# skamann/mcmc-dynamics

Measured on AMD Instinct MI355X. Metric: star-walker log-L terms/sec, higher is better.
Workload: dtype f64; 1 GPU; C3: 1e6 synthetic stars x 256 walkers, rotation+dispersion + fixed single-Gaussian background mixture (ConstantFit + background.Gaussian), fixed centre; stars_per_gpu=1000000, stars_total=1000000, walkers=256, likelihood=bgfixed, parallelism=1 GPU

## Files before the change

include/mcd.h:

```cpp
#ifndef MCD_H
#define MCD_H

#include <stdint.h>

#ifdef __cplusplus
extern "C" {
#endif

#define MCD_ABI_VERSION 1
#define MCD_UNIQUE_ID_BYTES 128

typedef struct mcd_ctx mcd_ctx;
typedef struct mcd_catalog mcd_catalog;

typedef enum {
    MCD_OK = 0,
    MCD_ERR_INVALID = -1,
    MCD_ERR_HIP = -2,
    MCD_ERR_RCCL = -3,
    MCD_ERR_NO_DEVICE = -4,
    MCD_ERR_NONFINITE = -5,
    MCD_ERR_NOMEM = -6
} mcd_status;

typedef enum {
    MCD_MODEL_CONST = 0,
    MCD_MODEL_CONST_BGFIXED = 1,
    MCD_MODEL_CONST_BGGAUSS = 2,
    MCD_MODEL_PROFILE = 3,
    MCD_MODEL_PROFILE_BGGAUSS = 4,
    MCD_MODEL_PROFILE_BGDENS = 5,
    MCD_MODEL_PROFILE_BGFIXED = 6
} mcd_model;

typedef enum {
    MCD_CENTRE_FIXED = 0,
    MCD_CENTRE_FREE = 1
} mcd_centre;

typedef enum {
    MCD_F64 = 0,
    MCD_F32 = 1,
    MCD_F32_ACC64 = 2
} mcd_precision;

typedef struct {
    int64_t n_stars;
    const double* ra;
    const double* dec;
    const double* v;
    const double* verr;
    const double* lnlike_bg;
    const double* pmember;
    const double* density;
    int32_t model;
    int32_t centre;
    int32_t precision;
    int32_t reserved;
    double ra_center;
    double dec_center;
    int64_t n_bins;
    const int64_t* bin_offsets;
} mcd_catalog_desc;


int mcd_ctx_create(int n_dev, const int* dev_ids, mcd_ctx** out);

int mcd_get_unique_id(void* out_id);
int mcd_ctx_create_rank(int device, int rank, int n_ranks, const void* unique_id, mcd_ctx** out);

int mcd_ctx_set_option(mcd_ctx* ctx, const char* key, int64_t value);
int mcd_ctx_abort(mcd_ctx* ctx, const char* reason);
int mcd_ctx_failed(const mcd_ctx* ctx);

int mcd_ctx_destroy(mcd_ctx* ctx);
int mcd_ctx_n_devices(const mcd_ctx* ctx);
int mcd_ctx_comm_info(const mcd_ctx* ctx, int* comm_size, int* comm_rank, int* rccl_version);


int mcd_catalog_create(mcd_ctx* ctx, const mcd_catalog_desc* desc, mcd_catalog** out);
int mcd_catalog_destroy(mcd_catalog* cat);

int mcd_catalog_param_count(const mcd_catalog* cat);
int64_t mcd_catalog_n_stars(const mcd_catalog* cat);
int64_t mcd_catalog_n_outputs(const mcd_catalog* cat, int64_t n_walkers);


int mcd_loglike_batch(mcd_catalog* cat, int64_t n_walkers, int32_t k, const double* params, double* out);

int mcd_params_upload(mcd_catalog* cat, int64_t n_walkers, int32_t k, const double* params);
int mcd_loglike_enqueue(mcd_catalog* cat);
int mcd_loglike_fetch(mcd_catalog* cat, double* out);
int mcd_sync(mcd_catalog* cat);

int mcd_membership(mcd_catalog* cat, int32_t k, const double* params, double* out);
int mcd_loglike_per_star(mcd_catalog* cat, int32_t k, const double* params, double* out);
int mcd_loglike_grad_batch(mcd_catalog* cat, int64_t n_walkers, int32_t k, const double* params, double* out,
                           double* grad);
int mcd_pointwise_posterior(mcd_catalog* cat, int64_t n_samples, int32_t k, const double* params,
                            double* lppd, double* lnl_var, double* pmem_mean, double* pmem_std);
int mcd_psis_loo(mcd_catalog* cat, int64_t n_samples, int32_t k, const double* params, double r_eff,
                 double* elpd_loo, double* pareto_k, double* lppd, double* n_eff);

int mcd_kde_background(mcd_ctx* ctx, int64_t n_comp, const double* comp, int64_t n, const double* v,
                       const double* verr, double sigma_int, double* out, double* kernel_ms);


typedef struct {
    int64_t n_walkers;
    int32_t n_dim;
    int32_t k;
    const int32_t* col_source;
    const double* col_const;
    const double* col_factor;
    const double* lo;
    const double* hi;
    int32_t fixed_ok;
    int32_t n_bins;
} mcd_stretch_desc;

int mcd_stretch_move(mcd_catalog* cat, const mcd_stretch_desc* desc, int64_t n_steps, double* pos, double* lnp,
                     const int32_t* order, const double* zz, const double* thr, const int32_t* pick, double* chain,
                     double* lnprob_chain, int64_t* accepted);
int mcd_stretch_move_seeded(mcd_catalog* cat, const mcd_stretch_desc* desc, int64_t n_steps, double* pos, double* lnp,
                            uint64_t seed, int64_t step0, double* chain, double* lnprob_chain, int64_t* accepted);
int mcd_chain_numbers(uint64_t seed, int64_t step0, int64_t n_steps, int64_t n_bins, int64_t n_walkers, int32_t n_dim,
                      int32_t* order, double* zz, double* thr, int32_t* pick);

int mcd_stretch_info(const mcd_catalog* cat, int64_t* device_blocks, int64_t* host_blocks, int64_t* discarded_blocks,
                     int32_t* last_discard_status);

typedef struct {
    mcd_stretch_desc map;
    const double* chol;
    double step_size;
    double jitter;
    int32_t n_leap;
} mcd_hmc_desc;

int mcd_hmc_block(mcd_catalog* cat, const mcd_hmc_desc* desc, int64_t n_steps, double* pos, double* lnp, uint64_t seed,
                  int64_t step0, double* chain, double* lnprob_chain, int64_t* accepted, double* energy_error);
int mcd_hmc_numbers(uint64_t seed, int64_t step0, int64_t n_steps, int64_t n_walkers, int32_t n_dim, double* z, double* thr,
                    double* eps_factor);
int mcd_hmc_info(const mcd_catalog* cat, int64_t* device_blocks, int64_t* host_blocks);


const char* mcd_last_error(void);
int mcd_abi_version(void);
double mcd_last_kernel_ms(const mcd_catalog* cat);
double mcd_last_device_ms(const mcd_catalog* cat);
int mcd_set_option(mcd_catalog* cat, const char* key, int64_t value);
int mcd_timing_collect(mcd_catalog* cat, double* total_kernel_ms, int64_t* n_launches);
int64_t mcd_rerun_count(const mcd_catalog* cat);
int mcd_last_prefetch(const mcd_catalog* cat);
int mcd_last_narrow_bounded(const mcd_catalog* cat);
int64_t mcd_last_series_chunks(const mcd_catalog* cat);
int64_t mcd_last_direct_chunks(const mcd_catalog* cat);
int mcd_last_fast_level(const mcd_catalog* cat);

int mcd_last_f32_domain(const mcd_catalog* cat, double* kappa_v, double* kappa_theta);
int mcd_last_launch_info(const mcd_catalog* cat, int64_t* n_workgroups, int32_t* walker_tile,
                         int64_t* n_chunks, int32_t* record_bytes);

#ifdef __cplusplus
}
#endif
#endif
```

mcmc_dynamics_amd/_native.py:

```python
import atexit
import ctypes
import os
import weakref

import numpy as np

_HERE = os.path.dirname(os.path.abspath(__file__))
LIB_PATH = os.environ.get("MCD_LIB_PATH") or os.path.join(_HERE, "libmcd_hip.so")

MODEL_CONST, MODEL_CONST_BGFIXED, MODEL_CONST_BGGAUSS = 0, 1, 2
MODEL_PROFILE, MODEL_PROFILE_BGGAUSS, MODEL_PROFILE_BGDENS, MODEL_PROFILE_BGFIXED = 3, 4, 5, 6
CENTRE_FIXED, CENTRE_FREE = 0, 1
F64, F32, F32_ACC64 = 0, 1, 2
PRECISIONS = {"f64": F64, "f32": F32, "f32acc64": F32_ACC64}
UNIQUE_ID_BYTES = 128

_c_double_p = ctypes.POINTER(ctypes.c_double)
_c_int64_p = ctypes.POINTER(ctypes.c_int64)

SYMBOLS = {
    "mcd_ctx_create": (ctypes.c_int, [ctypes.c_int, ctypes.POINTER(ctypes.c_int), ctypes.POINTER(ctypes.c_void_p)]),
    "mcd_get_unique_id": (ctypes.c_int, [ctypes.c_void_p]),
    "mcd_ctx_create_rank": (ctypes.c_int, [ctypes.c_int, ctypes.c_int, ctypes.c_int, ctypes.c_void_p,
                                           ctypes.POINTER(ctypes.c_void_p)]),
    "mcd_ctx_destroy": (ctypes.c_int, [ctypes.c_void_p]),
    "mcd_ctx_set_option": (ctypes.c_int, [ctypes.c_void_p, ctypes.c_char_p, ctypes.c_int64]),
    "mcd_ctx_abort": (ctypes.c_int, [ctypes.c_void_p, ctypes.c_char_p]),
    "mcd_ctx_failed": (ctypes.c_int, [ctypes.c_void_p]),
    "mcd_ctx_n_devices": (ctypes.c_int, [ctypes.c_void_p]),
    "mcd_ctx_comm_info": (ctypes.c_int, [ctypes.c_void_p, ctypes.POINTER(ctypes.c_int), ctypes.POINTER(ctypes.c_int),
                                         ctypes.POINTER(ctypes.c_int)]),
    "mcd_catalog_create": (ctypes.c_int, [ctypes.c_void_p, ctypes.c_void_p, ctypes.POINTER(ctypes.c_void_p)]),
    "mcd_catalog_destroy": (ctypes.c_int, [ctypes.c_void_p]),
    "mcd_catalog_param_count": (ctypes.c_int, [ctypes.c_void_p]),
    "mcd_catalog_n_stars": (ctypes.c_int64, [ctypes.c_void_p]),
    "mcd_catalog_n_outputs": (ctypes.c_int64, [ctypes.c_void_p, ctypes.c_int64]),
    "mcd_loglike_batch": (ctypes.c_int, [ctypes.c_void_p, ctypes.c_int64, ctypes.c_int32, _c_double_p, _c_double_p]),
    "mcd_loglike_grad_batch": (ctypes.c_int, [ctypes.c_void_p, ctypes.c_int64, ctypes.c_int32, _c_double_p, _c_double_p,
                                              _c_double_p]),
    "mcd_params_upload": (ctypes.c_int, [ctypes.c_void_p, ctypes.c_int64, ctypes.c_int32, _c_double_p]),
    "mcd_loglike_enqueue": (ctypes.c_int, [ctypes.c_void_p]),
    "mcd_loglike_fetch": (ctypes.c_int, [ctypes.c_void_p, _c_double_p]),
    "mcd_sync": (ctypes.c_int, [ctypes.c_void_p]),
    "mcd_membership": (ctypes.c_int, [ctypes.c_void_p, ctypes.c_int32, _c_double_p, _c_double_p]),
    "mcd_loglike_per_star": (ctypes.c_int, [ctypes.c_void_p, ctypes.c_int32, _c_double_p, _c_double_p]),
    "mcd_pointwise_posterior": (ctypes.c_int, [ctypes.c_void_p, ctypes.c_int64, ctypes.c_int32, _c_double_p, _c_double_p,
                                               _c_double_p, _c_double_p, _c_double_p]),
    "mcd_psis_loo": (ctypes.c_int, [ctypes.c_void_p, ctypes.c_int64, ctypes.c_int32, _c_double_p, ctypes.c_double,
                                    _c_double_p, _c_double_p, _c_double_p, _c_double_p]),
    "mcd_kde_background": (ctypes.c_int, [ctypes.c_void_p, ctypes.c_int64, _c_double_p, ctypes.c_int64, _c_double_p,
                                          _c_double_p, ctypes.c_double, _c_double_p, _c_double_p]),
    "mcd_stretch_move": (ctypes.c_int, [ctypes.c_void_p, ctypes.c_void_p, ctypes.c_int64, _c_double_p, _c_double_p,
                                        ctypes.POINTER(ctypes.c_int32), _c_double_p, _c_double_p,
                                        ctypes.POINTER(ctypes.c_int32), _c_double_p, _c_double_p, _c_int64_p]),
    "mcd_stretch_move_seeded": (ctypes.c_int, [ctypes.c_void_p, ctypes.c_void_p, ctypes.c_int64, _c_double_p, _c_double_p,
                                               ctypes.c_uint64, ctypes.c_int64, _c_double_p, _c_double_p, _c_int64_p]),
    "mcd_chain_numbers": (ctypes.c_int, [ctypes.c_uint64, ctypes.c_int64, ctypes.c_int64, ctypes.c_int64, ctypes.c_int64,
                                         ctypes.c_int32, ctypes.POINTER(ctypes.c_int32), _c_double_p, _c_double_p,
                                         ctypes.POINTER(ctypes.c_int32)]),
    "mcd_stretch_info": (ctypes.c_int, [ctypes.c_void_p, _c_int64_p, _c_int64_p, _c_int64_p, ctypes.POINTER(ctypes.c_int32)]),
    "mcd_hmc_block": (ctypes.c_int, [ctypes.c_void_p, ctypes.c_void_p, ctypes.c_int64, _c_double_p, _c_double_p,
                                     ctypes.c_uint64, ctypes.c_int64, _c_double_p, _c_double_p, _c_int64_p, _c_double_p]),
    "mcd_hmc_numbers": (ctypes.c_int, [ctypes.c_uint64, ctypes.c_int64, ctypes.c_int64, ctypes.c_int64, ctypes.c_int32,
                                       _c_double_p, _c_double_p, _c_double_p]),
    "mcd_hmc_info": (ctypes.c_int, [ctypes.c_void_p, _c_int64_p, _c_int64_p]),
    "mcd_last_error": (ctypes.c_char_p, []),
    "mcd_abi_version": (ctypes.c_int, []),
    "mcd_last_kernel_ms": (ctypes.c_double, [ctypes.c_void_p]),
    "mcd_last_device_ms": (ctypes.c_double, [ctypes.c_void_p]),
    "mcd_timing_collect": (ctypes.c_int, [ctypes.c_void_p, _c_double_p, _c_int64_p]),
    "mcd_rerun_count": (ctypes.c_int64, [ctypes.c_void_p]),
    "mcd_last_prefetch": (ctypes.c_int, [ctypes.c_void_p]),
    "mcd_last_narrow_bounded": (ctypes.c_int, [ctypes.c_void_p]),
    "mcd_last_series_chunks": (ctypes.c_int64, [ctypes.c_void_p]),
    "mcd_last_direct_chunks": (ctypes.c_int64, [ctypes.c_void_p]),
    "mcd_last_fast_level": (ctypes.c_int, [ctypes.c_void_p]),
    "mcd_last_f32_domain": (ctypes.c_int, [ctypes.c_void_p, _c_double_p, _c_double_p]),
    "mcd_set_option": (ctypes.c_int, [ctypes.c_void_p, ctypes.c_char_p, ctypes.c_int64]),
    "mcd_last_launch_info": (ctypes.c_int, [ctypes.c_void_p, _c_int64_p, ctypes.POINTER(ctypes.c_int32), _c_int64_p,
                                            ctypes.POINTER(ctypes.c_int32)]),
}


class NativeError(RuntimeError):
    """Raised when the HIP library is missing, fails to load, or a call returns an error status."""


class CatalogDesc(ctypes.Structure):
    _fields_ = [
        ("n_stars", ctypes.c_int64),
        ("ra", _c_double_p), ("dec", _c_double_p), ("v", _c_double_p), ("verr", _c_double_p),
        ("lnlike_bg", _c_double_p), ("pmember", _c_double_p), ("density", _c_double_p),
        ("model", ctypes.c_int32), ("centre", ctypes.c_int32), ("precision", ctypes.c_int32),
        ("reserved", ctypes.c_int32),
        ("ra_center", ctypes.c_double), ("dec_center", ctypes.c_double),
        ("n_bins", ctypes.c_int64), ("bin_offsets", _c_int64_p),
    ]


class StretchDesc(ctypes.Structure):
    _fields_ = [
        ("n_walkers", ctypes.c_int64), ("n_dim", ctypes.c_int32), ("k", ctypes.c_int32),
        ("col_source", ctypes.POINTER(ctypes.c_int32)), ("col_const", _c_double_p), ("col_factor", _c_double_p),
        ("lo", _c_double_p), ("hi", _c_double_p), ("fixed_ok", ctypes.c_int32), ("n_bins", ctypes.c_int32),
    ]


class HmcDesc(ctypes.Structure):
    _fields_ = [("map", StretchDesc), ("chol", _c_double_p), ("step_size", ctypes.c_double), ("jitter", ctypes.c_double),
                ("n_leap", ctypes.c_int32)]


TEST_SWITCHES = ("MCD_LIB_PATH", "MCD_RCCL_LIBRARY", "MCD_ALLOW_SHARED_DEVICE", "MCD_FORCE_RCCL", "MCD_TARGET_WAVES",
                 "MCD_CHAIN_PART_BYTES", "MCD_CHAIN_PARTS", "MCD_COLLECTIVE_TIMEOUT_MS")

_lib = None
_live_catalogs = weakref.WeakSet()
_live_contexts = weakref.WeakSet()


@atexit.register
def _shutdown():
    for cat in list(_live_catalogs):
        try:
            cat.close()
        except Exception:
            pass
    for ctx in list(_live_contexts):
        try:
            ctx.close()
        except Exception:
            pass


def load_library(path=None):
    global _lib
    if _lib is not None and path is None:
        return _lib
    p = path or LIB_PATH
    if not os.path.exists(p):
        raise NativeError(
            "HIP library not found at {0}: build it with `make -C mcmc_dynamics_amd/csrc` "
            "(or __graft_entry__.build()); there is no CPU fallback.".format(p))
    try:
        lib = ctypes.CDLL(p)
    except OSError as exc:
        raise NativeError("could not load {0}: {1}".format(p, exc))
    for name, (restype, argtypes) in SYMBOLS.items():
        try:
            fn = getattr(lib, name)
        except AttributeError:
            raise NativeError("{0} does not export {1}".format(p, name))
        fn.restype = restype
        fn.argtypes = argtypes
    if path is None:
        _lib = lib
        active = ["{0}={1}".format(k, os.environ[k]) for k in TEST_SWITCHES if os.environ.get(k)]
        if active:
            import logging
            logging.getLogger("mcmc_dynamics_amd").warning(
                "test / tuning switches active (none is needed in production, see INTEGRATION.md): %s", ", ".join(active))
    return lib


def _check(lib, rc, what):
    if rc != 0:
        msg = lib.mcd_last_error()
        raise NativeError("{0} failed (status {1}): {2}".format(what, rc, msg.decode() if msg else ""))


def _f64(a):
    return np.ascontiguousarray(a, dtype=np.float64)


def _ptr(a):
    return a.ctypes.data_as(_c_double_p) if a is not None else None


class Context(object):

    def __init__(self, n_devices=1, device_ids=None, rank=None, n_ranks=None, unique_id=None, device=None):
        self.lib = load_library()
        handle = ctypes.c_void_p()
        if rank is not None:
            uid = ctypes.create_string_buffer(bytes(unique_id), UNIQUE_ID_BYTES) if unique_id is not None else None
            rc = self.lib.mcd_ctx_create_rank(int(device or 0), int(rank), int(n_ranks), uid, ctypes.byref(handle))
            _check(self.lib, rc, "mcd_ctx_create_rank")
            self.rank, self.n_ranks = int(rank), int(n_ranks)
        else:
            ids = None
            if device_ids is not None:
                ids = (ctypes.c_int * len(device_ids))(*[int(d) for d in device_ids])
                n_devices = len(device_ids)
            rc = self.lib.mcd_ctx_create(int(n_devices), ids, ctypes.byref(handle))
            _check(self.lib, rc, "mcd_ctx_create")
            self.rank, self.n_ranks = 0, 1
        self.handle = handle
        self.host_group = None
        self._catalogs = weakref.WeakSet()
        _live_contexts.add(self)

    @staticmethod
    def unique_id():
        lib = load_library()
        buf = ctypes.create_string_buffer(UNIQUE_ID_BYTES)
        _check(lib, lib.mcd_get_unique_id(buf), "mcd_get_unique_id")
        return buf.raw

    @property
    def n_devices(self):
        return self.lib.mcd_ctx_n_devices(self.handle)

    def set_option(self, key, value):
        _check(self.lib, self.lib.mcd_ctx_set_option(self.handle, key.encode(), int(value)), "mcd_ctx_set_option")

    def abort(self, reason=""):
        if getattr(self, "handle", None):
            self.lib.mcd_ctx_abort(self.handle, str(reason).encode()[:400])

    @property
    def failed(self):
        return bool(getattr(self, "handle", None)) and bool(self.lib.mcd_ctx_failed(self.handle))

    def comm_info(self):
        n, r, v = ctypes.c_int(), ctypes.c_int(), ctypes.c_int()
        _check(self.lib, self.lib.mcd_ctx_comm_info(self.handle, ctypes.byref(n), ctypes.byref(r), ctypes.byref(v)),
               "mcd_ctx_comm_info")
        return {"size": n.value, "rank": r.value, "rccl_version": v.value}
# ... 121 lines not shown
        if p.shape[-1] != self.k:
            raise ValueError("params have {0} columns, catalogue expects {1}".format(p.shape[-1], self.k))
        return np.ascontiguousarray(p), w

    def _alive(self):
        if not getattr(self, "handle", None):
            raise NativeError("catalogue is closed")

    def loglike(self, params):
        self._alive()
        p, w = self._params(params)
        out = np.empty((self.n_sets, w) if self.n_sets > 1 else (w,), dtype=np.float64)
        rc = self.lib.mcd_loglike_batch(self.handle, w, self.k, _ptr(p), _ptr(out))
        _check(self.lib, rc, "mcd_loglike_batch")
        self._walkers = w
        return out

    def loglike_grad(self, params, want_value=True):
        self._alive()
        p, w = self._params(params)
        lead = (self.n_sets, w) if self.n_sets > 1 else (w,)
        out = np.empty(lead, dtype=np.float64) if want_value else None
        grad = np.empty(lead + (self.k,), dtype=np.float64)
        rc = self.lib.mcd_loglike_grad_batch(self.handle, w, self.k, _ptr(p), _ptr(out), _ptr(grad))
        _check(self.lib, rc, "mcd_loglike_grad_batch")
        self._walkers = w
        return out, grad

    def upload_params(self, params):
        p, w = self._params(params)
        _check(self.lib, self.lib.mcd_params_upload(self.handle, w, self.k, _ptr(p)), "mcd_params_upload")
        self._walkers = w

    def enqueue(self):
        _check(self.lib, self.lib.mcd_loglike_enqueue(self.handle), "mcd_loglike_enqueue")

    def sync(self):
        _check(self.lib, self.lib.mcd_sync(self.handle), "mcd_sync")

    def fetch(self):
        w = self._walkers
        out = np.empty((self.n_sets, w) if self.n_sets > 1 else (w,), dtype=np.float64)
        _check(self.lib, self.lib.mcd_loglike_fetch(self.handle, _ptr(out)), "mcd_loglike_fetch")
        return out

    def membership(self, params_row):
        p = _f64(params_row).reshape(-1)
        out = np.empty(self.n_stars, dtype=np.float64)
        _check(self.lib, self.lib.mcd_membership(self.handle, p.size, _ptr(p), _ptr(out)), "mcd_membership")
        return out

    def loglike_per_star(self, params_row):
        p = _f64(params_row).reshape(-1)
        out = np.empty(self.n_stars, dtype=np.float64)
        _check(self.lib, self.lib.mcd_loglike_per_star(self.handle, p.size, _ptr(p), _ptr(out)), "mcd_loglike_per_star")
        return out

    def pointwise_posterior(self, table, membership=False):
        self._alive()
        if self.n_sets > 1:
            raise ValueError("pointwise_posterior is defined for un-binned catalogues only")
        p = _f64(table)
        if p.ndim == 1:
            p = p[None, :]
        if p.ndim != 2 or p.shape[1] != self.k:
            raise ValueError("table must have shape (S, {0})".format(self.k))
        p = np.ascontiguousarray(p)
        names = ("lppd", "lnl_var") + (("pmem_mean", "pmem_std") if membership else ())
        out = {k: np.empty(self.n_stars, dtype=np.float64) for k in names}
        ptrs = [_ptr(out[k]) if k in out else None for k in ("lppd", "lnl_var", "pmem_mean", "pmem_std")]
        rc = self.lib.mcd_pointwise_posterior(self.handle, p.shape[0], self.k, _ptr(p), *ptrs)
        _check(self.lib, rc, "mcd_pointwise_posterior")
        return out

    def psis_loo(self, table, r_eff=1.0):
        self._alive()
        if self.n_sets > 1:
            raise ValueError("psis_loo is defined for un-binned catalogues only")
        p = _f64(table)
        if p.ndim == 1:
            p = p[None, :]
        if p.ndim != 2 or p.shape[1] != self.k:
            raise ValueError("table must have shape (S, {0})".format(self.k))
        p = np.ascontiguousarray(p)
        names = ("elpd_loo", "pareto_k", "lppd", "n_eff")
        out = {k: np.empty(self.n_stars, dtype=np.float64) for k in names}
        rc = self.lib.mcd_psis_loo(self.handle, p.shape[0], self.k, _ptr(p), float(r_eff), *[_ptr(out[k]) for k in names])
        _check(self.lib, rc, "mcd_psis_loo")
        return out

    def _stretch_args(self, name, plan, pos, lnp, n_steps, chain, lnprob_chain, accepted):
        self._alive()
        for a in (pos, lnp):
            if a.dtype != np.float64 or not a.flags.c_contiguous:
                raise ValueError(name + " needs C-contiguous arrays of the documented dtypes")
        if pos.ndim not in (2, 3) or lnp.shape != pos.shape[:-1]:
            raise ValueError(name + ": inconsistent array shapes")
        lead, (w, p) = pos.shape[:-2], pos.shape[-2:]
        cols = [np.ascontiguousarray(plan["col_source"], dtype=np.int32), _f64(plan["col_const"]), _f64(plan["col_factor"]),
                _f64(plan["lo"]), _f64(plan["hi"])]
        if cols[0].size != self.k or cols[1].size != self.k or cols[2].size != self.k or cols[3].size != p or cols[4].size != p:
            raise ValueError("stretch_move: plan does not match the catalogue / the number of free parameters")
        d = StretchDesc()
        d.n_walkers, d.n_dim, d.k, d.n_bins = w, p, self.k, lead[0] if lead else 1
        d.col_source = cols[0].ctypes.data_as(ctypes.POINTER(ctypes.c_int32))
        d.col_const, d.col_factor, d.lo, d.hi = (_ptr(c) for c in cols[1:])
        d.fixed_ok = 1 if plan.get("fixed_ok", True) else 0
        for a, shape in ((chain, (n_steps,) + lead + (w, p)), (lnprob_chain, (n_steps,) + lead + (w,))):
            if a is not None and (a.dtype != np.float64 or not a.flags.c_contiguous or a.shape != shape):
                raise ValueError("stretch_move: chain buffers must be C-contiguous float64 of shape (steps, [B,] W, P) / (steps, [B,] W)")
        if accepted is not None and (accepted.dtype != np.int64 or accepted.shape != lead + (w,) or not accepted.flags.c_contiguous):
            raise ValueError("stretch_move: accepted must be a C-contiguous int64 array of shape ([B,] W)")
        return ((self.handle, ctypes.byref(d), n_steps, _ptr(pos), _ptr(lnp)),
                (_ptr(chain), _ptr(lnprob_chain), accepted.ctypes.data_as(_c_int64_p) if accepted is not None else None), cols)

    def stretch_move(self, plan, pos, lnp, order, zz, thr, pick, chain=None, lnprob_chain=None, accepted=None):
        head, tail, _keep = self._stretch_args("stretch_move", plan, pos, lnp, order.shape[0], chain, lnprob_chain, accepted)
        for a, dt in ((zz, np.float64), (thr, np.float64), (order, np.int32), (pick, np.int32)):
            if a.dtype != dt or not a.flags.c_contiguous:
                raise ValueError("stretch_move needs C-contiguous arrays of the documented dtypes")
        half_shape = (order.shape[0], 2) + pos.shape[:-2] + (pos.shape[-2] // 2,)
        if order.shape != order.shape[:1] + lnp.shape or zz.shape != half_shape or thr.shape != half_shape or \
                pick.shape != half_shape:
            raise ValueError("stretch_move: inconsistent array shapes")
        rc = self.lib.mcd_stretch_move(*head, order.ctypes.data_as(ctypes.POINTER(ctypes.c_int32)), _ptr(zz), _ptr(thr),
                                       pick.ctypes.data_as(ctypes.POINTER(ctypes.c_int32)), *tail)
        _check(self.lib, rc, "mcd_stretch_move")
        self._walkers = pos.shape[-2] // 2

    def stretch_move_seeded(self, plan, pos, lnp, seed, step0, n_steps, chain=None, lnprob_chain=None, accepted=None):
        if n_steps < 0 or step0 < 0:
            raise ValueError("stretch_move_seeded: inconsistent array shapes")
        head, tail, _keep = self._stretch_args("stretch_move_seeded", plan, pos, lnp, n_steps, chain, lnprob_chain, accepted)
        rc = self.lib.mcd_stretch_move_seeded(*head, int(seed) & 0xFFFFFFFFFFFFFFFF, int(step0), *tail)
        _check(self.lib, rc, "mcd_stretch_move_seeded")
        self._walkers = pos.shape[-2] // 2

    @property
    def last_prefetch(self):
        return self.lib.mcd_last_prefetch(self.handle)

    @property
    def last_narrow_bounded(self):
        return self.lib.mcd_last_narrow_bounded(self.handle)

    @property
    def last_series_chunks(self):
        return self.lib.mcd_last_series_chunks(self.handle)

    @property
    def last_direct_chunks(self):
        return self.lib.mcd_last_direct_chunks(self.handle)

    def hmc_block(self, plan, chol, step_size, n_leap, pos, lnp, seed, step0, n_steps, chain=None, lnprob_chain=None,
                  accepted=None, energy_error=None, jitter=0.1):
        if n_steps < 0 or step0 < 0 or pos.ndim != 2:
            raise ValueError("hmc_block: inconsistent array shapes")
        head, tail, _keep = self._stretch_args("hmc_block", plan, pos, lnp, n_steps, chain, lnprob_chain, accepted)
        chol = np.ascontiguousarray(chol, dtype=np.float64)
        if chol.shape != (pos.shape[1], pos.shape[1]):
            raise ValueError("hmc_block: chol must have shape (P, P)")
        if energy_error is not None and (energy_error.dtype != np.float64 or not energy_error.flags.c_contiguous or
                                         energy_error.shape != (n_steps, pos.shape[0])):
            raise ValueError("hmc_block: energy_error must be a C-contiguous float64 array of shape (steps, W)")
        d = HmcDesc()
        d.map = head[1]._obj
        d.chol, d.step_size, d.jitter, d.n_leap = _ptr(chol), float(step_size), float(jitter), int(n_leap)
        rc = self.lib.mcd_hmc_block(self.handle, ctypes.byref(d), int(n_steps), head[3], head[4],
                                    int(seed) & 0xFFFFFFFFFFFFFFFF, int(step0), *tail, _ptr(energy_error))
        _check(self.lib, rc, "mcd_hmc_block")

    def hmc_info(self):
        a, b = ctypes.c_int64(), ctypes.c_int64()
        _check(self.lib, self.lib.mcd_hmc_info(self.handle, ctypes.byref(a), ctypes.byref(b)), "mcd_hmc_info")
        return {"device_blocks": a.value, "host_blocks": b.value}

    def stretch_info(self):
        a, b, c, st = ctypes.c_int64(), ctypes.c_int64(), ctypes.c_int64(), ctypes.c_int32()
        _check(self.lib, self.lib.mcd_stretch_info(self.handle, ctypes.byref(a), ctypes.byref(b), ctypes.byref(c), ctypes.byref(st)),
               "mcd_stretch_info")
        return {"device_blocks": a.value, "host_blocks": b.value, "discarded_blocks": c.value, "last_discard_status": st.value}

    def set_option(self, key, value):
        _check(self.lib, self.lib.mcd_set_option(self.handle, key.encode(), int(value)), "mcd_set_option")

    @property
    def last_kernel_ms(self):
        return self.lib.mcd_last_kernel_ms(self.handle)

    @property
    def last_device_ms(self):
        return self.lib.mcd_last_device_ms(self.handle)

    def timing_collect(self):
        total, n = ctypes.c_double(), ctypes.c_int64()
        _check(self.lib, self.lib.mcd_timing_collect(self.handle, ctypes.byref(total), ctypes.byref(n)),
               "mcd_timing_collect")
        return total.value, n.value

    @property
    def rerun_count(self):
        return self.lib.mcd_rerun_count(self.handle)

    @property
    def fast_level(self):
        return self.lib.mcd_last_fast_level(self.handle)

    @property
    def f32_in_domain(self):
        return bool(self.lib.mcd_last_f32_domain(self.handle, None, None))

    @property
    def f32_condition(self):
        kv, kt = ctypes.c_double(), ctypes.c_double()
        self.lib.mcd_last_f32_domain(self.handle, ctypes.byref(kv), ctypes.byref(kt))
        return kv.value, kt.value

    def launch_info(self):
        wg, ch = ctypes.c_int64(), ctypes.c_int64()
        tile, rb = ctypes.c_int32(), ctypes.c_int32()
        _check(self.lib, self.lib.mcd_last_launch_info(self.handle, ctypes.byref(wg), ctypes.byref(tile),
                                                       ctypes.byref(ch), ctypes.byref(rb)), "mcd_last_launch_info")
        return {"workgroups": wg.value, "walker_tile": tile.value, "chunks": ch.value, "record_bytes": rb.value,
                "series_chunks": self.last_series_chunks, "direct_chunks": self.last_direct_chunks}

    def close(self):
        if getattr(self, "handle", None):
            self.lib.mcd_catalog_destroy(self.handle)
            self.handle = None

    def __del__(self):
        try:
            self.close()
        except Exception:
            pass
```

mcmc_dynamics_amd/csrc/mcd_api_catalog.hip:

```cpp
#include "mcd_host.h"

using namespace mcd::host;

namespace {

int param_count(int model, bool free_centre) {
    int k = (mcd::is_profile(model) ? 6 : 4) + (free_centre ? 2 : 0);
    const int bg = mcd::bg_kind(model);
    if (bg == mcd::BG_GAUSS) k += 3;
    if (bg == mcd::BG_FIXED_DENSITY) k += 1;
    return k;
}

void free_workset(WorkSet& w) {
    if (w.d_chunks) (void)hipFree(w.d_chunks);
    if (w.d_offsets) (void)hipFree(w.d_offsets);
    if (w.d_chunk_general) (void)hipFree(w.d_chunk_general);
    if (w.d_params) (void)hipFree(w.d_params);
    if (w.d_wpar) (void)hipFree(w.d_wpar);
    if (w.d_partials) (void)hipFree(w.d_partials);
    if (w.d_out) (void)hipFree(w.d_out);
    if (w.d_out2) (void)hipFree(w.d_out2);
    if (w.d_partials2) (void)hipFree(w.d_partials2);
    if (w.d_grad_partials) (void)hipFree(w.d_grad_partials);
    if (w.d_grad_out) (void)hipFree(w.d_grad_out);
    if (w.h_grad_out) (void)hipHostFree(w.h_grad_out);
    if (w.ev_staged) (void)hipEventDestroy(w.ev_staged);
    for (int b = 0; b < 2; ++b) {
        if (w.ev_reduced[b]) (void)hipEventDestroy(w.ev_reduced[b]);
        if (w.ev_comm[b]) (void)hipEventDestroy(w.ev_comm[b]);
    }
    if (w.h_params) (void)hipHostFree(w.h_params);
    if (w.h_out) (void)hipHostFree(w.h_out);
    w = WorkSet();
}

double model_cost(int model, bool free_centre) {
    static const double kCost[mcd::kNumModels] = {8.5, 24.0, 45.0, 25.0, 60.0, 40.0, 42.0};
    return (kCost[model] + (free_centre ? 7.0 : 0.0)) / 8.5;
}
int balance_auto_m(const mcd_catalog* cat, int64_t n, int64_t n_walkers) {
    const int64_t n_wtiles = (n_walkers + 63) / 64;
    const double tiles = n_wtiles <= 4 ? (double)n_wtiles : 4.0 * (double)((n_wtiles + 3) / 4);
    const double work = (double)n * tiles / 4.0 * model_cost(cat->model, cat->free_centre);
    const double limit = mcd::bg_kind(cat->model) == mcd::BG_NONE ? 9.0e5 : 1.3e6;
    if (cat->n_psets != 1 || work > limit) return 0;
    return work < 6.0e4 ? 2 : (work <= 3.4e5 ? 4 : 8);
}

bool wants_prefetch(const mcd_catalog* cat, const Shard& sh) {
    if (cat->prefetch >= 0) return cat->prefetch != 0;
    const size_t bytes = (size_t)sh.n * (size_t)mcd::record_bytes(cat->model, cat->free_centre, cat->precision);
    if (mcd::bg_kind(cat->model) == mcd::BG_NONE) return cat->n_psets == 1 && bytes >= ((size_t)128 << 20);
    return bytes >= ((size_t)8 << 20);
}

bool wants_sorted(const mcd_catalog* cat, const Shard& sh) {
    if (cat->model != mcd::MODEL_BGFIXED || cat->free_centre || cat->precision != MCD_F64 || cat->n_psets != 1 || sh.n <= 0)
        return false;
    if (cat->verr_sorted >= 0) return cat->verr_sorted != 0;
    if (cat->chunk_len > 0) return false;
    return (size_t)sh.n * (size_t)mcd::record_bytes(cat->model, cat->free_centre, cat->precision) >= ((size_t)8 << 20);
}

int ensure_sorted_records(mcd_catalog* cat, Shard& sh) {
    if (sh.records_sorted) return MCD_OK;
    const DeviceSlot& slot = cat->ctx->slots[sh.slot];
    constexpr int ND = mcd::record_doubles(mcd::MODEL_BGFIXED, false);
    const size_t n = (size_t)sh.n, bytes = n * ND * sizeof(double);
    MCD_HIP(hipStreamSynchronize(slot.stream));
    std::vector<double> rec(n * ND), out(n * ND);
    MCD_HIP(hipMemcpy(rec.data(), sh.records, bytes, hipMemcpyDeviceToHost));
    const std::vector<int64_t> perm = mcd::verr_order(rec.data(), (int64_t)n, ND);
    sh.sorted_e2.resize(n);
    for (size_t i = 0; i < n; ++i) {
        std::memcpy(&out[i * ND], &rec[(size_t)perm[i] * ND], ND * sizeof(double));
        sh.sorted_e2[i] = out[i * ND + 1];
    }
    sh.sorted_exceptions = mcd::permuted_exceptions(cat->stats.narrow_exceptions, perm, sh.star_begin);
    void* d = nullptr;
    MCD_HIP(hipMalloc(&d, bytes + 2048));
    hipError_t e = hipMemset(d, 0, bytes + 2048);
    if (e == hipSuccess) e = hipMemcpy(d, out.data(), bytes, hipMemcpyHostToDevice);
    if (e != hipSuccess) { (void)hipFree(d); MCD_HIP(e); }
    sh.records_sorted = d;
    return MCD_OK;
}

struct Option {
    const char* key;
    int64_t min, max;
    const char* message;
    bool sync, replan;
    void (*set)(mcd_catalog* c, int64_t v);
    bool (*accepts)(int64_t v) = nullptr;
};
constexpr int64_t kMin = std::numeric_limits<int64_t>::min(), kMax = std::numeric_limits<int64_t>::max();
#define MCD_SET(statement) [](mcd_catalog* c, int64_t v) { statement; }
const Option kOptions[] = {
    {"fast_path", 0, 2, "fast_path: 0 (plain), 1 (guarded, default) or 2 (guarded, no narrow variant)", false, false, MCD_SET(c->allow_fast = (int)v)},
    {"zero_copy", kMin, kMax, nullptr, false, false, MCD_SET(c->zero_copy = v != 0)},
    {"device_chain", 0, 2, "device_chain: 0 (host-driven blocks), 1 (default) or 2 (as 1 with the general step kernel, testing aid)", false, false,
     MCD_SET(c->device_chain = (int)v; c->chain_backoff = 0; c->chain_consecutive = 0; c->chain_hint = -1)},
    {"fused_reduce", kMin, kMax, nullptr, false, false, MCD_SET(c->fused_reduce = v != 0)},
    {"defer_guard", kMin, kMax, nullptr, false, false, MCD_SET(c->defer_guard = v != 0)},
    {"f32_domain", kMin, kMax, nullptr, false, false, MCD_SET(c->f32_domain = v != 0)},
    {"loo_scratch_mb", 1, kMax, "loo_scratch_mb must be >= 1", false, false, MCD_SET(c->loo_scratch_mb = v)},
    {"posterior_pass", 1, kMax, "posterior_pass must be >= 1", false, false, MCD_SET(c->posterior_pass = v)},
    {"two_lanes", kMin, kMax, nullptr, true, false, MCD_SET(c->two_lanes = v != 0)},
    {"narrow_bounded", 0, 1, "narrow_bounded: 1 (where the guard admits it, default) or 0 (never)", false, false, MCD_SET(c->narrow_bounded = (int)v)},
    {"verr_sorted", -1, 1, "verr_sorted: -1 (by record volume, default), 0 (catalogue order) or 1 (sorted by verr)", true, true, MCD_SET(c->verr_sorted = (int)v)},
    {"root_series", 0, 1, "root_series: 1 (series root on the narrow chunks of verr-sorted records, default) or 0 (never)", false, false, MCD_SET(c->root_series = (int)v)},
    {"root_direct", 0, 1, "root_direct: 1 (direct form of the series root where a chunk admits it, default) or 0 (delta form only)", false, false, MCD_SET(c->root_direct = (int)v)},
    {"prefetch", -1, 1, "prefetch: -1 (by record volume, default), 0 (off) or 1 (on)", false, false, MCD_SET(c->prefetch = (int)v)},
    {"spin_us", 0, kMax, "spin_us must be >= 0", false, false, MCD_SET(c->spin_us = v)},
    {"tail_split", kMin, kMax, nullptr, true, true, MCD_SET(c->tail_split = (int)v)},
    {"target_waves", 1, kMax, "target_waves must be positive", true, true, MCD_SET(c->target_waves = v)},
    {"chunk_len", 0, kMax, "chunk_len must be >= 0", true, true, MCD_SET(c->chunk_len = v)},
    {"balance", -1, 8, "balance: -1 (auto), 0 (off) or 1 .. 8 workgroups per CU", true, true, MCD_SET(c->balance = (int)v)},
    {"combine", 0, 16, "combine: 0 (never), 1 (largest workgroup the plan allows), 8 or 16 (waves per workgroup at most)", true, true,
     MCD_SET(c->combine = (int)v), [](int64_t v) { return v <= 1 || v == 8 || v == 16; }},
};
#undef MCD_SET
}

MCD_HOST_BEGIN

LaunchShape main_launch_shape(mcd_catalog* cat, const Shard& sh, const WorkSet& w, int level, bool coll, double* out_buf,
                              int64_t n_out) {
    LaunchShape shape{cat->model, cat->free_centre, cat->precision, level, w.uniform_len, sh.n};
    shape.uniform_extra = w.uniform_extra;
    shape.waves = w.waves;
    shape.chunk_general = w.d_chunk_general;
    shape.prefetch = wants_prefetch(cat, sh);
    cat->last_prefetch = shape.prefetch && shape.fast != 0;
    shape.rerun_flag = coll ? nullptr : out_buf + n_out;
    shape.root_series = w.sorted && cat->root_series != 0;
    shape.root_direct = shape.root_series && cat->root_direct != 0;
    return shape;
}

const void* main_records(const Shard& sh, const WorkSet& w) { return w.sorted ? sh.records_sorted : sh.records; }

int64_t series_chunk_count(const mcd_catalog* cat, const WorkSet& w, int level, const double* params, int64_t n_rows) {
    if (!w.sorted || !cat->root_series || level != 2 || w.series_need.empty()) return 0;
    const mcd::ParamRanges pr = mcd::table_ranges(cat->model, cat->free_centre, cat->k, params, n_rows);
    if (!pr.finite) return 0;
    return (int64_t)(std::upper_bound(w.series_need.begin(), w.series_need.end(), pr.s2_min) - w.series_need.begin());
}

int64_t direct_chunk_count(const mcd_catalog* cat, const WorkSet& w, int level, const double* params, int64_t n_rows) {
    if (!w.sorted || !cat->root_series || !cat->root_direct || level != 2 || w.direct_need.empty()) return 0;
    const mcd::ParamRanges pr = mcd::table_ranges(cat->model, cat->free_centre, cat->k, params, n_rows);
    if (!pr.finite) return 0;
    return (int64_t)(std::upper_bound(w.direct_need.begin(), w.direct_need.end(), pr.s2_min) - w.direct_need.begin());
}

const double* fast_pset_const(const mcd_catalog* cat, const Shard& sh, int level) {
    const int bgk = mcd::bg_kind(cat->model);
    return (level && (bgk == mcd::BG_FIXED || bgk == mcd::BG_FIXED_DENSITY)) ? sh.d_pset_const : nullptr;
}

int build_workset(mcd_catalog* cat, Shard& sh, int64_t n_walkers, WorkSet** out) {
    auto it = sh.work.find(n_walkers);
    if (it != sh.work.end()) { *out = &it->second; return MCD_OK; }
    if (sh.work.size() >= 8) {
        for (auto& kv : sh.work) free_workset(kv.second);
        sh.work.clear();
        cat->cur_walkers = 0;
    }
    const DeviceSlot& slot = cat->ctx->slots[sh.slot];
    MCD_HIP(hipSetDevice(slot.device));

    const bool sorted = wants_sorted(cat, sh);
    if (sorted)
        if (int rc = ensure_sorted_records(cat, sh)) return rc;
    const std::vector<int64_t>& exceptions = sorted ? sh.sorted_exceptions : cat->stats.narrow_exceptions;
    mcd::ChunkPlan plan;
    for (int m = cat->balance < 0 ? balance_auto_m(cat, sh.n, n_walkers) : cat->balance;; m /= 2) {
        plan = mcd::plan_chunks(cat->bin_offsets, sh.star_begin, sh.n, n_walkers, cat->target_waves, cat->tail_split,
                                exceptions, cat->chunk_len, m);
        if (m == 0 || plan.balanced_m > 0) break;
    }
    const std::vector<mcd::Chunk>& chunks = plan.chunks;
    const std::vector<int64_t>& offs = plan.offsets;
    const std::vector<uint8_t>& general = plan.general;

    WorkSet w;
    w.n_walkers = n_walkers;
    w.n_chunks = (int64_t)chunks.size();
    w.max_chunks_per_pset = plan.max_chunks_per_pset;
    w.uniform_len = plan.uniform_len;
    w.uniform_extra = plan.uniform_extra;
    w.sorted = sorted;
    if (sorted) {
        w.series_need = mcd::series_thresholds(plan, sh.sorted_e2.data());
        w.direct_need = mcd::direct_thresholds(plan, sh.sorted_e2.data());
    }
    {
        const int64_t n_wtiles = (n_walkers + 63) / 64;
        const bool shape_ok = plan.balanced_m > 0 && plan.balanced_m % 2 == 0 && (n_wtiles == 1 || n_wtiles == 2 || n_wtiles == 4) &&
                              cat->precision == MCD_F64;
        w.waves = 4;
        if (cat->combine != 0 && shape_ok) {
            const bool can16 = mcd::bg_kind(cat->model) != mcd::BG_GAUSS;
            w.waves = 8;
            if (cat->combine == 16 && plan.balanced_m % 4 == 0 && can16) w.waves = 16;
            if (cat->combine == 1 && plan.balanced_m == 4 && can16) w.waves = 16;
        }
    }
    const int64_t n_out = cat->n_psets * n_walkers;
    const size_t term_bytes = cat->precision == MCD_F64 ? 8 : 4;
    auto allocate = [&]() -> hipError_t {
        hipError_t e;
        if (!general.empty()) {
            if ((e = hipMalloc(&w.d_chunk_general, general.size())) != hipSuccess) return e;
            if ((e = hipMemcpy(w.d_chunk_general, general.data(), general.size(), hipMemcpyHostToDevice)) != hipSuccess) return e;
        }
        if ((e = hipMalloc(&w.d_chunks, std::max<size_t>(1, chunks.size()) * sizeof(mcd::Chunk))) != hipSuccess) return e;
        if ((e = hipMalloc(&w.d_offsets, offs.size() * sizeof(int64_t))) != hipSuccess) return e;
        if ((e = hipMalloc(&w.d_params, (size_t)n_out * cat->k * sizeof(double))) != hipSuccess) return e;
        if ((e = hipMalloc(&w.d_wpar, (size_t)n_out * mcd::KD * term_bytes)) != hipSuccess) return e;
        if ((e = hipMalloc(&w.d_partials, std::max<size_t>(1, (size_t)mcd::padded_walkers(n_walkers) * w.n_chunks) * sizeof(double))) != hipSuccess) return e;
        if ((e = hipMalloc(&w.d_out, (size_t)(n_out + 1) * sizeof(double))) != hipSuccess) return e;
        if ((e = hipMemset(w.d_out, 0, (size_t)(n_out + 1) * sizeof(double))) != hipSuccess) return e;
        if ((e = hipMalloc(&w.d_out2, (size_t)(n_out + 1) * sizeof(double))) != hipSuccess) return e;
        if ((e = hipMemset(w.d_out2, 0, (size_t)(n_out + 1) * sizeof(double))) != hipSuccess) return e;
        if ((e = hipEventCreateWithFlags(&w.ev_staged, hipEventDisableTiming)) != hipSuccess) return e;
        for (int b = 0; b < 2; ++b) {
            if ((e = hipEventCreateWithFlags(&w.ev_reduced[b], hipEventDisableTiming)) != hipSuccess) return e;
            if ((e = hipEventCreateWithFlags(&w.ev_comm[b], hipEventDisableTiming)) != hipSuccess) return e;
        }
        if ((e = hipHostMalloc(&w.h_params, (size_t)n_out * cat->k * sizeof(double), hipHostMallocMapped)) != hipSuccess) return e;
        if ((e = hipHostMalloc(&w.h_out, (size_t)(n_out + 1) * sizeof(double), hipHostMallocMapped)) != hipSuccess) return e;
        std::memset(w.h_out, 0, (size_t)(n_out + 1) * sizeof(double));
        if ((e = hipHostGetDevicePointer((void**)&w.m_params, w.h_params, 0)) != hipSuccess) return e;
        if ((e = hipHostGetDevicePointer((void**)&w.m_out, w.h_out, 0)) != hipSuccess) return e;
        if (!chunks.empty() &&
            (e = hipMemcpy(w.d_chunks, chunks.data(), chunks.size() * sizeof(mcd::Chunk), hipMemcpyHostToDevice)) != hipSuccess)
            return e;
        return hipMemcpy(w.d_offsets, offs.data(), offs.size() * sizeof(int64_t), hipMemcpyHostToDevice);
    };
    const hipError_t err = allocate();
    if (err != hipSuccess) {
        free_workset(w);
        return fail(MCD_ERR_HIP, std::string("work buffers for this walker count: ") + hipGetErrorString(err));
    }
    auto ins = sh.work.emplace(n_walkers, w);
    *out = &ins.first->second;
    return MCD_OK;
}

MCD_HOST_END

extern "C" {

static int catalog_create_impl(mcd_ctx* ctx, const mcd_catalog_desc* d, std::unique_ptr<mcd_catalog>& cat);

int mcd_catalog_create(mcd_ctx* ctx, const mcd_catalog_desc* d, mcd_catalog** out) {
    try {
    if (!ctx || !d || !out) return fail(MCD_ERR_INVALID, "mcd_catalog_create: null argument");
    std::unique_ptr<mcd_catalog> cat;
    const int rc = catalog_create_impl(ctx, d, cat);
    if (rc != MCD_OK) {
        if (cat) {
            const std::string msg = g_last_error;
            mcd_catalog_destroy(cat.release());
            g_last_error = msg;
        }
        return rc;
    }
    *out = cat.release();
    return MCD_OK;
    } catch (...) { return on_exception("mcd_catalog_create"); }
}

static int catalog_create_impl(mcd_ctx* ctx, const mcd_catalog_desc* d, std::unique_ptr<mcd_catalog>& cat) {
    if (int urc = ctx_usable(ctx)) return urc;
    if (d->n_stars < 0) return fail(MCD_ERR_INVALID, "negative n_stars");
    if (d->model < 0 || d->model >= mcd::kNumModels) return fail(MCD_ERR_INVALID, "unknown model");
    const int bgk = mcd::bg_kind(d->model);
    if (d->centre != MCD_CENTRE_FIXED && d->centre != MCD_CENTRE_FREE) return fail(MCD_ERR_INVALID, "unknown centre mode");
    if (d->precision < MCD_F64 || d->precision > MCD_F32_ACC64) return fail(MCD_ERR_INVALID, "unknown precision");
    if (d->n_stars > 0 && (!d->ra || !d->dec || !d->v || !d->verr)) return fail(MCD_ERR_INVALID, "missing ra/dec/v/verr column");
    if (bgk == mcd::BG_FIXED && d->n_stars > 0 && (!d->lnlike_bg || !d->pmember))
        return fail(MCD_ERR_INVALID, "background model needs lnlike_bg and pmember columns");
    if (bgk == mcd::BG_GAUSS && d->n_stars > 0 && !d->density)
        return fail(MCD_ERR_INVALID, "Gaussian-background model needs the density column");
    if (bgk == mcd::BG_FIXED_DENSITY && d->n_stars > 0 && (!d->lnlike_bg || !d->density))
        return fail(MCD_ERR_INVALID, "constant-background model needs lnlike_bg and density columns");

    cat.reset(new (std::nothrow) mcd_catalog());
    if (!cat) return fail(MCD_ERR_INVALID, "out of memory");
    cat->ctx = ctx;
    cat->model = d->model;
    cat->free_centre = d->centre == MCD_CENTRE_FREE;
    cat->precision = d->precision;
    cat->k = param_count(d->model, cat->free_centre);
    cat->n_stars = d->n_stars;
    if (const char* tw = std::getenv("MCD_TARGET_WAVES")) {
        long v = std::atol(tw);
        if (v > 0) cat->target_waves = v;
    }
    if (d->n_bins > 1) {
        if (!d->bin_offsets) return fail(MCD_ERR_INVALID, "bin_offsets required when n_bins > 1");
        cat->n_psets = d->n_bins;
        cat->bin_offsets.assign(d->bin_offsets, d->bin_offsets + d->n_bins + 1);
        if (cat->bin_offsets.front() != 0 || cat->bin_offsets.back() != d->n_stars)
            return fail(MCD_ERR_INVALID, "bin_offsets must start at 0 and end at n_stars");
        for (int64_t b = 0; b < d->n_bins; ++b)
            if (cat->bin_offsets[b + 1] < cat->bin_offsets[b]) return fail(MCD_ERR_INVALID, "bin_offsets must be non-decreasing");
    } else {
        cat->n_psets = 1;
        cat->bin_offsets = {0, d->n_stars};
    }

    cat->stats = mcd::compute_stats(d->n_stars, d->v, d->verr, d->lnlike_bg, d->pmember, d->density, bgk,
                                    cat->precision != MCD_F64 || mcd::is_profile(cat->model) ? d->ra : nullptr, d->dec,
                                    !cat->free_centre, d->ra_center, d->dec_center);

    const int n_dev = (int)ctx->slots.size();
    cat->shards.resize(n_dev);
    const int rec_bytes = mcd::record_bytes(cat->model, cat->free_centre, cat->precision);
    for (int i = 0; i < n_dev; ++i) {
        Shard& sh = cat->shards[i];
        sh.slot = i;
        const mcd::ShardRange range = mcd::shard_range(d->n_stars, i, n_dev);
        sh.star_begin = range.begin;
        sh.n = range.n;
        const DeviceSlot& slot = ctx->slots[i];
        MCD_HIP(hipSetDevice(slot.device));
        MCD_HIP(hipEventCreate(&sh.ev_begin));
        MCD_HIP(hipEventCreate(&sh.ev_k0));
        MCD_HIP(hipEventCreate(&sh.ev_k1));
        MCD_HIP(hipEventCreate(&sh.ev_end));
        MCD_HIP(hipMalloc(&sh.records, (size_t)sh.n * rec_bytes + 2048));
        MCD_HIP(hipMemsetAsync(sh.records, 0, (size_t)sh.n * rec_bytes + 2048, slot.stream));
        if (bgk == mcd::BG_FIXED || bgk == mcd::BG_FIXED_DENSITY) {
            const std::vector<double> sums = mcd::pset_background_sums(d->lnlike_bg, cat->bin_offsets, sh.star_begin, sh.n);
            MCD_HIP(hipMalloc(&sh.d_pset_const, sums.size() * sizeof(double)));
            MCD_HIP(hipMemcpy(sh.d_pset_const, sums.data(), sums.size() * sizeof(double), hipMemcpyHostToDevice));
        }
        if (sh.n == 0) continue;
        const double* host_cols[7] = {d->ra, d->dec, d->v, d->verr, d->lnlike_bg, d->pmember, d->density};
        struct Scratch {
            double* p[7] = {nullptr, nullptr, nullptr, nullptr, nullptr, nullptr, nullptr};
            ~Scratch() { for (double* q : p) if (q) (void)hipFree(q); }
        } dev;
        for (int c = 0; c < 7; ++c) {
            if (!host_cols[c]) continue;
            MCD_HIP(hipMalloc(&dev.p[c], (size_t)sh.n * sizeof(double)));
            MCD_HIP(hipMemcpyAsync(dev.p[c], host_cols[c] + sh.star_begin, (size_t)sh.n * sizeof(double),
                                   hipMemcpyHostToDevice, slot.stream));
        }
        mcd::RawColumns raw{dev.p[0], dev.p[1], dev.p[2], dev.p[3], dev.p[4], dev.p[5], dev.p[6]};
        MCD_HIP(mcd::launch_prepare_records(slot.stream, raw, sh.n, cat->model, cat->free_centre, cat->precision,
                                            d->ra_center, d->dec_center, sh.records));
        MCD_HIP(hipStreamSynchronize(slot.stream));
    }
    return MCD_OK;
}

int mcd_catalog_destroy(mcd_catalog* cat) {
    if (!cat) return MCD_OK;
    if (cat->ctx && cat->ctx->failed.load()) { delete cat; return MCD_OK; }
    for (Shard& sh : cat->shards) {
        (void)hipSetDevice(cat->ctx->slots[sh.slot].device);
        (void)hipStreamSynchronize(cat->ctx->slots[sh.slot].stream);
        (void)hipStreamSynchronize(cat->ctx->slots[sh.slot].comm_stream);
        (void)hipStreamSynchronize(cat->ctx->slots[sh.slot].stream2);
        for (auto& kv : sh.work) free_workset(kv.second);
        if (sh.records) (void)hipFree(sh.records);
        if (sh.records_sorted) (void)hipFree(sh.records_sorted);
        if (sh.d_pset_const) (void)hipFree(sh.d_pset_const);
        if (sh.ev_begin) (void)hipEventDestroy(sh.ev_begin);
        if (sh.ev_k0) (void)hipEventDestroy(sh.ev_k0);
        if (sh.ev_k1) (void)hipEventDestroy(sh.ev_k1);
        if (sh.ev_end) (void)hipEventDestroy(sh.ev_end);
        for (auto& pr : sh.ring) { (void)hipEventDestroy(pr.first); (void)hipEventDestroy(pr.second); }
    }
    for (hipEvent_t e : cat->chain_events) (void)hipEventDestroy(e);
    if (cat->chain.d) (void)hipFree(cat->chain.d);
    if (cat->chain.h) (void)hipHostFree(cat->chain.h);
    if (cat->hmc.d) (void)hipFree(cat->hmc.d);
    if (cat->hmc.h) (void)hipHostFree(cat->hmc.h);
    delete cat;
    return MCD_OK;
}

int mcd_catalog_param_count(const mcd_catalog* cat) { return cat ? cat->k : MCD_ERR_INVALID; }
int64_t mcd_catalog_n_stars(const mcd_catalog* cat) { return cat ? cat->n_stars : MCD_ERR_INVALID; }
int64_t mcd_catalog_n_outputs(const mcd_catalog* cat, int64_t n_walkers) {
    return cat ? cat->n_psets * n_walkers : MCD_ERR_INVALID;
}

int mcd_set_option(mcd_catalog* cat, const char* key, int64_t value) {
    try {
    if (!cat || !key) return fail(MCD_ERR_INVALID, "mcd_set_option: null argument");
    if (!std::strcmp(key, "timing")) {
        int rc = sync_all(cat);
        if (rc != MCD_OK) return rc;
        cat->timing = value != 0;
        cat->timing_all = value == 2;
        for (Shard& sh : cat->shards) sh.ring_used = 0;
        return MCD_OK;
    }
    if (!std::strcmp(key, "timing_discard")) {
        int rc = sync_all(cat);
        if (rc != MCD_OK) return rc;
        for (Shard& sh : cat->shards) sh.ring_used = 0;
        cat->timing_launches = 0;
        return MCD_OK;
    }
    if (!std::strcmp(key, "timing_stride")) {
        if (value < 1) return fail(MCD_ERR_INVALID, "timing_stride must be >= 1");
        int rc = sync_all(cat);
        if (rc != MCD_OK) return rc;
        cat->timing_stride = value;
        cat->timing_launches = 0;
        return MCD_OK;
    }
    if (!std::strcmp(key, "timing_reserve")) {
        if (value < 0 || value > ((int64_t)1 << 16)) return fail(MCD_ERR_INVALID, "timing_reserve: 0 .. 65536 launches");
        for (Shard& sh : cat->shards) {
            MCD_HIP(hipSetDevice(cat->ctx->slots[sh.slot].device));
            while ((int64_t)sh.ring.size() < value) {
                hipEvent_t a, b;
                MCD_HIP(hipEventCreate(&a));
                if (hipEventCreate(&b) != hipSuccess) { (void)hipEventDestroy(a); return fail(MCD_ERR_HIP, "hipEventCreate"); }
                sh.ring.emplace_back(a, b);
            }
        }
        return MCD_OK;
    }
    for (const Option& o : kOptions) {
        if (std::strcmp(key, o.key)) continue;
        if (value < o.min || value > o.max || (o.accepts && !o.accepts(value))) return fail(MCD_ERR_INVALID, o.message);
        if (o.sync)
            if (int rc = sync_all(cat)) return rc;
        o.set(cat, value);
        if (o.replan) {
            for (Shard& sh : cat->shards) {
                (void)hipSetDevice(cat->ctx->slots[sh.slot].device);
                for (auto& kv : sh.work) free_workset(kv.second);
                sh.work.clear();
            }
            cat->cur_walkers = 0;
        }
        return MCD_OK;
    }
    return fail(MCD_ERR_INVALID, std::string("unknown option: ") + key);
    } catch (...) { return on_exception("mcd_set_option"); }
}

int mcd_timing_collect(mcd_catalog* cat, double* total_kernel_ms, int64_t* n_launches) {
    try {
    if (!cat) return fail(MCD_ERR_INVALID, "null catalogue");
    int rc = sync_all(cat);
    if (rc != MCD_OK) return rc;
    Shard& sh = cat->shards[0];
    double total = 0.0;
    for (size_t i = 0; i < sh.ring_used; ++i) {
        float ms = 0.f;
        MCD_HIP(hipEventElapsedTime(&ms, sh.ring[i].first, sh.ring[i].second));
        total += ms;
    }
    if (total_kernel_ms) *total_kernel_ms = total;
    if (n_launches) *n_launches = (int64_t)sh.ring_used;
    for (Shard& s2 : cat->shards) s2.ring_used = 0;
    cat->timing_launches = 0;
    return MCD_OK;
    } catch (...) { return on_exception("mcd_timing_collect"); }
}

int64_t mcd_rerun_count(const mcd_catalog* cat) { return cat ? cat->n_reruns : MCD_ERR_INVALID; }

int mcd_stretch_info(const mcd_catalog* cat, int64_t* device_blocks, int64_t* host_blocks, int64_t* discarded_blocks,
                     int32_t* last_discard_status) {
    if (!cat) return fail(MCD_ERR_INVALID, "null catalogue");
    if (device_blocks) *device_blocks = cat->chain_device_blocks;
    if (host_blocks) *host_blocks = cat->chain_host_blocks;
    if (discarded_blocks) *discarded_blocks = cat->chain_discarded;
    if (last_discard_status) *last_discard_status = cat->chain_last_status;
    return MCD_OK;
}

int mcd_last_prefetch(const mcd_catalog* cat) { return cat ? cat->last_prefetch : -1; }

int64_t mcd_last_series_chunks(const mcd_catalog* cat) { return cat ? cat->last_series_chunks : -1; }
int64_t mcd_last_direct_chunks(const mcd_catalog* cat) { return cat ? cat->last_direct_chunks : -1; }

int mcd_last_narrow_bounded(const mcd_catalog* cat) { return cat ? cat->last_narrow_bounded : -1; }

int mcd_last_f32_domain(const mcd_catalog* cat, double* kappa_v, double* kappa_theta) {
    if (!cat) return -1;
    if (kappa_v) *kappa_v = cat->last_f32.kappa_v;
    if (kappa_theta) *kappa_theta = cat->last_f32.kappa_theta;
    if (cat->precision == MCD_F64) return 1;
    return cat->last_f32.inside ? 1 : 0;
}

int mcd_last_fast_level(const mcd_catalog* cat) {
    if (!cat || cat->cur_walkers <= 0 || cat->shards.empty()) return -1;
    const auto it = cat->shards.front().work.find(cat->cur_walkers);
    return it == cat->shards.front().work.end() ? -1 : it->second.fast;
}

double mcd_last_kernel_ms(const mcd_catalog* cat) { return cat ? cat->last_kernel_ms : -1.0; }
double mcd_last_device_ms(const mcd_catalog* cat) { return cat ? cat->last_device_ms : -1.0; }

int mcd_last_launch_info(const mcd_catalog* cat, int64_t* n_workgroups, int32_t* walker_tile, int64_t* n_chunks,
                         int32_t* record_bytes) {
    if (!cat) return fail(MCD_ERR_INVALID, "null catalogue");
    if (n_workgroups) *n_workgroups = cat->last_grid;
    if (walker_tile) *walker_tile = 64;
    if (n_chunks) *n_chunks = cat->last_chunks;
    if (record_bytes) *record_bytes = mcd::record_bytes(cat->model, cat->free_centre, cat->precision);
    return MCD_OK;
}

}
```

mcmc_dynamics_amd/csrc/mcd_api_chain.hip:

```cpp
#include "mcd_host.h"
#include "mcd_rng.h"
#include "mcd_stretch.h"
#include "mcd_grad.h"
#include "mcd_hmc.h"

using namespace mcd::host;

namespace {

void big_copy(void* dst, const void* src, size_t bytes) {
    constexpr size_t kSerial = (size_t)4 << 20;
    if (bytes < kSerial) { std::memcpy(dst, src, bytes); return; }
    constexpr int kMaxThreads = 16;
    static const int kThreads = [] {
        const char* e = std::getenv("MCD_COPY_THREADS");
        const int n = e ? std::atoi(e) : 4;
        return n < 1 ? 1 : (n > kMaxThreads ? kMaxThreads : n);
    }();
    std::thread workers[kMaxThreads - 1];
    const size_t part = (bytes / kThreads + 63) / 64 * 64;
    int started = 0;
    for (int t = 1; t < kThreads; ++t) {
        const size_t at = std::min(bytes, part * t), len = std::min(bytes, part * (t + 1)) - at;
        try {
// ... 14 lines not shown
                         double* lnprob_chain, int64_t* accepted, bool* done, const uint64_t* seed = nullptr,
                         int64_t step0 = 0) {
    *done = false;
    mcd_ctx* ctx = cat->ctx;
    if (int urc = ctx_usable(ctx)) return urc;
    const int64_t B = cat->n_psets;
    if (!cat->device_chain || cat->shards.size() != 1 || cat->precision != MCD_F64 || n_steps < 1 || cat->timing || !d->fixed_ok)
        return MCD_OK;
    if (B > 1 && cat->device_chain != 1) return MCD_OK;
    if (cat->chain_backoff > 0) { --cat->chain_backoff; return MCD_OK; }
    const int64_t W = d->n_walkers, half = W / 2;
    const int P = d->n_dim, K = d->k;
    bool small_ensemble = false;
    {
        mcd::StretchDevice probe;
        probe.n_bins = B; probe.n_walkers = W; probe.n_dim = P; probe.k = K;
        probe.force_general = cat->device_chain == 2;
        if (!mcd::stretch_step_handles(probe)) return MCD_OK;
        small_ensemble = mcd::stretch_step_fuses(probe);
    }
    Shard& sh = cat->shards[0];
    const DeviceSlot& slot = ctx->slots[sh.slot];
    MCD_HIP(hipSetDevice(slot.device));
    WorkSet* wp = nullptr;
    int rc = build_workset(cat, sh, half, &wp);
    if (rc != MCD_OK) return rc;
    WorkSet& w = *wp;
    MCD_WAIT(cat->ctx, slot.stream, cat->spin_us, "mcd_stretch_move (previous evaluation)");
    MCD_WAIT(cat->ctx, slot.stream2, cat->spin_us, "mcd_stretch_move (previous evaluation, second lane)");
    MCD_WAIT(cat->ctx, slot.comm_stream, cat->spin_us, "mcd_stretch_move (previous collective)");
    w.comm_pending[0] = w.comm_pending[1] = false;
    w.staged = false;

    size_t off = 0;
    auto take = [&](size_t bytes) { const size_t at = off; off += (bytes + 63) / 64 * 64; return at; };
    const size_t BW = (size_t)B * W, Bh = (size_t)B * half;
    const size_t o_pos = take(BW * P * 8), o_lnp = take(BW * 8), o_acc = take(BW * 8);
    const size_t o_meta = take(mcd::META_WORDS * 4), o_status = take(8);
    const size_t n_launches = (size_t)2 * n_steps;
    const bool defer = cat->defer_guard != 0 && B == 1 && small_ensemble && n_launches * half * K * 8 <= ((size_t)64 << 20);
    const size_t o_levels = take(defer ? n_launches * 4 : 0);
    const size_t state_end = off;
    const size_t o_src = take((size_t)K * 4), o_const = take((size_t)K * 8), o_fac = take((size_t)K * 8);
    const size_t o_lo = take((size_t)P * 8), o_hi = take((size_t)P * 8);
    const bool seeded = seed != nullptr;
    const bool gen_device = seeded && mcd::chain_numbers_on_device(W);
    const size_t n_in = (size_t)n_steps;
    const size_t o_order = take(n_in * BW * 4), o_zz = take(n_in * BW * 8);
    const size_t o_thr = take(n_in * BW * 8), o_pick = take(n_in * BW * 4);
    const size_t input_end = off;
    const size_t o_prop = take(Bh * P * 8), o_ok = take(Bh), o_nok = take((size_t)2 * B * 4), o_ranges = take((size_t)2 * B * 10 * 8);
    const size_t o_nok_log = take(defer ? n_launches * 4 : 0), o_table_log = take(defer ? n_launches * half * K * 8 : 0);
    const size_t o_chain = take(chain ? (size_t)n_steps * BW * P * 8 : 0);
    const size_t o_lnpc = take(lnprob_chain ? (size_t)n_steps * BW * 8 : 0);
    const size_t total = off;
    ChainArena& a = cat->chain;
    if (a.bytes < total) {
        if (a.d) (void)hipFree(a.d);
        if (a.h) (void)hipHostFree(a.h);
        a = ChainArena();
        const size_t want = total + total / 2;
        const bool must_agree = ctx->n_ranks > 1 || ctx->force_collective;
        if (hipMalloc((void**)&a.d, want) != hipSuccess) {
            (void)hipGetLastError();
            a = ChainArena();
            if (must_agree) return fail(MCD_ERR_NOMEM, "mcd_stretch_move: no device memory for the resident block of this rank (use shorter blocks)");
            return MCD_OK;
        }
        if (hipHostMalloc((void**)&a.h, want, hipHostMallocDefault) != hipSuccess) {
            (void)hipGetLastError();
            (void)hipFree(a.d);
            a = ChainArena();
            if (must_agree) return fail(MCD_ERR_NOMEM, "mcd_stretch_move: no pinned host memory for the resident block of this rank (use shorter blocks)");
            return MCD_OK;
        }
        a.bytes = want;
    }
    std::memcpy(a.h + o_pos, pos, BW * P * 8);
    std::memcpy(a.h + o_lnp, lnp, BW * 8);
    if (accepted) std::memcpy(a.h + o_acc, accepted, BW * 8);
    else std::memset(a.h + o_acc, 0, BW * 8);
    std::memset(a.h + o_meta, 0, mcd::META_WORDS * 4);
    std::memset(a.h + o_status, 0, 8);
    std::memcpy(a.h + o_src, d->col_source, (size_t)K * 4);
    std::memcpy(a.h + o_const, d->col_const, (size_t)K * 8);
    std::memcpy(a.h + o_fac, d->col_factor, (size_t)K * 8);
    std::memcpy(a.h + o_lo, d->lo, (size_t)P * 8);
    std::memcpy(a.h + o_hi, d->hi, (size_t)P * 8);
    const size_t moved = (size_t)n_steps * BW * ((gen_device ? 0 : 24) + (chain ? (size_t)P * 8 : 0) + (lnprob_chain ? 8 : 0));
    size_t part_threshold = (size_t)16 << 20;
    if (const char* e = std::getenv("MCD_CHAIN_PART_BYTES")) part_threshold = (size_t)std::strtoull(e, nullptr, 10);
    int64_t max_parts = 16;
    if (const char* e = std::getenv("MCD_CHAIN_PARTS")) max_parts = std::max<long long>(1, std::atoll(e));
    const int64_t n_parts = moved >= part_threshold ? std::min<int64_t>(max_parts, n_steps) : 1;
    auto part_begin = [&](int64_t k) { return n_steps * k / n_parts; };
    auto copy_in = [&](int64_t i0, int64_t i1) {
        if (gen_device) return;
        const size_t at = (size_t)i0 * BW, n = (size_t)(i1 - i0) * BW;
        if (seeded) {
            std::vector<uint64_t> sorter;
            for (int64_t i = i0; i < i1; ++i)
                mcd::chain_numbers_of_step(*seed, step0 + i, B, W, P, (int32_t*)(a.h + o_order) + (size_t)i * BW,
                                           (double*)(a.h + o_zz) + (size_t)i * BW, (double*)(a.h + o_thr) + (size_t)i * BW,
                                           (int32_t*)(a.h + o_pick) + (size_t)i * BW, sorter);
            return;
        }
        big_copy(a.h + o_order + at * 4, order + at, n * 4);
        big_copy(a.h + o_zz + at * 8, zz + at, n * 8);
        big_copy(a.h + o_thr + at * 8, thr + at, n * 8);
        big_copy(a.h + o_pick + at * 4, pick + at, n * 4);
    };
    if (n_parts == 1) copy_in(0, n_steps);

    int level = cat->chain_hint;
    if (level < 0) {
        std::vector<double> table(BW * K);
        for (size_t j = 0; j < BW; ++j)
            for (int c = 0; c < K; ++c) {
                const int src = d->col_source[c];
                table[j * K + c] = src < 0 ? d->col_const[c]
                                           : (d->col_factor[c] == 1.0 ? pos[j * P + src] : pos[j * P + src] * d->col_factor[c]);
            }
        level = fast_level(cat, table.data(), (int64_t)BW);
    }

    mcd::StretchDevice sd;
    sd.n_bins = B;
    sd.n_walkers = W; sd.n_dim = P; sd.k = K; sd.fixed_ok = d->fixed_ok;
    sd.model = cat->model; sd.free_centre = cat->free_centre ? 1 : 0; sd.allow_fast = cat->allow_fast;
    sd.expected_level = level;
    sd.force_general = cat->device_chain == 2;
    sd.stats = cat->stats;
    sd.col_source = (const int32_t*)(a.d + o_src); sd.col_const = (const double*)(a.d + o_const);
    sd.col_factor = (const double*)(a.d + o_fac); sd.lo = (const double*)(a.d + o_lo); sd.hi = (const double*)(a.d + o_hi);
    sd.pos = (double*)(a.d + o_pos); sd.lnp = (double*)(a.d + o_lnp); sd.accepted = (long long*)(a.d + o_acc);
    sd.order = (const int32_t*)(a.d + o_order); sd.zz = (const double*)(a.d + o_zz); sd.thr = (const double*)(a.d + o_thr);
    sd.pick = (const int32_t*)(a.d + o_pick);
    sd.chain = chain ? (double*)(a.d + o_chain) : nullptr;
    sd.lnprob_chain = lnprob_chain ? (double*)(a.d + o_lnpc) : nullptr;
    sd.proposal = (double*)(a.d + o_prop); sd.ok = (uint8_t*)(a.d + o_ok); sd.meta = (int32_t*)(a.d + o_meta);
    sd.n_ok = (int32_t*)(a.d + o_nok); sd.ranges = (double*)(a.d + o_ranges);
    sd.table = w.d_params; sd.wpar = (double*)w.d_wpar;
    if (defer) {
        sd.defer_guard = 1;
        sd.table_log = (double*)(a.d + o_table_log); sd.n_ok_log = (int32_t*)(a.d + o_nok_log); sd.level_log = (int32_t*)(a.d + o_levels);
    }

    const bool coll = ctx->n_ranks > 1 || ctx->force_collective;
    double* const out_buf = w.d_out;
    mcd::LaunchShape shape = main_launch_shape(cat, sh, w, level, coll, out_buf, (int64_t)Bh);
    cat->last_narrow_bounded = 0;
    cat->last_series_chunks = 0;
    cat->last_direct_chunks = 0;
    const double* pset_const = fast_pset_const(cat, sh, level);
    const int64_t n_slots = mcd::partial_slots(shape, w.n_chunks, half);
    const int64_t max_slots = B == 1 ? n_slots : w.max_chunks_per_pset;
    const bool fused = cat->fused_reduce != 0 && !coll && max_slots <= mcd::kFusedReduceSlots && mcd::stretch_step_fuses(sd);
    sd.fused = fused ? 1 : 0;
    sd.partials = w.d_partials;
    sd.n_slots = n_slots;
    sd.slot_offsets = B == 1 ? nullptr : w.d_offsets;
    sd.pset_const = pset_const;
    cat->chain_last_fused = fused;
    double prev_tag = 0.0;
    int64_t acc_step = -1;
    int acc_h = 0;
#ifdef MCD_CHAIN_STAMPS
    static unsigned long long* d_stamps = nullptr;
    if (!d_stamps) MCD_HIP(hipMalloc((void**)&d_stamps, 8 * 8 * 4096));
    MCD_HIP(hipMemsetAsync(d_stamps, 0, 8 * 8 * 4096, slot.stream));
    sd.stamps = d_stamps;
#endif
    auto enqueue_steps = [&](int64_t i0, int64_t i1, hipEvent_t mark) -> int {
        for (int64_t i = i0; i < i1; ++i)
            for (int h = 0; h < 2; ++h) {
#ifdef MCD_CHAIN_STAMPS
                sd.launch_index = i * 2 + h;
#endif
                MCD_HIP(mcd::launch_stretch_step(slot.stream, sd, acc_step, acc_h, i, h, out_buf, prev_tag));
                if (mark && i == i0 && h == 0) MCD_HIP(hipEventRecord(mark, slot.stream));
                prev_tag = coll ? 0.0 : (double)(++cat->launch_seq);
                shape.launch_tag = prev_tag;
                MCD_HIP(mcd::launch_loglike(slot.stream, shape, main_records(sh, w), w.d_chunks, w.n_chunks, w.d_wpar, w.d_partials, half));
                if (!fused)
                    MCD_HIP(mcd::launch_reduce(slot.stream, w.d_partials, w.d_offsets, B, n_slots, max_slots, half, pset_const,
                                               out_buf));
                if (coll) {
                    if (!ctx->multi_process) MCD_NCCL(g_rccl.GroupStart());
                    MCD_NCCL(g_rccl.AllReduce(out_buf, out_buf, Bh, ncclDouble, ncclSum, slot.comm, slot.stream));
                    if (!ctx->multi_process) MCD_NCCL(g_rccl.GroupEnd());
                }
                acc_step = i;
                acc_h = h;
            }
        return MCD_OK;
    };
    auto finish = [&]() -> int {
        MCD_HIP(mcd::launch_stretch_step(slot.stream, sd, acc_step, acc_h, -1, 0, out_buf, prev_tag));
        if (defer) MCD_HIP(mcd::launch_stretch_judge(slot.stream, sd, (int64_t)n_launches));
        if (coll) {
            double* status = (double*)(a.d + o_status);
            MCD_HIP(mcd::launch_stretch_status(slot.stream, sd.meta, status));
            if (!ctx->multi_process) MCD_NCCL(g_rccl.GroupStart());
            MCD_NCCL(g_rccl.AllReduce(status, status, 1, ncclDouble, ncclSum, slot.comm, slot.stream));
            if (!ctx->multi_process) MCD_NCCL(g_rccl.GroupEnd());
        }
        return MCD_OK;
    };
    struct MidBlockGuard {
        mcd_ctx* ctx; bool armed; bool ok;
        ~MidBlockGuard() {
            if (armed && !ok && !ctx->failed.load()) {
                const std::string cause = g_last_error;
                (void)ctx_fail(ctx, "mcd_stretch_move: this rank failed in the middle of a resident block (" + cause + ")");
            }
        }
    } mid_block{ctx, coll, false};
    bool rows_delivered = false;
    auto generate = [&](hipStream_t s, int64_t i0, int64_t i1) {
        return mcd::launch_chain_numbers(s, *seed, step0, i0, i1, B, W, P, (int32_t*)(a.d + o_order), (double*)(a.d + o_zz),
                                         (double*)(a.d + o_thr), (int32_t*)(a.d + o_pick));
    };
    if (n_parts == 1) {
        MCD_HIP(hipMemcpyAsync(a.d, a.h, gen_device ? o_order : input_end, hipMemcpyHostToDevice, slot.stream));
        if (gen_device) MCD_HIP(generate(slot.stream, 0, n_steps));
        rc = enqueue_steps(0, n_steps, nullptr);
        if (rc != MCD_OK) return rc;
        rc = finish();
        if (rc != MCD_OK) return rc;
        MCD_HIP(hipMemcpyAsync(a.h, a.d, state_end, hipMemcpyDeviceToHost, slot.stream));
        if (total > o_chain)
            MCD_HIP(hipMemcpyAsync(a.h + o_chain, a.d + o_chain, total - o_chain, hipMemcpyDeviceToHost, slot.stream));
        MCD_WAIT(cat->ctx, slot.stream, cat->spin_us, "mcd_stretch_move (resident block)");
    } else {
        while ((int64_t)cat->chain_events.size() < 3 * n_parts) {
            hipEvent_t e;
            MCD_HIP(hipEventCreateWithFlags(&e, hipEventDisableTiming));
            cat->chain_events.push_back(e);
        }
        hipEvent_t* ev_in = cat->chain_events.data();
        hipEvent_t* ev_rows = ev_in + n_parts;
        hipEvent_t* ev_out = ev_rows + n_parts;
        auto rows_to_host = [&](int64_t k) -> int {
            const size_t at = (size_t)part_begin(k) * BW, n = (size_t)(part_begin(k + 1) - part_begin(k)) * BW;
            MCD_HIP(hipStreamWaitEvent(slot.comm_stream, ev_rows[k], 0));
            if (chain) MCD_HIP(hipMemcpyAsync(a.h + o_chain + at * P * 8, a.d + o_chain + at * P * 8, n * P * 8, hipMemcpyDeviceToHost, slot.comm_stream));
            if (lnprob_chain) MCD_HIP(hipMemcpyAsync(a.h + o_lnpc + at * 8, a.d + o_lnpc + at * 8, n * 8, hipMemcpyDeviceToHost, slot.comm_stream));
            MCD_HIP(hipEventRecord(ev_out[k], slot.comm_stream));
            return MCD_OK;
        };
        auto rows_to_caller = [&](int64_t k) -> int {
            const size_t at = (size_t)part_begin(k) * BW, n = (size_t)(part_begin(k + 1) - part_begin(k)) * BW;
            MCD_WAIT(cat->ctx, slot.comm_stream, cat->spin_us, "mcd_stretch_move (chain rows of a part)");
            if (chain) big_copy(chain + at * P, a.h + o_chain + at * P * 8, n * P * 8);
            if (lnprob_chain) big_copy(lnprob_chain + at, a.h + o_lnpc + at * 8, n * 8);
            return MCD_OK;
        };
        MCD_HIP(hipMemcpyAsync(a.d, a.h, o_order, hipMemcpyHostToDevice, slot.stream));
        for (int64_t k = 0; k < n_parts; ++k) {
            const int64_t i0 = part_begin(k), i1 = part_begin(k + 1);
            const size_t at = (size_t)i0 * BW, n = (size_t)(i1 - i0) * BW;
            if (gen_device) {
                MCD_HIP(generate(slot.comm_stream, i0, i1));
                MCD_HIP(hipEventRecord(ev_in[k], slot.comm_stream));
                MCD_HIP(hipStreamWaitEvent(slot.stream, ev_in[k], 0));
            } else {
                copy_in(i0, i1);
                MCD_HIP(hipMemcpyAsync(a.d + o_order + at * 4, a.h + o_order + at * 4, n * 4, hipMemcpyHostToDevice, slot.comm_stream));
                MCD_HIP(hipMemcpyAsync(a.d + o_zz + at * 8, a.h + o_zz + at * 8, n * 8, hipMemcpyHostToDevice, slot.comm_stream));
                MCD_HIP(hipMemcpyAsync(a.d + o_thr + at * 8, a.h + o_thr + at * 8, n * 8, hipMemcpyHostToDevice, slot.comm_stream));
                MCD_HIP(hipMemcpyAsync(a.d + o_pick + at * 4, a.h + o_pick + at * 4, n * 4, hipMemcpyHostToDevice, slot.comm_stream));
                MCD_HIP(hipEventRecord(ev_in[k], slot.comm_stream));
                MCD_HIP(hipStreamWaitEvent(slot.stream, ev_in[k], 0));
            }
            rc = enqueue_steps(i0, i1, k > 0 ? ev_rows[k - 1] : nullptr);
            if (rc != MCD_OK) return rc;
            if (k > 0) {
                rc = rows_to_host(k - 1);
                if (rc != MCD_OK) return rc;
                rc = rows_to_caller(k - 1);
                if (rc != MCD_OK) return rc;
            }
        }
        rc = finish();
        if (rc != MCD_OK) return rc;
        MCD_HIP(hipEventRecord(ev_rows[n_parts - 1], slot.stream));
        MCD_HIP(hipMemcpyAsync(a.h, a.d, state_end, hipMemcpyDeviceToHost, slot.stream));
        rc = rows_to_host(n_parts - 1);
        if (rc != MCD_OK) return rc;
        rc = rows_to_caller(n_parts - 1);
        if (rc != MCD_OK) return rc;
        MCD_WAIT(cat->ctx, slot.stream, cat->spin_us, "mcd_stretch_move (resident block, last part)");
        MCD_WAIT(cat->ctx, slot.comm_stream, cat->spin_us, "mcd_stretch_move (resident block, chain rows)");
        rows_delivered = true;
    }
#ifdef MCD_CHAIN_STAMPS
    {
        const int64_t n = std::min<int64_t>(n_steps * 2, 4096);
        std::vector<unsigned long long> st((size_t)n * 8);
        MCD_HIP(hipMemcpy(st.data(), d_stamps, st.size() * 8, hipMemcpyDeviceToHost));
        double sum[8] = {0}, period = 0;
        int64_t cnt = 0;
        for (int64_t i = 2; i + 1 < n; ++i) {
            for (int k = 1; k < 8; ++k) sum[k] += (double)(st[i * 8 + k] - st[i * 8 + k - 1]);
            period += (double)(st[(i + 1) * 8] - st[i * 8]);
            ++cnt;
// ... 333 lines not shown
```

mcmc_dynamics_amd/csrc/mcd_api_eval.hip:

```cpp
#include "mcd_host.h"
#include "mcd_grad.h"

using namespace mcd::host;

MCD_HOST_BEGIN

int fast_level(const mcd_catalog* cat, const double* params, int64_t n_rows) {
    if (!cat->allow_fast) return 0;
    const int level = mcd::fast_level(cat->stats, cat->model, cat->free_centre, cat->precision != MCD_F64, cat->k, params, n_rows);
    return cat->allow_fast == 2 && level > 1 ? 1 : level;
}

int sync_all(mcd_catalog* cat) {
    if (!cat) return fail(MCD_ERR_INVALID, "null catalogue");
    if (int rc = ctx_usable(cat->ctx)) return rc;
    for (Shard& sh : cat->shards) {
        const DeviceSlot& slot = cat->ctx->slots[sh.slot];
        MCD_HIP(hipSetDevice(slot.device));
        MCD_WAIT(cat->ctx, slot.stream, cat->spin_us, "mcd_sync / mcd_loglike_fetch (compute stream)");
        MCD_WAIT(cat->ctx, slot.stream2, cat->spin_us, "mcd_sync / mcd_loglike_fetch (second compute lane)");
        MCD_WAIT(cat->ctx, slot.comm_stream, cat->spin_us, "mcd_sync / mcd_loglike_fetch (communication stream)");
    }
    if (cat->timing && cat->timing_pending) {
        Shard& sh = cat->shards[0];
        float k_ms = 0.f, d_ms = 0.f;
        if (cat->timing_all) {
            if (sh.ring_used > 0)
                MCD_HIP(hipEventElapsedTime(&k_ms, sh.ring[sh.ring_used - 1].first, sh.ring[sh.ring_used - 1].second));
        } else {
            MCD_HIP(hipEventElapsedTime(&k_ms, sh.ev_k0, sh.ev_k1));
        }
        if (!cat->timing_all) MCD_HIP(hipEventElapsedTime(&d_ms, sh.ev_begin, sh.ev_end));
        cat->last_kernel_ms = k_ms;
        cat->last_device_ms = cat->timing_all ? -1.0 : d_ms;
        cat->timing_pending = false;
    }
    return MCD_OK;
}

MCD_HOST_END

namespace {

WorkSet* find_work(Shard& sh, int64_t W) {
    const auto it = sh.work.find(W);
    return it == sh.work.end() ? nullptr : &it->second;
}

bool all_staged(mcd_catalog* cat) {
    if (cat->cur_walkers <= 0) return false;
    for (Shard& sh : cat->shards) {
        const WorkSet* w = find_work(sh, cat->cur_walkers);
        if (!w || !w->staged) return false;
    }
    return true;
}

int stage_params_impl(mcd_catalog* cat, int64_t n_walkers, int32_t k, const double* params, bool zero_copy) {
    if (!cat || !params) return fail(MCD_ERR_INVALID, "null catalogue or params");
    if (int rc = ctx_usable(cat->ctx)) return rc;
    if (n_walkers <= 0) return fail(MCD_ERR_INVALID, "n_walkers must be positive");
    if (k != cat->k) {
        char buf[128];
        snprintf(buf, sizeof buf, "parameter table has %d columns, catalogue expects %d", (int)k, cat->k);
        return fail(MCD_ERR_INVALID, buf);
    }
    const int64_t n_rows = cat->n_psets * n_walkers;
    if (cat->precision != MCD_F64) {
        cat->last_f32 = mcd::f32_domain(cat->stats, cat->model, cat->free_centre, cat->k, params, n_rows);
        if (!cat->last_f32.inside && cat->f32_domain)
            return fail(MCD_ERR_INVALID, std::string("outside the float32 accuracy domain (use an MCD_F64 catalogue, or option "
                                                     "f32_domain = 0 to evaluate regardless): ") + cat->last_f32.reason);
    }
    const int fast = fast_level(cat, params, n_rows);
    const int narrow_rescale = fast == 2 && cat->precision == MCD_F64
                                   ? mcd::bounded_rescale(cat->stats, cat->model, cat->free_centre, cat->k, params, n_rows) : 0;
    for (Shard& sh : cat->shards) {
        WorkSet* w = nullptr;
        int rc = build_workset(cat, sh, n_walkers, &w);
        if (rc != MCD_OK) return rc;
        const DeviceSlot& slot = cat->ctx->slots[sh.slot];
        MCD_HIP(hipSetDevice(slot.device));
        MCD_WAIT(cat->ctx, slot.stream, cat->spin_us, "mcd_params_upload (previous evaluation)");
        if (w->lane1_used) {
            MCD_WAIT(cat->ctx, slot.stream2, cat->spin_us, "mcd_params_upload (previous evaluation, second lane)");
            w->lane1_used = false;
        }
        std::memcpy(w->h_params, params, (size_t)n_rows * k * sizeof(double));
        w->mapped = zero_copy;
        const double* src = w->m_params;
        if (!zero_copy) {
            MCD_HIP(hipMemcpyAsync(w->d_params, w->h_params, (size_t)n_rows * k * sizeof(double), hipMemcpyHostToDevice,
                                   slot.stream));
            src = w->d_params;
        }
        MCD_HIP(mcd::launch_prepare_walkers(slot.stream, src, n_rows, k, cat->model, cat->free_centre,
                                            cat->precision, w->d_wpar));
        MCD_HIP(hipEventRecord(w->ev_staged, slot.stream));
        w->lane1_knows_staging = false;
        w->fast = fast;
        w->narrow_rescale = narrow_rescale;
        w->series_chunks = series_chunk_count(cat, *w, fast, params, n_rows);
        w->direct_chunks = direct_chunk_count(cat, *w, fast, params, n_rows);
        w->staged = true;
    }
    cat->cur_walkers = n_walkers;
    return MCD_OK;
}

int stage_params(mcd_catalog* cat, int64_t n_walkers, int32_t k, const double* params, bool zero_copy) {
    const int rc = stage_params_impl(cat, n_walkers, k, params, zero_copy);
    if (rc != MCD_OK && cat) cat->cur_walkers = 0;
    return rc;
}

int timing_pair(const mcd_catalog* cat, Shard& sh, bool sampled, hipEvent_t* k0, hipEvent_t* k1) {
    *k0 = sh.ev_k0;
    *k1 = sh.ev_k1;
    if (!(cat->timing_all && sampled)) return MCD_OK;
    if (sh.ring_used >= (size_t)1 << 16) sh.ring_used = 0;
    if (sh.ring_used == sh.ring.size()) {
        hipEvent_t a, b;
        MCD_HIP(hipEventCreate(&a));
        MCD_HIP(hipEventCreate(&b));
        sh.ring.emplace_back(a, b);
    }
    *k0 = sh.ring[sh.ring_used].first;
    *k1 = sh.ring[sh.ring_used].second;
    ++sh.ring_used;
    return MCD_OK;
}

int timing_end(mcd_catalog* cat) {
    if (cat->timing_all) ++cat->timing_launches;
    if (!cat->timing) return MCD_OK;
    if (!cat->timing_all) {
        for (Shard& sh : cat->shards) {
            const DeviceSlot& slot = cat->ctx->slots[sh.slot];
            MCD_HIP(hipSetDevice(slot.device));
            MCD_HIP(hipEventRecord(sh.ev_end, slot.stream));
        }
    }
    cat->timing_pending = true;
    return MCD_OK;
}

int enqueue(mcd_catalog* cat, bool pipelined) {
    if (!cat) return fail(MCD_ERR_INVALID, "null catalogue");
    if (int rc = ctx_usable(cat->ctx)) return rc;
    if (cat->cur_walkers <= 0) return fail(MCD_ERR_INVALID, "no parameters staged (call mcd_params_upload first)");
    if (!all_staged(cat)) return fail(MCD_ERR_INVALID, "no parameters staged for this walker count (the last upload failed?)");
    const int64_t W = cat->cur_walkers;
    const int64_t n_out = cat->n_psets * W;
    mcd_ctx* ctx = cat->ctx;
    for (Shard& sh : cat->shards) {
        WorkSet& w = (*find_work(sh, W));
        const DeviceSlot& slot = ctx->slots[sh.slot];
        MCD_HIP(hipSetDevice(slot.device));
        const bool coll = ctx->has_comm();
        double* out_buf = w.mapped ? w.m_out : w.d_out;
        const bool two_lanes = pipelined && cat->two_lanes && !(cat->timing && !cat->timing_all);
        hipStream_t lane_stream = slot.stream;
        double* lane_partials = w.d_partials;
        if (coll || two_lanes) {
            w.buf ^= 1;
            out_buf = w.buf ? w.d_out2 : w.d_out;
            if (two_lanes && w.buf) {
                if (!w.d_partials2) {
                    MCD_HIP(hipMalloc(&w.d_partials2, std::max<size_t>(1, (size_t)mcd::padded_walkers(W) * w.n_chunks) * sizeof(double)));
                }
                if (!w.lane1_knows_staging) {
                    MCD_HIP(hipStreamWaitEvent(slot.stream2, w.ev_staged, 0));
                    w.lane1_knows_staging = true;
                }
                lane_stream = slot.stream2;
                lane_partials = w.d_partials2;
                w.lane1_used = true;
            }
        } else {
            w.buf = 0;
        }
        mcd::LaunchShape shape = main_launch_shape(cat, sh, w, w.fast, coll, out_buf, n_out);
        shape.narrow_rescale = cat->narrow_bounded ? w.narrow_rescale : 0;
        cat->last_narrow_bounded = mcd::narrow_bounded_launch(shape) ? shape.narrow_rescale : 0;
        if (&sh == &cat->shards.front()) cat->last_series_chunks = cat->last_direct_chunks = 0;
        cat->last_series_chunks += shape.root_series && shape.fast == 2 ? w.series_chunks : 0;
        cat->last_direct_chunks += shape.root_direct && shape.fast == 2 ? w.direct_chunks : 0;
        w.launch_tag = coll ? 0.0 : (double)(++cat->launch_seq);
        shape.launch_tag = w.launch_tag;
        const bool sampled = !cat->timing_all || (cat->timing_launches % cat->timing_stride) == 0;
        hipEvent_t k0, k1;
        if (int rc = timing_pair(cat, sh, sampled, &k0, &k1)) return rc;
        if (cat->timing && !cat->timing_all) MCD_HIP(hipEventRecord(sh.ev_begin, slot.stream));
        if (cat->timing && sampled) MCD_HIP(hipEventRecord(k0, lane_stream));
        MCD_HIP(mcd::launch_loglike(lane_stream, shape, main_records(sh, w), w.d_chunks, w.n_chunks, w.d_wpar, lane_partials, W));
        if (cat->timing && sampled) MCD_HIP(hipEventRecord(k1, lane_stream));
        const double* pset_const = fast_pset_const(cat, sh, w.fast);
        if (coll && w.comm_pending[w.buf]) {
            MCD_HIP(hipStreamWaitEvent(lane_stream, w.ev_comm[w.buf], 0));
            w.comm_pending[w.buf] = false;
        }
        {
            const int64_t n_slots = mcd::partial_slots(shape, w.n_chunks, W);
            MCD_HIP(mcd::launch_reduce(lane_stream, lane_partials, w.d_offsets, cat->n_psets, n_slots,
                                       cat->n_psets == 1 ? n_slots : w.max_chunks_per_pset, W, pset_const, out_buf));
        }
        if (coll && pipelined) MCD_HIP(hipEventRecord(w.ev_reduced[w.buf], lane_stream));
    }
    if (ctx->has_comm()) {
        if (!ctx->multi_process) MCD_NCCL(g_rccl.GroupStart());
        for (Shard& sh : cat->shards) {
            WorkSet& w = (*find_work(sh, W));
            const DeviceSlot& slot = ctx->slots[sh.slot];
            MCD_HIP(hipSetDevice(slot.device));
            double* buf = w.buf ? w.d_out2 : w.d_out;
            if (pipelined) {
                MCD_HIP(hipStreamWaitEvent(slot.comm_stream, w.ev_reduced[w.buf], 0));
                MCD_NCCL(g_rccl.AllReduce(buf, buf, (size_t)n_out, ncclDouble, ncclSum, slot.comm, slot.comm_stream));
            } else {
                if (w.comm_pending[w.buf ^ 1]) {
                    MCD_HIP(hipStreamWaitEvent(slot.stream, w.ev_comm[w.buf ^ 1], 0));
                    w.comm_pending[w.buf ^ 1] = false;
                }
                MCD_NCCL(g_rccl.AllReduce(buf, buf, (size_t)n_out, ncclDouble, ncclSum, slot.comm, slot.stream));
            }
        }
        if (!ctx->multi_process) MCD_NCCL(g_rccl.GroupEnd());
        if (pipelined) {
            for (Shard& sh : cat->shards) {
                WorkSet& w = (*find_work(sh, W));
                const DeviceSlot& slot = ctx->slots[sh.slot];
                MCD_HIP(hipSetDevice(slot.device));
                MCD_HIP(hipEventRecord(w.ev_comm[w.buf], slot.comm_stream));
                w.comm_pending[w.buf] = true;
            }
        }
    }
    if (int rc = timing_end(cat)) return rc;
    {
        WorkSet& w0 = (*find_work(cat->shards[0], W));
        cat->last_chunks = w0.n_chunks;
        mcd::LaunchShape sh0{cat->model, cat->free_centre, cat->precision, w0.fast};
        sh0.waves = w0.waves;
        const int64_t slots = mcd::partial_slots(sh0, w0.n_chunks, W);
        cat->last_grid = slots != w0.n_chunks ? slots : mcd::main_grid(w0.n_chunks, W);
    }
    return MCD_OK;
}

int fetch_once(mcd_catalog* cat, bool* rerun) {
    const int64_t W = cat->cur_walkers;
    const int64_t n_out = cat->n_psets * W;
    *rerun = false;
    const bool coll = cat->ctx->has_comm();
    bool any_fast = false;
    for (Shard& sh : cat->shards) {
        WorkSet& w = (*find_work(sh, W));
        any_fast = any_fast || w.fast != 0;
        const DeviceSlot& slot = cat->ctx->slots[sh.slot];
        MCD_HIP(hipSetDevice(slot.device));
        if (!w.mapped && &sh == &cat->shards[0]) {
            const double* res = w.buf ? w.d_out2 : w.d_out;
            if (w.comm_pending[w.buf]) MCD_HIP(hipStreamWaitEvent(slot.stream, w.ev_comm[w.buf], 0));
            hipStream_t copy_stream = (!coll && w.buf && w.lane1_used) ? slot.stream2 : slot.stream;
            MCD_HIP(hipMemcpyAsync(w.h_out, res, (size_t)(n_out + 1) * sizeof(double), hipMemcpyDeviceToHost, copy_stream));
        }
    }
    int rc = sync_all(cat);
    if (rc != MCD_OK) return rc;
    const WorkSet& w0 = (*find_work(cat->shards[0], W));
    if (coll) {
        for (int64_t i = 0; i < n_out && !*rerun; ++i) *rerun = w0.h_out[i] != w0.h_out[i];
    } else if (any_fast) {
        *rerun = w0.h_out[n_out] == w0.launch_tag;
    }
    return MCD_OK;
}

int fetch(mcd_catalog* cat, double* out) {
    if (!cat || !out) return fail(MCD_ERR_INVALID, "null catalogue or output");
    if (cat->cur_walkers <= 0 || !all_staged(cat)) return fail(MCD_ERR_INVALID, "nothing evaluated yet");
    const int64_t W = cat->cur_walkers;
    const int64_t n_out = cat->n_psets * W;
    bool rerun = false;
    int rc = fetch_once(cat, &rerun);
    if (rc != MCD_OK) return rc;
    if (rerun) {
        ++cat->n_reruns;
        for (Shard& sh : cat->shards) (*find_work(sh, W)).fast = 0;
        rc = enqueue(cat, false);
        if (rc != MCD_OK) return rc;
        rc = fetch_once(cat, &rerun);
        if (rc != MCD_OK) return rc;
    }
    std::memcpy(out, (*find_work(cat->shards[0], W)).h_out, (size_t)n_out * sizeof(double));
    return MCD_OK;
}

int per_star(mcd_catalog* cat, int32_t k, const double* params, int mode, double* out) {
    if (!cat || !params || !out) return fail(MCD_ERR_INVALID, "per-star output: null argument");
    if (mcd::bg_kind(cat->model) == mcd::BG_NONE) return fail(MCD_ERR_INVALID, "per-star outputs need a background model");
    if (cat->n_psets != 1) return fail(MCD_ERR_INVALID, "per-star outputs are defined for un-binned catalogues");
    if (k != cat->k) return fail(MCD_ERR_INVALID, "parameter row has the wrong number of columns");
    const size_t term_bytes = cat->precision == MCD_F64 ? 8 : 4;
    for (Shard& sh : cat->shards) {
        if (sh.n == 0) continue;
        const DeviceSlot& slot = cat->ctx->slots[sh.slot];
        MCD_HIP(hipSetDevice(slot.device));
        double* d_p = nullptr; void* d_w = nullptr; double* d_o = nullptr;
        MCD_HIP(hipMalloc(&d_p, k * sizeof(double)));
        MCD_HIP(hipMalloc(&d_w, mcd::KD * term_bytes));
        MCD_HIP(hipMalloc(&d_o, (size_t)sh.n * sizeof(double)));
        MCD_HIP(hipMemcpyAsync(d_p, params, k * sizeof(double), hipMemcpyHostToDevice, slot.stream));
        MCD_HIP(mcd::launch_prepare_walkers(slot.stream, d_p, 1, k, cat->model, cat->free_centre, cat->precision, d_w));
        mcd::LaunchShape shape{cat->model, cat->free_centre, cat->precision, 0};
        MCD_HIP(mcd::launch_per_star(slot.stream, shape, sh.records, sh.n, d_w, mode, d_o));
        MCD_HIP(hipMemcpyAsync(out + sh.star_begin, d_o, (size_t)sh.n * sizeof(double), hipMemcpyDeviceToHost, slot.stream));
        MCD_HIP(hipStreamSynchronize(slot.stream));
        MCD_HIP(hipFree(d_p)); MCD_HIP(hipFree(d_w)); MCD_HIP(hipFree(d_o));
    }
    return MCD_OK;
}

int loglike_grad(mcd_catalog* cat, int64_t n_walkers, int32_t k, const double* params, double* out, double* grad) {
    if (!cat || !params || !grad) return fail(MCD_ERR_INVALID, "mcd_loglike_grad_batch: null catalogue, params or grad");
    if (int rc = ctx_usable(cat->ctx)) return rc;
    if (cat->precision != MCD_F64) return fail(MCD_ERR_INVALID, "gradients need an MCD_F64 catalogue");
    int rc = stage_params(cat, n_walkers, k, params, false);
    if (rc != MCD_OK) return rc;
    mcd_ctx* ctx = cat->ctx;
    const int64_t W = n_walkers;
    const int64_t fields = 1 + k;
    const int64_t padded = mcd::padded_walkers(W);
    const size_t n_res = (size_t)(cat->n_psets * fields * padded);
    const bool coll = ctx->has_comm();
    for (Shard& sh : cat->shards) {
        WorkSet& w = (*find_work(sh, W));
// ... 103 lines not shown
```

mcmc_dynamics_amd/csrc/mcd_guard.h:

```cpp
#pragma once

#include <algorithm>
#include <cmath>
#include <cstdint>
#include <limits>
#include <vector>

#include "mcd_math.h"

namespace mcd {

constexpr double kInfinity = std::numeric_limits<double>::infinity();

struct StatsScalars {
    double e2_min = 0, e2_max = 0, v_abs_max = 0;
    double rho_min = 0, rho_max = 0;
    double lnbg_min = 0, lnbg_max = 0, pm_max = 0;
    bool stats_finite = true;
    bool extras_ok = true;
    bool narrow_possible = false;
    double r_max_fixed = 0.0;
    double nbp_min = 0, nbp_max = 0;
};

// ... 89 lines not shown

struct GuardRanges {
    double n_min = 0, n_max = 0;
    double nb_min = 0, nb_max = 0;
    double d_max = 0;
    double f_min = 0, f_max = 0;
};

struct ParamRanges {
    double s2_min = kInfinity, s2_max = 0.0, amp = 0.0, sb2_min = kInfinity, sb2_max = 0.0, f_min = kInfinity, f_max = 0.0;
    double len_min = kInfinity, len_max = 0.0;
    bool finite = true;

    MCD_HD static double lesser(double a, double b) { return b < a ? b : a; }
    MCD_HD static double greater(double a, double b) { return a < b ? b : a; }

    MCD_HD void add_row(const double* p, int k, int model, bool free_centre) {
        const bool prof = is_profile(model);
        const int bg = bg_kind(model);
        const int ix = prof ? 3 : 2, iy = prof ? 4 : 3;
        const double s2 = p[1] * p[1];
        double a = fabs(p[0]) + fabs(p[ix]) + fabs(p[iy]);
        bool ok = true;
        if (prof) ok = ok && finite_value(p[2]) && finite_value(p[5]);
        double sb2 = 0.0, f = 0.0;
        if (bg == BG_GAUSS) {
            sb2 = p[k - 2] * p[k - 2];
            a = greater(a, fabs(p[k - 3]));
            ok = ok && finite_value(sb2);
        }
        if (bg == BG_GAUSS || bg == BG_FIXED_DENSITY) {
            f = p[k - 1];
            ok = ok && finite_value(f);
        }
        if (free_centre) {
            const int ic = prof ? 6 : 4;
            ok = ok && finite_value(p[ic]) && finite_value(p[ic + 1]);
        }
        ok = ok && finite_value(s2) && finite_value(a);
        if (!ok) { finite = false; return; }
        if (prof) {
            len_min = lesser(len_min, lesser(p[2], p[5]));
            len_max = greater(len_max, greater(p[2], p[5]));
        }
        if (bg == BG_GAUSS) { sb2_min = lesser(sb2_min, sb2); sb2_max = greater(sb2_max, sb2); }
        if (bg == BG_GAUSS || bg == BG_FIXED_DENSITY) { f_min = lesser(f_min, f); f_max = greater(f_max, f); }
        s2_min = lesser(s2_min, s2);
        s2_max = greater(s2_max, s2);
        amp = greater(amp, a);
    }

    MCD_HD void merge(const ParamRanges& o) {
        s2_min = lesser(s2_min, o.s2_min); s2_max = greater(s2_max, o.s2_max); amp = greater(amp, o.amp);
        sb2_min = lesser(sb2_min, o.sb2_min); sb2_max = greater(sb2_max, o.sb2_max);
        f_min = lesser(f_min, o.f_min); f_max = greater(f_max, o.f_max);
        len_min = lesser(len_min, o.len_min); len_max = greater(len_max, o.len_max);
        finite = finite && o.finite;
    }

    MCD_HD static bool finite_value(double x) { return fabs(x) <= 1.7976931348623157e308; }
};

MCD_HD bool guard_verdict(const StatsScalars& st, int model, bool f32, int64_t n_rows, const ParamRanges& pr,
                          GuardRanges* ranges) {
    if (!st.stats_finite || n_rows == 0 || !pr.finite) return false;
    const bool prof = is_profile(model);
    const int bg = bg_kind(model);
    const double s2_min = pr.s2_min, s2_max = pr.s2_max, amp = pr.amp, sb2_min = pr.sb2_min, sb2_max = pr.sb2_max;
    const double f_min = pr.f_min, f_max = pr.f_max, len_min = pr.len_min, len_max = pr.len_max;
    const double d_max = st.v_abs_max + amp;
    if (!(d_max <= 0x1p58)) return false;
    const double n_min = st.e2_min + (prof ? 0.0 : s2_min), n_max = st.e2_max + s2_max;
    if (ranges) {
        ranges->n_min = n_min; ranges->n_max = n_max; ranges->d_max = d_max;
        ranges->nb_min = st.e2_min + sb2_min; ranges->nb_max = st.e2_max + sb2_max;
        ranges->f_min = f_min; ranges->f_max = f_max;
    }
    if (prof && !(len_min >= 0x1p-100 && len_max <= 0x1p100)) return false;
    if (bg == BG_NONE) {
        if (f32)
            return (n_min >= 0x1p-15) && (n_max <= 0x1p15) && (d_max <= 0x1p15) &&
                   (!prof || (len_min >= 0x1p-20 && len_max <= 0x1p20));
        return (n_min >= 0x1p-55) && (n_max <= 0x1p55) && (d_max <= 0x1p50);
    }
    if (f32) {
        const double flo = 0x1p-15, fhi = 0x1p15;
        if (!(n_min >= flo && n_max <= fhi && d_max <= fhi && st.extras_ok)) return false;
        if (prof && !(len_min >= 0x1p-20 && len_max <= 0x1p20)) return false;
        const double g_max_log2 = -0.5 * log2(n_min), kLog2e = 1.4426950408889634;
        if (bg == BG_FIXED) {
            if (!(st.pm_max <= 1.0 - 0x1p-20 && st.lnbg_max <= 60.0 && st.lnbg_min >= -80.0)) return false;
            return ParamRanges::greater(0.0, -(st.lnbg_min + kHalfLn2Pi) * kLog2e + g_max_log2) + 1.0 <= 30.0;
        }
        if (bg == BG_FIXED_DENSITY) {
            if (!(f_min >= 0x1p-20 && f_max <= 0x1p20 && st.rho_min >= 0.0 && st.lnbg_max <= 60.0 && st.lnbg_min >= -80.0)) return false;
            const double up = log2(ParamRanges::greater(st.rho_max, 0x1p-60)) - (st.lnbg_min + kHalfLn2Pi) * kLog2e + g_max_log2;
            return ParamRanges::greater(log2(f_max), up) + 1.0 <= 30.0 && st.rho_min + f_min >= 0x1p-30 && st.rho_max + f_max <= 0x1p30;
        }
        if (!(st.e2_min + sb2_min >= flo && st.e2_max + sb2_max <= fhi)) return false;
        if (!(f_min >= 0x1p-20 && f_max <= 0x1p20 && st.rho_min >= 0x1p-20 && st.rho_max <= 0x1p20)) return false;
        const double gb_max_log2 = -0.5 * log2(st.e2_min + sb2_min);
        const double g_min_log2 = -0.5 * log2(n_max), gb_min_log2 = -0.5 * log2(st.e2_max + sb2_max);
        const double hi2 = ParamRanges::greater(log2(st.rho_max) + g_max_log2, log2(f_max) + gb_max_log2) + 1.0;
        const double lo2 = ParamRanges::lesser(log2(st.rho_min) + g_min_log2, log2(f_min) + gb_min_log2);
        return hi2 <= 30.0 && lo2 >= -30.0;
    }
    const double lo = 0x1p-200, hi = 0x1p200;
    if (!((n_min >= lo) && (n_max <= hi))) return false;
    if (!(d_max * d_max <= 1.6e9 * n_min)) return false;
    if (!st.extras_ok) return false;
    if (bg == BG_GAUSS) {
        if (!((st.e2_min + sb2_min >= lo) && (st.e2_max + sb2_max <= hi))) return false;
        if (!(d_max * d_max <= 1.6e9 * (st.e2_min + sb2_min))) return false;
    }
    if (bg == BG_GAUSS || bg == BG_FIXED_DENSITY)
        return f_min >= 0.0 && (st.rho_min + f_min >= 0x1p-100) && (st.rho_max + f_max <= 0x1p100);
    return true;
}

MCD_HD int level_verdict(const StatsScalars& st, int model, bool f32, int64_t n_rows, const ParamRanges& pr) {
    GuardRanges g;
    if (!guard_verdict(st, model, f32, n_rows, pr, &g)) return 0;
    if (f32) return 1;
    if (model == MODEL_PROFILE)
        return (st.r_max_fixed > 0.0 && pr.len_min >= 0x1p-10 && pr.len_max <= 0x1p16 &&
                st.r_max_fixed * st.r_max_fixed * 1.1 + pr.len_max * pr.len_max <= 0x1p34 && g.n_min >= 0x1p-30 &&
                g.n_max <= 0x1p30 && g.d_max <= 0x1p30) ? 2 : 1;
    const double lo = 0x1p-60, hi = 0x1p60;
    if (!st.narrow_possible) return 1;
    if (model == MODEL_BGFIXED && g.n_min >= lo && g.d_max * g.d_max <= 2.0e6 * g.n_min) return 2;
    if (bg_kind(model) == BG_FIXED_DENSITY && g.f_min >= 0x1p-20 && g.f_max <= 0x1p20 && g.n_min >= lo &&
        g.d_max * g.d_max <= 2.0e6 * g.n_min)
        return 2;
    if (bg_kind(model) == BG_GAUSS && g.f_min >= 0x1p-20 && g.f_max <= 0x1p20 && g.n_min >= lo && g.n_max <= hi &&
        g.nb_min >= lo && g.nb_max <= hi && g.d_max * g.d_max <= 2.0e6 * ParamRanges::lesser(g.n_min, g.nb_min))
        return 2;
    return 1;
}

MCD_HD int bounded_rescale(const StatsScalars& st, int model, bool free_centre, int64_t n_rows, const ParamRanges& pr) {
    if (model != MODEL_BGFIXED || free_centre) return 0;
    if (level_verdict(st, model, false, n_rows, pr) != 2) return 0;
    GuardRanges g;
    if (!guard_verdict(st, model, false, n_rows, pr, &g)) return 0;
    const double u_min = st.nbp_min - (1.0 + 0x1p-20) * (g.d_max * g.d_max) / (2.0 * g.n_min);
    if (!(u_min >= -700.0)) return 0;
    const double lo2 = -log2(1.0 - st.pm_max);
    const double hi2 = log2(1.0 + exp(st.nbp_max) / sqrt(g.n_min));
    for (int R = 32; R >= 16; R /= 2)
        if (R * hi2 <= 1000.0 && 1.0 + R * lo2 <= 1000.0) return R;
    return 0;
}

constexpr double kF32KappaV = 96.0;
constexpr double kF32KappaTheta = 2.0e-5;

struct F32Domain {
    bool inside = false;
    double kappa_v = 0.0, kappa_theta = 0.0;
    const char* reason = "";
};

inline F32Domain f32_domain(const CatalogStats& st, int model, bool free_centre, int k, const double* params, int64_t n_rows) {
    F32Domain out;
    ParamRanges pr;
    double rot = 0.0, a_min = kInfinity, off_max = 0.0;
    const bool prof = is_profile(model);
    const int ix = prof ? 3 : 2, ic = prof ? 6 : 4;
    for (int64_t i = 0; i < n_rows; ++i) {
        const double* p = params + i * k;
        pr.add_row(p, k, model, free_centre);
        rot = ParamRanges::greater(rot, std::fabs(p[ix]) + std::fabs(p[ix + 1]));
        if (prof) a_min = ParamRanges::lesser(a_min, p[2]);
        if (free_centre)
            off_max = ParamRanges::greater(off_max, std::hypot((p[ic] - st.ref_ra) * std::cos(st.ref_dec * 0.017453292519943295),
                                                               p[ic + 1] - st.ref_dec) * 3600.0);
    }
    GuardRanges g;
    const bool ranges_ok = guard_verdict(st, model, true, n_rows, pr, &g);
    double n_min = g.n_min;
    if (prof && st.r_max_arcsec > 0.0 && a_min > 0.0 && a_min < kInfinity) {
        const double R = st.r_max_arcsec + off_max;
        const double floor2 = pr.s2_min * a_min / std::sqrt(a_min * a_min + R * R);
        if (floor2 > 0.0 && floor2 < kInfinity) n_min += floor2;
    }
    if (bg_kind(model) == BG_GAUSS) n_min = ParamRanges::lesser(n_min, g.nb_min);
    out.kappa_v = n_min > 0.0 ? g.d_max / std::sqrt(n_min) : kInfinity;
    out.kappa_theta = free_centre ? (st.sep_harm > 0.0 && n_min > 0.0 ? rot / std::sqrt(n_min) * 0x1p-23 / st.sep_harm : kInfinity) : 0.0;
    if (!ranges_ok) out.reason = "variances, residuals or mixture values outside the float32 ranges (norm within 2^-15 .. 2^15, |v - v_los| <= 2^15, lnL_bg within -80 .. 60, pmember <= 1 - 2^-20, density and f_back within 2^-20 .. 2^20)";
    else if (!(out.kappa_v <= kF32KappaV)) out.reason = "(max|v| + |v_sys| + |v_maxx| + |v_maxy|) / sqrt(min(verr^2) + sigma^2) exceeds 96: the float32 rounding of the velocities is amplified beyond the stated tolerance";
    else if (free_centre && !(out.kappa_theta <= kF32KappaTheta)) out.reason = "free centre: rotation amplitude over dispersion times 2^-23 / (harmonic mean separation of the stars) exceeds 2e-5: the float32 tangent-plane offsets are too coarse for this catalogue";
    else out.inside = true;
    return out;
}

inline ParamRanges table_ranges(int model, bool free_centre, int k, const double* params, int64_t n_rows) {
    ParamRanges pr;
    for (int64_t i = 0; i < n_rows; ++i) pr.add_row(params + i * k, k, model, free_centre);
    return pr;
}

inline bool fast_guard(const CatalogStats& st, int model, bool free_centre, bool f32, int k, const double* params,
                       int64_t n_rows, GuardRanges* ranges = nullptr) {
    return guard_verdict(st, model, f32, n_rows, table_ranges(model, free_centre, k, params, n_rows), ranges);
}

inline int fast_level(const CatalogStats& st, int model, bool free_centre, bool f32, int k, const double* params,
                      int64_t n_rows) {
    return level_verdict(st, model, f32, n_rows, table_ranges(model, free_centre, k, params, n_rows));
}

inline int bounded_rescale(const CatalogStats& st, int model, bool free_centre, int k, const double* params, int64_t n_rows) {
    return bounded_rescale(st, model, free_centre, n_rows, table_ranges(model, free_centre, k, params, n_rows));
}

}
```

mcmc_dynamics_amd/csrc/mcd_host.h:

```cpp
#pragma once

#include <hip/hip_runtime.h>
#include <rccl/rccl.h>

#include <algorithm>
#include <atomic>
#include <chrono>
#include <cmath>
#include <cstdio>
#include <cstdlib>
#include <cstring>
#include <limits>
#include <map>
#include <memory>
#include <mutex>
#include <string>
#include <thread>
#include <vector>

#include "../../include/mcd.h"
#include "mcd_internal.h"
#include "mcd_guard.h"
#include "mcd_math.h"

struct mcd_ctx;
struct mcd_catalog;

#define MCD_HOST_BEGIN namespace mcd { namespace host __attribute__((visibility("hidden"))) {
#define MCD_HOST_END }}
MCD_HOST_BEGIN

extern thread_local std::string g_last_error;
int fail(int code, const std::string& msg);
int on_exception(const char* where) noexcept;

#define MCD_HIP(call)                                                                                   \
    do {                                                                                                \
        hipError_t e_ = (call);                                                                         \
        if (e_ != hipSuccess)                                                                           \
            return ::mcd::host::fail(MCD_ERR_HIP, std::string(#call) + ": " + hipGetErrorString(e_));   \
    } while (0)

struct Rccl {
    void* handle = nullptr;
    decltype(&ncclGetUniqueId) GetUniqueId = nullptr;
    decltype(&ncclCommInitRank) CommInitRank = nullptr;
    decltype(&ncclCommInitAll) CommInitAll = nullptr;
    decltype(&ncclCommDestroy) CommDestroy = nullptr;
    decltype(&ncclAllReduce) AllReduce = nullptr;
    decltype(&ncclGroupStart) GroupStart = nullptr;
    decltype(&ncclGroupEnd) GroupEnd = nullptr;
    decltype(&ncclGetErrorString) GetErrorString = nullptr;
    decltype(&ncclCommCount) CommCount = nullptr;
    decltype(&ncclCommUserRank) CommUserRank = nullptr;
    decltype(&ncclGetVersion) GetVersion = nullptr;
};
extern Rccl g_rccl;
int load_rccl();

#define MCD_NCCL(call)                                                                                  \
    do {                                                                                                \
        ncclResult_t r_ = (call);                                                                       \
        if (r_ != ncclSuccess)                                                                          \
            return ::mcd::host::fail(MCD_ERR_RCCL,                                                      \
                                   std::string(#call) + ": " + ::mcd::host::g_rccl.GetErrorString(r_)); \
    } while (0)

struct DeviceSlot {
    int device = 0;
    hipStream_t stream = nullptr;
    hipStream_t stream2 = nullptr;
    hipStream_t comm_stream = nullptr;
    ncclComm_t comm = nullptr;
};

struct WorkSet {
    int64_t n_walkers = 0;
    int64_t n_chunks = 0;
    int64_t max_chunks_per_pset = 0;
    int uniform_len = 0;
    int uniform_extra = 0;
    int waves = 4;
    mcd::Chunk* d_chunks = nullptr;
    int64_t* d_offsets = nullptr;
    uint8_t* d_chunk_general = nullptr;
    double* d_params = nullptr;
    void* d_wpar = nullptr;
    double* d_partials = nullptr;
    double* d_out = nullptr;
    double* d_out2 = nullptr;
    int buf = 0;
    double* d_partials2 = nullptr;
    double* d_grad_partials = nullptr;
    double* d_grad_out = nullptr;
    double* h_grad_out = nullptr;
    hipEvent_t ev_staged = nullptr;
    bool lane1_knows_staging = false;
    bool lane1_used = false;
    hipEvent_t ev_reduced[2] = {nullptr, nullptr};
    hipEvent_t ev_comm[2] = {nullptr, nullptr};
    bool comm_pending[2] = {false, false};
    double* h_params = nullptr;
    double* h_out = nullptr;
    double* m_params = nullptr;
    double* m_out = nullptr;
    bool mapped = false;
    double launch_tag = 0.0;
    int fast = 0;
    int narrow_rescale = 0;
    bool staged = false;
    bool sorted = false;
    std::vector<double> series_need;
    int64_t series_chunks = 0;
    std::vector<double> direct_need;
    int64_t direct_chunks = 0;
};

struct ChainArena {
    char* d = nullptr;
    char* h = nullptr;
    size_t bytes = 0;
};

struct Shard {
    int slot = 0;
    int64_t star_begin = 0;
    int64_t n = 0;
    void* records = nullptr;
    void* records_sorted = nullptr;
    std::vector<double> sorted_e2;
    std::vector<int64_t> sorted_exceptions;
    double* d_pset_const = nullptr;
    std::map<int64_t, WorkSet> work;
    hipEvent_t ev_begin = nullptr, ev_k0 = nullptr, ev_k1 = nullptr, ev_end = nullptr;
    std::vector<std::pair<hipEvent_t, hipEvent_t>> ring;
    size_t ring_used = 0;
};

struct DeviceScratch {
    std::vector<void*> blocks;
    hipEvent_t e0 = nullptr, e1 = nullptr;
    DeviceScratch() = default;
    DeviceScratch(const DeviceScratch&) = delete;
    template <class T>
    hipError_t malloc(T** p, size_t bytes) {
        blocks.push_back(nullptr);
        const hipError_t e = hipMalloc(&blocks.back(), bytes);
        *p = static_cast<T*>(blocks.back());
        return e;
    }
    hipError_t create_events() {
        const hipError_t e = hipEventCreate(&e0);
        return e != hipSuccess ? e : hipEventCreate(&e1);
    }
    ~DeviceScratch() {
        for (void* p : blocks) (void)hipFree(p);
        if (e0) (void)hipEventDestroy(e0);
        if (e1) (void)hipEventDestroy(e1);
    }
};

int ctx_fail(mcd_ctx* ctx, const std::string& what);
int ctx_usable(mcd_ctx* ctx);
int wait_ctx_stream(mcd_ctx* ctx, hipStream_t s, int64_t spin_us, const char* stage);
int build_workset(mcd_catalog* cat, Shard& sh, int64_t n_walkers, WorkSet** out);
LaunchShape main_launch_shape(mcd_catalog* cat, const Shard& sh, const WorkSet& w, int level, bool coll, double* out_buf,
                              int64_t n_out);
const double* fast_pset_const(const mcd_catalog* cat, const Shard& sh, int level);
const void* main_records(const Shard& sh, const WorkSet& w);
int64_t series_chunk_count(const mcd_catalog* cat, const WorkSet& w, int level, const double* params, int64_t n_rows);
int64_t direct_chunk_count(const mcd_catalog* cat, const WorkSet& w, int level, const double* params, int64_t n_rows);
int fast_level(const mcd_catalog* cat, const double* params, int64_t n_rows);
int sync_all(mcd_catalog* cat);

MCD_HOST_END

struct mcd_ctx {
    std::vector<mcd::host::DeviceSlot> slots;
    int rank = 0;
    int n_ranks = 1;
    bool multi_process = false;
    bool force_collective = false;
    int64_t collective_timeout_ms = 120000;
    std::atomic<int> abort_flag{0};
    std::atomic<int> failed{0};
    std::mutex note_mutex;
    std::string abort_reason;
    std::string failure;
    bool has_comm() const { return n_ranks > 1 || slots.size() > 1 || force_collective; }
};

struct mcd_catalog {
    mcd_ctx* ctx = nullptr;
    int model = 0;
    bool free_centre = false;
    int precision = 0;
    int k = 4;
    int64_t n_stars = 0;
    int64_t n_psets = 1;
    std::vector<int64_t> bin_offsets;
    std::vector<mcd::host::Shard> shards;
    mcd::CatalogStats stats;
    bool timing = false;
    bool timing_all = false;
    int allow_fast = 1;
    bool zero_copy = true;
    int64_t timing_stride = 1;
    int64_t timing_launches = 0;
    int64_t spin_us = 20000;
    int tail_split = 1;
    int64_t target_waves = 10240;
    int64_t chunk_len = 0;
    int prefetch = -1;
    int narrow_bounded = 1;
    int verr_sorted = -1;
    int root_series = 1;
    int root_direct = 1;
    int balance = -1;
    int two_lanes = 1;
    int f32_domain = 1;
    mcd::F32Domain last_f32;
    int64_t posterior_pass = 65536;
    int64_t loo_scratch_mb = 2048;
    int combine = 1;
    int64_t cur_walkers = 0;
    double last_kernel_ms = -1.0, last_device_ms = -1.0;
    bool timing_pending = false;
    int64_t last_grid = 0, last_chunks = 0;
    uint64_t launch_seq = 0;
    int64_t n_reruns = 0;
    int device_chain = 1;
    int fused_reduce = 1;
    int defer_guard = 1;
    bool chain_last_fused = false;
    mcd::host::ChainArena chain;
    int chain_hint = -1;
    int64_t chain_backoff = 0;
    int chain_consecutive = 0;
    int64_t chain_device_blocks = 0, chain_host_blocks = 0, chain_discarded = 0;
    int chain_last_status = 0;
    std::vector<hipEvent_t> chain_events;
    mcd::host::ChainArena hmc;
    int64_t hmc_device_blocks = 0, hmc_host_blocks = 0;
    int last_prefetch = -1;
    int64_t last_series_chunks = -1;
    int64_t last_direct_chunks = -1;
    int last_narrow_bounded = -1;
};

#define MCD_WAIT(ctx, stream, spin, stage)                                                              \
    do {                                                                                                \
        const int w_rc_ = ::mcd::host::wait_ctx_stream((ctx), (stream), (spin), (stage));               \
        if (w_rc_ != MCD_OK) return w_rc_;                                                              \
    } while (0)
```

mcmc_dynamics_amd/csrc/mcd_internal.h:

```cpp
#pragma once

#include <hip/hip_runtime.h>
#include <cstdint>

#include "mcd_chunks.h"
#include "mcd_guard.h"
#include "mcd_launch.h"

namespace mcd {

struct LaunchShape {
    int model;
    bool free_centre;
    int precision;
    int fast;
    int uniform_len = 0;
    int64_t n_records = 0;
    int uniform_extra = 0;
    int waves = 4;
    const uint8_t* chunk_general = nullptr;
    bool prefetch = false;
    int narrow_rescale = 0;
    bool root_series = false;
    bool root_direct = false;
    double* rerun_flag = nullptr;
    double launch_tag = 0.0;
};

struct RawColumns {
    const double* ra;
    const double* dec;
    const double* v;
    const double* verr;
    const double* lnbg;
    const double* pmember;
    const double* density;
};

hipError_t launch_prepare_records(hipStream_t s, const RawColumns& raw, int64_t n, int model, bool free_centre,
                                  int precision, double ra_c_deg, double dec_c_deg, void* records);

hipError_t launch_prepare_walkers(hipStream_t s, const double* params, int64_t n_rows, int k, int model,
                                  bool free_centre, int precision, void* wpar);

inline bool narrow_bounded_launch(const LaunchShape& sh) {
    return sh.fast == 2 && sh.model == MODEL_BGFIXED && !sh.free_centre && sh.precision == 0 && sh.prefetch &&
           (sh.narrow_rescale == 16 || sh.narrow_rescale == 32);
}

hipError_t launch_loglike(hipStream_t s, const LaunchShape& shape, const void* records, const Chunk* chunks,
                          int64_t n_chunks, const void* wpar, double* partials, int64_t n_walkers);

hipError_t launch_reduce(hipStream_t s, const double* partials, const int64_t* pset_slot_offsets,
                         int64_t n_psets, int64_t n_slots, int64_t max_slots_per_pset, int64_t n_walkers,
                         const double* pset_const, double* out);
int64_t partial_slots(const LaunchShape& shape, int64_t n_chunks, int64_t n_walkers);
constexpr int64_t kFusedReduceSlots = 256;

hipError_t launch_per_star(hipStream_t s, const LaunchShape& shape, const void* records, int64_t n,
                           const void* wpar_row, int mode, double* out);

int record_bytes(int model, bool free_centre, int precision);

enum ChainMeta : int { META_N_OK = 0, META_STATUS = 1, META_LEVEL = 2, META_WORDS = 4 };
enum ChainStatus : int {
    CHAIN_NAN = 1,
    CHAIN_RERUN = 2,
    CHAIN_LEVEL = 4,
    CHAIN_NO_PROPOSAL = 8
};
struct StretchDevice {
    int64_t n_bins = 1;
    int64_t n_walkers = 0;
    int32_t n_dim = 0, k = 0;
    int32_t fixed_ok = 1;
    int32_t model = 0, free_centre = 0;
    int32_t allow_fast = 1;
    int32_t expected_level = 0;
#ifdef MCD_CHAIN_STAMPS
    unsigned long long* stamps = nullptr;
    long long launch_index = 0;
#endif
    int32_t force_general = 0;
    int32_t fused = 0;
    const double* partials = nullptr;
    int64_t n_slots = 0;
    const int64_t* slot_offsets = nullptr;
    const double* pset_const = nullptr;
    StatsScalars stats;
    const int32_t* col_source = nullptr;
    const double* col_const = nullptr;
    const double* col_factor = nullptr;
    const double* lo = nullptr;
    const double* hi = nullptr;
    double* pos = nullptr;
    double* lnp = nullptr;
    long long* accepted = nullptr;
    const int32_t* order = nullptr;
    const double* zz = nullptr;
    const double* thr = nullptr;
    const int32_t* pick = nullptr;
    double* chain = nullptr;
    double* lnprob_chain = nullptr;
    double* proposal = nullptr;
    uint8_t* ok = nullptr;
    int32_t* meta = nullptr;
    int32_t* n_ok = nullptr;
    double* ranges = nullptr;
    double* table = nullptr;
    int32_t defer_guard = 0;
    double* table_log = nullptr;
    int32_t* n_ok_log = nullptr;
    int32_t* level_log = nullptr;
    double* wpar = nullptr;
};

hipError_t launch_stretch_step(hipStream_t s, const StretchDevice& d, int64_t acc_step, int acc_h, int64_t prop_step,
                               int prop_h, const double* ll, double rerun_tag);
hipError_t launch_stretch_status(hipStream_t s, const int32_t* meta, double* out);
hipError_t launch_stretch_judge(hipStream_t s, const StretchDevice& d, int64_t n_launches);
bool chain_numbers_on_device(int64_t n_walkers);
hipError_t launch_chain_numbers(hipStream_t s, uint64_t seed, int64_t step0, int64_t i0, int64_t i1, int64_t n_bins,
                                int64_t n_walkers, int n_dim, int32_t* order, double* zz, double* thr, int32_t* pick);
bool stretch_step_handles(const StretchDevice& d);
bool stretch_step_fuses(const StretchDevice& d);

int kde_slices(int64_t n, int64_t m, int* slice_len);
hipError_t launch_kde(hipStream_t s, const double* comp, int64_t m, const double* v, const double* verr, int64_t n,
                      double sigma_int, int slice_len, int n_slices, double* part_dmin, double* part_sum,
                      double* out);

}
```

mcmc_dynamics_amd/csrc/mcd_kernels.hip:

```cpp
#include <type_traits>

#include "mcd_internal.h"
#include "mcd_dispatch.h"
#include "mcd_math.h"
#include "mcd_prep.h"
#include "mcd_reduce.h"

namespace mcd {

namespace {

constexpr double kR0Arcmin = 3437.7467707849392526;

template <class T>
__global__ __launch_bounds__(kBlock) void prepare_records_kernel(RawColumns raw, int64_t n, int model,
                                                                  int free_centre, double ra_c, double dec_c,
                                                                  T* __restrict__ rec) {
    int64_t i = (int64_t)blockIdx.x * kBlock + threadIdx.x;
    if (i >= n) return;
    const int nd = record_doubles(model, free_centre != 0);
    T* r = rec + i * nd;
    const double verr = raw.verr[i];
    r[0] = (T)raw.v[i];
    r[1] = (T)(verr * verr);
    const double ra = raw.ra[i], dec = raw.dec[i];
    const int k = geometry_doubles(model, free_centre != 0);
    if (free_centre) {
        double sa, ca, sd, cd;
        sincos(ra * kDeg2Rad, &sa, &ca);
        sincos(dec * kDeg2Rad, &sd, &cd);
        r[2] = (T)(cd * sa); r[3] = (T)(cd * ca); r[4] = (T)sd; r[5] = (T)0;
    } else {
        const double dra = (ra - ra_c) * kDeg2Rad;
        const double dec_r = dec * kDeg2Rad, dec_cr = dec_c * kDeg2Rad;
        const double dx = -kR0Arcmin * cos(dec_r) * sin(dra);
        const double dy = kR0Arcmin * (sin(dec_r) * cos(dec_cr) - cos(dec_r) * sin(dec_cr) * cos(dra));
        if (is_profile(model)) {
            const double xs = 60.0 * dx, ys = 60.0 * dy;
            r[2] = (T)xs; r[3] = (T)ys; r[4] = (T)(xs * xs + ys * ys); r[5] = (T)0;
        } else {
            const double rr = hypot(dx, dy);
            double s, c;
            if (rr > 0.0) { s = dy / rr; c = dx / rr; }
            else { s = 0.0; c = signbit(dx) ? -1.0 : 1.0; }
            r[2] = (T)s; r[3] = (T)c;
        }
    }
    const int bg = bg_kind(model);
    if (bg == BG_FIXED) {
        const double b = raw.lnbg[i], pm = raw.pmember[i];
        r[k] = (T)b; r[k + 1] = (T)pm; r[k + 2] = (T)(1.0 - pm); r[k + 3] = (T)fmax(log(pm) - (b + kHalfLn2Pi), -2000.0);
    } else if (bg == BG_GAUSS) {
        r[k] = (T)raw.density[i]; r[k + 1] = (T)0;
    } else if (bg == BG_FIXED_DENSITY) {
        const double b = raw.lnbg[i];
        r[k] = (T)b; r[k + 1] = (T)fmax(log(raw.density[i]) - (b + kHalfLn2Pi), -2000.0); r[k + 2] = (T)raw.density[i];
        r[k + 3] = (T)0;
    }
}

template <class T>
__global__ __launch_bounds__(kBlock) void prepare_walkers_kernel(const double* __restrict__ params, int64_t n_rows,
                                                                  int k, int model, int free_centre,
                                                                  T* __restrict__ wpar) {
    int64_t i = (int64_t)blockIdx.x * kBlock + threadIdx.x;
    if (i >= n_rows) return;
    walker_constants<T>(params + i * k, model, free_centre != 0, wpar + i * KD);
}

#ifdef MCD_MAIN_STAMPS
constexpr int kStampBlocks = 1 << 16;
__device__ unsigned long long g_main_stamps[kStampBlocks][4];
#endif

__device__ const double kExpTabDevice[kExpTabSize] = {MCD_EXP_TABLE_VALUES};
__device__ const double kExpTabSqrt2Device[kExpTabSize] = {MCD_EXP_TABLE_SQRT2_VALUES};

template <int MODEL, bool FREE, class T, class A, int FAST, bool PF, int WAVES, bool BOUNDED = false>
__global__ __launch_bounds__(WAVES * kWave, WAVES > 4 ? 4 : 1) void loglike_kernel(const T* __restrict__ recs,
                                                                 const Chunk* __restrict__ chunks,
                                                                 const T* __restrict__ wpar,
                                                                 double* __restrict__ partials, int64_t n_tasks,
                                                                 int n_wtiles, int64_t n_walkers, int64_t n_chunks,
                                                                 int uniform_len, int uniform_extra, int64_t n_records,
                                                                 double* __restrict__ rerun_flag, double launch_tag,
                                                                 const uint8_t* __restrict__ chunk_general,
                                                                 int64_t n_slots, int narrow_iters, int root_series) {
    constexpr int ND = record_doubles(MODEL, FREE);
    constexpr int kThreads = WAVES * kWave;
    constexpr bool kCombine = WAVES > kWavesPerBlock;
#ifdef MCD_MAIN_STAMPS
    const unsigned long long stamp_entry = __builtin_amdgcn_s_memrealtime();
#endif
    constexpr bool kUsesExpTab = FAST && bg_kind(MODEL) != BG_NONE && sizeof(T) == 8;
    __shared__ double exptab_lds[kUsesExpTab ? kExpTabSize : 1];
    constexpr bool kTabBiased = kUsesExpTab && FAST == 2 && MODEL == MODEL_BGFIXED;
    __shared__ double combine_lds[kCombine ? WAVES : 1][kCombine ? kWave : 1];
    if constexpr (kUsesExpTab) {
        static_assert(kExpTabSize % kThreads == 0, "whole table entries per thread");
        const double* __restrict__ src = exp_table_is_sqrt2_scaled(MODEL) ? kExpTabSqrt2Device : kExpTabDevice;
#pragma unroll
        for (int i = 0; i < kExpTabSize / kThreads; ++i) {
            const int j = i * kThreads + threadIdx.x;
            exptab_lds[j] = kTabBiased ? exp_tab_bias(src[j], j) : src[j];
        }
        __syncthreads();
    }
    const int wave = __builtin_amdgcn_readfirstlane((int)(threadIdx.x >> 6));
    const int lane = threadIdx.x & (kWave - 1);
    int64_t chunk_id;
    int wtile;
    bool live = true;
    if (kCombine || n_wtiles <= kWavesPerBlock) {
        const int64_t task = (int64_t)blockIdx.x * WAVES + wave;
        if (task >= n_tasks) {
            if constexpr (!kCombine) return;
            live = false;
        }
        chunk_id = task / n_wtiles;
        wtile = (int)(task - chunk_id * n_wtiles);
        if (!live) { chunk_id = 0; wtile = wave % n_wtiles; }
    } else {
        const int m = (n_wtiles + kWavesPerBlock - 1) / kWavesPerBlock;
        const int64_t group = blockIdx.x / (8 * m);
        const int j = (int)(blockIdx.x - group * (8 * m));
        chunk_id = group * 8 + (j & 7);
        wtile = (j >> 3) * kWavesPerBlock + wave;
        if (chunk_id >= n_chunks || wtile >= n_wtiles) return;
    }
    Chunk ch;
    if (uniform_len > 0) {
        const int64_t shifted = chunk_id < (int64_t)uniform_extra ? chunk_id : (int64_t)uniform_extra;
        ch.begin = chunk_id * uniform_len + 8 * shifted;
        const int64_t left = n_records - ch.begin;
        ch.count = chunk_id == n_chunks - 1 ? (int32_t)left : uniform_len + (chunk_id < (int64_t)uniform_extra ? 8 : 0);
        ch.pset = 0;
    } else {
        ch = chunks[chunk_id];
    }
    const int64_t w_raw = (int64_t)wtile * kWave + lane;
    const bool active = w_raw < n_walkers;
    const int64_t w_idx = active ? w_raw : n_walkers - 1;

    double result = 0.0;
    if (live) {
        const T* __restrict__ wp = wpar + ((int64_t)ch.pset * n_walkers + w_idx) * KD;
        WalkerConsts<T> w;
        w.load(wp);

        const RecPtr<T> chunk_recs = (RecPtr<T>)(recs + ch.begin * ND);
        bool denormal;
        if constexpr (FAST == 2) {
            const bool general = bg_kind(MODEL) != BG_NONE && chunk_general != nullptr && chunk_general[chunk_id] != 0;
            if (general) result = chunk_loglike<MODEL, FREE, T, A, 1, PF, kTabBiased>(chunk_recs, ch.count, w, denormal, exptab_lds);
            else result = chunk_loglike<MODEL, FREE, T, A, 2, PF, kTabBiased, BOUNDED>(chunk_recs, ch.count, w, denormal,
                                                                                         exptab_lds, narrow_iters, root_series != 0,
                                                                                         root_series > 1);
        } else {
            result = chunk_loglike<MODEL, FREE, T, A, FAST, PF>(chunk_recs, ch.count, w, denormal, exptab_lds);
        }
        if (FAST && denormal && active) {
            if (rerun_flag) *rerun_flag = launch_tag;
            else result = __builtin_nan("");
        }
    }
    if constexpr (kCombine) {
        combine_lds[wave][lane] = result;
        __syncthreads();
        if (wave < n_wtiles) {
            double sum = combine_lds[wave][lane];
            for (int c = n_wtiles; c < WAVES; c += n_wtiles) sum += combine_lds[c + wave][lane];
            partials[partial_index(w_raw, n_slots, blockIdx.x)] = sum;
        }
    } else {
        partials[partial_index(w_raw, n_slots, chunk_id)] = result;
    }
#ifdef MCD_MAIN_STAMPS
    if (threadIdx.x == 0 && blockIdx.x < kStampBlocks) {
        g_main_stamps[blockIdx.x][0] = stamp_entry;
        g_main_stamps[blockIdx.x][1] = __builtin_amdgcn_s_memrealtime();
        g_main_stamps[blockIdx.x][2] = ((unsigned long long)__builtin_amdgcn_s_getreg((31 << 11) | 20) << 32) |
                                       (unsigned)__builtin_amdgcn_s_getreg((31 << 11) | 4);
        g_main_stamps[blockIdx.x][3] = (unsigned long long)ch.count;
    }
#endif
}

template <int SUB, int U, bool ONE_ROUND>
__global__ __launch_bounds__(kPartialGroup * SUB) void reduce_group_kernel(const double* __restrict__ partials,
                                                                            const int64_t* __restrict__ offs,
                                                                            int64_t n_slots, int64_t n_walkers,
                                                                            int64_t n_groups,
                                                                            const double* __restrict__ pset_const,
                                                                            double* __restrict__ out, int64_t single0) {
    constexpr int kThreads = kPartialGroup * SUB;
    constexpr int kWaves = kThreads / kWave;
    __shared__ double lds[kWaves > 1 ? kWaves : 1][kPartialGroup];
    const int64_t pset = blockIdx.x / n_groups, g = blockIdx.x - pset * n_groups;
    const int q = threadIdx.x & 3, s = threadIdx.x >> 2;
    const int64_t c0 = single0 >= 0 ? 0 : offs[pset], c1 = single0 >= 0 ? single0 : offs[pset + 1];
    const double add = pset_const ? pset_const[pset] : 0.0;
    const double2* __restrict__ col = reinterpret_cast<const double2*>(partials + g * n_slots * kPartialGroup) + q;
    double ax, ay;
    reduce_sublane_sum<SUB, U, ONE_ROUND>(col, c0, c1, s, ax, ay);
    reduce_wave_combine(ax, ay);
    const int lane = threadIdx.x & (kWave - 1);
    if constexpr (kWaves > 1) {
        if (lane < 4) { lds[threadIdx.x >> 6][2 * q] = ax; lds[threadIdx.x >> 6][2 * q + 1] = ay; }
        __syncthreads();
        if (threadIdx.x < kPartialGroup) {
            double acc = lds[0][threadIdx.x];
#pragma unroll
            for (int w = 1; w < kWaves; ++w) acc += lds[w][threadIdx.x];
            const int64_t w = g * kPartialGroup + threadIdx.x;
            if (w < n_walkers) out[pset * n_walkers + w] = acc + add;
        }
    } else {
        if (lane < 4) {
            const int64_t w = g * kPartialGroup + 2 * q;
            if (w < n_walkers) out[pset * n_walkers + w] = ax + add;
            if (w + 1 < n_walkers) out[pset * n_walkers + w + 1] = ay + add;
        }
    }
}

template <int MODEL, bool FREE, class T>
__global__ __launch_bounds__(kBlock) void per_star_kernel(const T* __restrict__ recs, int64_t n,
                                                           const T* __restrict__ wp, int mode,
                                                           double* __restrict__ out) {
    constexpr int ND = record_doubles(MODEL, FREE);
    const int64_t i = (int64_t)blockIdx.x * kBlock + threadIdx.x;
    if (i >= n) return;
    WalkerConsts<T> w;
    w.load(wp);
    T lc, lb, m;
    star_components<MODEL, FREE, T>((RecPtr<T>)(recs + i * ND), w, lc, lb, m);
    if (mode == 1) { out[i] = (double)mixture_lnl(lc, lb, m); return; }
    const T shift = is_profile(MODEL) ? max_(lc, lb) : T(0);
    const T ec = m * exp_(lc - shift), eb = (T(1) - m) * exp_(lb - shift);
    out[i] = (double)(ec / (ec + eb));
}

template <int MODEL, bool FREE, class T, class A, int FAST>
hipError_t launch_one(hipStream_t s, const LaunchShape& sh, const void* records, const Chunk* chunks, int64_t n_chunks,
                      const void* wpar, double* partials, int64_t n_walkers) {
    const int n_wtiles = (int)((n_walkers + kWave - 1) / kWave);
    const int64_t n_tasks = n_chunks * n_wtiles;
    constexpr bool kCanCombine = FAST != 0 && sizeof(T) == 8 && sizeof(A) == 8;
    const bool combine = kCanCombine && sh.waves > kWavesPerBlock;
    const int64_t grid = combine ? (n_tasks + sh.waves - 1) / sh.waves
                                 : main_grid(n_chunks, n_walkers);
    if (grid <= 0) return hipSuccess;
    const int64_t n_slots = combine ? grid : n_chunks;
    constexpr bool kCanBound = FAST == 2 && MODEL == MODEL_BGFIXED && !FREE && sizeof(T) == 8 && sizeof(A) == 8;
    const bool bounded = kCanBound && sh.prefetch && narrow_bounded_launch(sh);
    const int narrow_iters = bounded ? sh.narrow_rescale / 8 : 1;
#define MCD_LAUNCH_MAIN(PF_, WAVES_, BOUNDED_)                                                                               \
    hipLaunchKernelGGL((loglike_kernel<MODEL, FREE, T, A, FAST, PF_, WAVES_, BOUNDED_>), dim3((unsigned)grid),               \
                       dim3(WAVES_ * kWave), 0, s, (const T*)records, chunks, (const T*)wpar, partials, n_tasks, n_wtiles,   \
                       n_walkers, n_chunks, sh.uniform_len, sh.uniform_extra, sh.n_records, sh.rerun_flag, sh.launch_tag,    \
                       sh.chunk_general, n_slots, narrow_iters, sh.root_series ? (sh.root_direct ? 2 : 1) : 0)
    auto launch = [&](auto waves) {
        constexpr int W = decltype(waves)::value;
        if (bounded) MCD_LAUNCH_MAIN(true, W, kCanBound);
        else if (FAST != 0 && sh.prefetch) MCD_LAUNCH_MAIN((FAST != 0), W, false);
        else MCD_LAUNCH_MAIN(false, W, false);
        return hipGetLastError();
    };
#undef MCD_LAUNCH_MAIN
    if constexpr (kCanCombine) {
        if (combine && sh.waves == 8) return launch(std::integral_constant<int, 8>());
        if constexpr (bg_kind(MODEL) != BG_GAUSS) {
            if (combine && sh.waves == 16) return launch(std::integral_constant<int, 16>());
        }
        if (combine) return hipErrorInvalidValue;
    }
    return launch(std::integral_constant<int, kWavesPerBlock>());
}

template <int MODEL, bool FREE>
hipError_t launch_precision(hipStream_t s, const LaunchShape& sh, const void* records, const Chunk* chunks,
                            int64_t n_chunks, const void* wpar, double* partials, int64_t n_walkers) {
    switch (sh.precision) {
        case 0:
            if constexpr (bg_kind(MODEL) != BG_NONE || (MODEL == MODEL_PROFILE && !FREE)) {
                if (sh.fast == 2)
                    return launch_one<MODEL, FREE, double, double, 2>(s, sh, records, chunks, n_chunks, wpar, partials, n_walkers);
            }
            if (sh.fast) return launch_one<MODEL, FREE, double, double, 1>(s, sh, records, chunks, n_chunks, wpar, partials, n_walkers);
            return launch_one<MODEL, FREE, double, double, 0>(s, sh, records, chunks, n_chunks, wpar, partials, n_walkers);
        case 1:
            if (sh.fast) return launch_one<MODEL, FREE, float, float, 1>(s, sh, records, chunks, n_chunks, wpar, partials, n_walkers);
            return launch_one<MODEL, FREE, float, float, 0>(s, sh, records, chunks, n_chunks, wpar, partials, n_walkers);
        case 2:
            if (sh.fast) return launch_one<MODEL, FREE, float, double, 1>(s, sh, records, chunks, n_chunks, wpar, partials, n_walkers);
            return launch_one<MODEL, FREE, float, double, 0>(s, sh, records, chunks, n_chunks, wpar, partials, n_walkers);
    }
    return hipErrorInvalidValue;
}

}

#ifdef MCD_MAIN_STAMPS
extern "C" int mcd_debug_main_stamps(unsigned long long* out, long long n_blocks) {
    if (n_blocks > kStampBlocks) n_blocks = kStampBlocks;
    return (int)hipMemcpyFromSymbol(out, HIP_SYMBOL(g_main_stamps), (size_t)n_blocks * 4 * sizeof(unsigned long long));
}
#endif

int record_bytes(int model, bool free_centre, int precision) {
    return record_doubles(model, free_centre) * (precision == 0 ? 8 : 4);
}

hipError_t launch_prepare_records(hipStream_t s, const RawColumns& raw, int64_t n, int model, bool free_centre,
                                  int precision, double ra_c_deg, double dec_c_deg, void* records) {
    if (n <= 0) return hipSuccess;
    const unsigned grid = (unsigned)((n + kBlock - 1) / kBlock);
    return dispatch_term_type(precision, [&](auto t) {
        using T = decltype(t);
        hipLaunchKernelGGL(prepare_records_kernel<T>, dim3(grid), dim3(kBlock), 0, s, raw, n, model, (int)free_centre,
                           ra_c_deg, dec_c_deg, (T*)records);
        return hipGetLastError();
    });
}

hipError_t launch_prepare_walkers(hipStream_t s, const double* params, int64_t n_rows, int k, int model,
                                  bool free_centre, int precision, void* wpar) {
    if (n_rows <= 0) return hipSuccess;
    const unsigned grid = (unsigned)((n_rows + kBlock - 1) / kBlock);
    return dispatch_term_type(precision, [&](auto t) {
        using T = decltype(t);
        hipLaunchKernelGGL(prepare_walkers_kernel<T>, dim3(grid), dim3(kBlock), 0, s, params, n_rows, k, model,
                           (int)free_centre, (T*)wpar);
        return hipGetLastError();
    });
}

hipError_t launch_loglike(hipStream_t s, const LaunchShape& sh, const void* records, const Chunk* chunks,
                          int64_t n_chunks, const void* wpar, double* partials, int64_t n_walkers) {
    return dispatch_model(sh.model, sh.free_centre, [&](auto M, auto FREE) {
        return launch_precision<decltype(M)::value, decltype(FREE)::value>(s, sh, records, chunks, n_chunks, wpar, partials,
                                                                           n_walkers);
    }, hipErrorInvalidValue);
}

int64_t partial_slots(const LaunchShape& sh, int64_t n_chunks, int64_t n_walkers) {
    if (sh.waves <= kWavesPerBlock || sh.fast == 0 || sh.precision != 0) return n_chunks;
    const int64_t n_wtiles = (n_walkers + kWave - 1) / kWave;
    return (n_chunks * n_wtiles + sh.waves - 1) / sh.waves;
}

hipError_t launch_reduce(hipStream_t s, const double* partials, const int64_t* offs, int64_t n_psets,
                         int64_t n_slots, int64_t max_slots_per_pset, int64_t n_walkers, const double* pset_const,
                         double* out) {
    if (n_psets * n_walkers <= 0) return hipSuccess;
    const int64_t n_groups = (n_walkers + kPartialGroup - 1) / kPartialGroup;
    const dim3 grid((unsigned)(n_psets * n_groups));
    const int64_t single0 = n_psets == 1 ? n_slots : -1;
#define MCD_LAUNCH_REDUCE(SUB_, U_, ONE_)                                                                                   \
    hipLaunchKernelGGL((reduce_group_kernel<SUB_, U_, ONE_>), grid, dim3(kPartialGroup * SUB_), 0, s, partials, offs,       \
                       n_slots, n_walkers, n_groups, pset_const, out, single0)
    static_assert(kFusedReduceSlots == 2 * 8 * 16, "one round of the one-wave shape");
    if (max_slots_per_pset <= kFusedReduceSlots) MCD_LAUNCH_REDUCE(8, 16, true);
    else if (max_slots_per_pset <= 1024) MCD_LAUNCH_REDUCE(32, 16, true);
    else if (max_slots_per_pset <= 4096) MCD_LAUNCH_REDUCE(128, 16, true);
    else MCD_LAUNCH_REDUCE(128, 16, false);
#undef MCD_LAUNCH_REDUCE
    return hipGetLastError();
}

hipError_t launch_per_star(hipStream_t s, const LaunchShape& sh, const void* records, int64_t n,
                           const void* wpar_row, int mode, double* out) {
    if (n <= 0) return hipSuccess;
    const unsigned grid = (unsigned)((n + kBlock - 1) / kBlock);
    return dispatch_model(sh.model, sh.free_centre, [&](auto M, auto FREE) {
        if constexpr (bg_kind(decltype(M)::value) == BG_NONE) return hipErrorInvalidValue;
        else return dispatch_term_type(sh.precision, [&](auto t) {
            using T = decltype(t);
            hipLaunchKernelGGL((per_star_kernel<decltype(M)::value, decltype(FREE)::value, T>), dim3(grid), dim3(kBlock), 0, s,
                               (const T*)records, n, (const T*)wpar_row, mode, out);
            return hipGetLastError();
        });
    }, hipErrorInvalidValue);
}

}
```

mcmc_dynamics_amd/csrc/mcd_math.h:

```cpp
#pragma once

#include <cmath>
#include <cstdint>
#include <cstring>
#include <type_traits>

#include "mcd_exp_table.h"

#if defined(__HIPCC__)
#define MCD_HD __host__ __device__ __forceinline__
#else
#define MCD_HD inline
#endif
#if defined(__HIP_DEVICE_COMPILE__)
#define MCD_CONST_AS __attribute__((address_space(4)))
#else
#define MCD_CONST_AS
#endif
namespace mcd { template <class T> using RecPtr = const T MCD_CONST_AS*; }

#if defined(__HIP_DEVICE_COMPILE__)
#define MCD_KEEP_BRANCH() asm volatile("")
#else
#define MCD_KEEP_BRANCH() ((void)0)
// ... 305 lines not shown
    return y * s;
}

MCD_HD double add_hi_word(double x, int32_t v) {
    uint32_t w[2];
    std::memcpy(w, &x, sizeof w);
    w[1] += (uint32_t)v;
    std::memcpy(&x, w, sizeof x);
    return x;
}

constexpr int kExpTabHiShift = 20 - kExpTabBits;
MCD_HD double exp_tab_bias(double t, int j) { return add_hi_word(t, -(j << kExpTabHiShift)); }

template <bool TWO_STEP>
MCD_HD double exp_tab_reduce(double u, int& k) {
    constexpr double kMagic = 6755399441055744.0;
    const double shifted = fma_(u, kExpTabInvStep, kMagic);
    const double kf = shifted - kMagic;
    uint64_t bits;
    std::memcpy(&bits, &shifted, sizeof bits);
    k = (int)(uint32_t)bits;
    if constexpr (TWO_STEP) {
        const double r = fma_(-kf, kExpTabStepHi, u);
        return fma_(-kf, kExpTabStepLo, r);
    } else {
        return fma_(-kf, kExpTabStepHi + kExpTabStepLo, u);
    }
}
MCD_HD double exp_poly(double r) {
    double p;
    if constexpr (kExpPolyDegree == 4) p = fma_(fma_(r, kExpPolyC4, kExpPolyC3), r, kExpPolyC2);
    else p = fma_(r, kExpPolyC3, kExpPolyC2);
    p = fma_(p, r, 1.0);
    return fma_(p, r, 1.0);
}

template <bool TWO_STEP = true, bool BIASED = false>
MCD_HD double exp_tab(double u, int& e_out, const double* __restrict__ tab) {
    int k;
    const double p = exp_poly(exp_tab_reduce<TWO_STEP>(u, k));
    e_out = k >> kExpTabBits;
    const int j = k & (kExpTabSize - 1);
    if constexpr (BIASED) return add_hi_word(tab[j], j << kExpTabHiShift) * p;
    else return tab[j] * p;
}

constexpr int kExpTabKMin = -1021 * kExpTabSize;
MCD_HD double vgpr_constant(double x) {
#if defined(__HIP_DEVICE_COMPILE__)
    asm("" : "+v"(x));
#endif
    return x;
}
MCD_HD double vgpr_pinned(double x) {
#if defined(__HIP_DEVICE_COMPILE__)
    asm volatile("" : "+v"(x));
#endif
    return x;
}
template <bool TWO_STEP = false, bool CLAMP = true>
MCD_HD double exp_tab_scaled(double u, const double* __restrict__ tab) {
    int k;
    const double p = exp_poly(exp_tab_reduce<TWO_STEP>(u, k));
    if constexpr (CLAMP) k = k > kExpTabKMin ? k : kExpTabKMin;
    const double t = tab[k & (kExpTabSize - 1)];
    const int32_t kh = (int32_t)((uint32_t)k << kExpTabHiShift);
#if defined(__HIP_DEVICE_COMPILE__)
    if constexpr (!CLAMP) {
        typedef uint32_t word2 __attribute__((ext_vector_type(2)));
        word2 w = __builtin_bit_cast(word2, t);
        w.y += (uint32_t)kh;
        return __builtin_bit_cast(double, w) * p;
    }
#endif
    return add_hi_word(t, kh) * p;
}

struct RootCentre {
    double p, m0, inv, G0, q, corr;
    MCD_HD void setup(double eb, double s2) {
        p = 8.0 * eb;
        const double s2x = 8.0 * s2;
        m0 = p + s2x;
        const double bb = m0 - p;
        const double err = (p - (m0 - bb)) + (s2x - bb);
        inv = rcp_nr(m0);
        const double y = rsqrt_nr(m0);
        const double h = m0 * y;
        const double eh = fma_(m0, y, -h);
        const double res = fma_(-h, y, 1.0) - eh * y;
        G0 = 2.0 * y;
        q = 8.0 * inv;
        corr = 0.5 * (res - err * inv);
    }
};

struct RootSeries {
    static constexpr double kMaxT = 0x1p-13;
    double eb, b0, b1, b2, b3;
    MCD_HD bool setup(double eb_, double half, double s2) {
        eb = eb_;
        RootCentre c;
        c.setup(eb, s2);
        const double m0 = c.m0, G0 = c.G0, q = c.q;
        b0 = fma_(G0, c.corr, G0);
        b1 = -0.5 * (G0 * q);
        b2 = -0.75 * (b1 * q);
        b3 = (-5.0 / 6.0) * (b2 * q);
        return half >= 0.0 && 8.0 * half <= kMaxT * m0;
    }
    MCD_HD bool setup_chunk(double e_first, double e_last, double s2) {
        return setup(0.5 * e_first + 0.5 * e_last, 0.5 * (e_last - e_first), s2);
    }
    MCD_HD double g(double e) const {
        const double delta = e - eb;
        return fma_(fma_(fma_(b3, delta, b2), delta, b1), delta, b0);
    }
};

MCD_HD double fma_sgpr_factor(double a, double s, double c) {
#if defined(__HIP_DEVICE_COMPILE__)
    double r;
    asm("v_fma_f64 %0, %1, %2, %3" : "=v"(r) : "v"(a), "s"(s), "v"(c));
    return r;
#else
    return std::fma(a, s, c);
#endif
}

struct RootDirect {
    static constexpr double kRhoMax = 0.125;
    static constexpr double kErrorBound = 4.6e-16;
    double c0, c1, c2, c3;
    static MCD_HD bool direct_ok(double eb, double s2) { return (1.0 / kRhoMax - 1.0) * eb <= s2; }
    MCD_HD void setup(double eb, double s2) {
        RootCentre c;
        c.setup(eb, s2);
        const double G0 = c.G0, q = c.q;
        const double rho = c.p * c.inv;
        const double P = rho * fma_(rho, fma_(rho, 0.3125, 0.375), 0.5);
        c0 = fma_(G0, c.corr + P, G0);
        const double gq = G0 * q;
        c1 = -gq * fma_(rho, fma_(rho, 0.9375, 0.75), 0.5);
        const double gq2 = gq * q;
        c2 = gq2 * fma_(rho, 0.9375, 0.375);
        c3 = -0.3125 * (gq2 * q);
    }
    MCD_HD double g_direct(double e) const {
        return fma_sgpr_factor(fma_sgpr_factor(fma_sgpr_factor(c3, e, c2), e, c1), e, c0);
    }
};

MCD_HD bool wave_all(bool ok) {
#if defined(__HIP_DEVICE_COMPILE__)
    return __builtin_amdgcn_ballot_w64(!ok) == 0;
#else
    return ok;
#endif
}

MCD_HD bool is_zero_bits(double x) {
    uint64_t b;
    __builtin_memcpy(&b, &x, sizeof b);
    return (b << 1) == 0;
}

struct BgFixedAcc {
    LogProduct l;
    LogProduct lden;
    int emin;
    MCD_HD void init() { l.init(); lden.init(); emin = LogProduct::kTrackInit; }
    MCD_HD bool denormal() const { return emin < LogProduct::kTrackFloor; }
    template <bool NARROW = false>
    MCD_HD void add_density(double d, double n, double rho, double f, double nbp, const double* __restrict__ exptab) {
        add<false, false, NARROW>(d, n, f, nbp, exptab);
        lden.mul(rho + f);
    }
    template <bool UNIFORM_OMP = true, bool HALVED = false, bool NARROW = false, bool TAB_BIASED = false, bool CLAMP = true>
    MCD_HD void add(double d, double n, double omp, double nbp, const double* __restrict__ exptab) {
        const double g = (NARROW && HALVED) ? rsqrt2_newton(n) : rsqrt_nr(n);
        add_g<UNIFORM_OMP, HALVED, NARROW, TAB_BIASED, CLAMP>(d, g, omp, nbp, exptab);
    }
    template <bool UNIFORM_OMP = true, bool HALVED = false, bool NARROW = false, bool TAB_BIASED = false, bool CLAMP = true>
    MCD_HD void add_g(double d, double g, double omp, double nbp, const double* __restrict__ exptab) {
        const double dg = d * g;
        const double u0 = HALVED ? fnma_sgpr_addend(dg, dg, nbp) : fma_sgpr_addend(-0.5 * dg, dg, nbp);
        const double u = NARROW ? u0 : fmax_raw(u0, -1100.0);
        if constexpr (NARROW && TAB_BIASED) {
            const double es = exp_tab_scaled<false, CLAMP>(u, exptab);
            const double y = UNIFORM_OMP ? fma_sgpr_addend(g, es, omp) : fma_(g, es, omp);
            l.mul(y);
            return;
        }
        int k;
        const double er = exp_tab<!NARROW, TAB_BIASED>(u, k, exptab);
        if constexpr (NARROW) {
            const double y = UNIFORM_OMP ? fma_sgpr_addend(g, ldexp_(er, k), omp) : fma_(g, ldexp_(er, k), omp);
            l.mul(y);
            return;
        }
        const int kc = k > 1000 ? 1000 : k;
        const double y = UNIFORM_OMP ? fma_sgpr_addend(g, ldexp_(er, kc), omp) : fma_(g, ldexp_(er, kc), omp);
        l.mul_any_track(y, emin);
        l.e32 += k - kc;
    }
    MCD_HD void rescale() { l.rescale(); }
    MCD_HD void rescale_density() { l.rescale(); lden.rescale(); }
    MCD_HD void rescale_narrow() { l.rescale_narrow(); }
    MCD_HD void rescale_density_narrow() { l.rescale_narrow(); lden.rescale_narrow(); }
    MCD_HD double finish() { return l.value(); }
    MCD_HD double finish_density() { return l.value() - lden.value(); }
};

struct BgGaussAcc {
    double sum_min;
    LogProduct ly;
    LogProduct lden;
    int emin;
    MCD_HD void init() { sum_min = 0.0; ly.init(); lden.init(); emin = LogProduct::kTrackInit; }
    MCD_HD bool denormal() const { return emin < LogProduct::kTrackFloor; }
    template <bool HALVED = false, bool NARROW = false>
    MCD_HD void add(double d, double n, double db, double nb, double rho, double f, const double* __restrict__ exptab) {
        const double g = (NARROW && HALVED) ? rsqrt2_newton(n) : rsqrt_nr(n);
        const double gb = (NARROW && HALVED) ? rsqrt2_newton(nb) : rsqrt_nr(nb);
        const double dg = d * g, dbg = db * gb;
        const double w = dg * dg, wb = dbg * dbg;
        const double t = wb - w;
        const bool cluster_big = t >= 0.0;
        const double u0 = HALVED ? -fabs_(t) : -0.5 * fabs_(t);
        int k;
        const double er = exp_tab<!NARROW>(NARROW ? u0 : fmax_(u0, -1100.0), k, exptab);
        const double e = ldexp_(er, k);
        const double a = rho * g, b = f * gb;
        const double y = cluster_big ? fma_(b, e, a) : fma_(a, e, b);
        if constexpr (NARROW) ly.mul(y);
        else ly.mul_any_track(y, emin);
        lden.mul(rho + f);
        sum_min += fmin_(w, wb);
    }
    MCD_HD void rescale() { ly.rescale(); lden.rescale(); }
    MCD_HD void rescale_narrow() { ly.rescale_narrow(); lden.rescale_narrow(); }
    template <bool HALVED = false>
    MCD_HD double finish(int64_t count) {
        const double per_star = HALVED ? kHalfLn2Pi - 0.5 * kLn2 : kHalfLn2Pi;
        return fma_(-(double)count, per_star, HALVED ? -sum_min : -0.5 * sum_min) + (ly.value() - lden.value());
    }
};

template <class A>
struct LogProductF {
    A p;
    int e;
    MCD_HD void init() { p = 1; e = 0; }
    MCD_HD void mul(float x) { p *= (A)x; }
    MCD_HD void rescale() {
        int ex;
        p = frexp_(p, &ex);
        e += ex;
    }
    MCD_HD double value() {
        rescale();
        return fma_((double)e, kLn2, log_unit((double)p));
    }
};
template <class A>
struct BgFixedAccF {
    LogProductF<A> l, lden;
    MCD_HD void init() { l.init(); lden.init(); }
    MCD_HD void add(float d, float n, float w0, float nbp) {
        const float g = rsqf_(n);
        const float dg = d * g;
        l.mul(fma_(g, expf_(fma_(-0.5f * dg, dg, nbp)), w0));
    }
    MCD_HD void add_density(float d, float n, float rho, float f, float nbp) {
        add(d, n, f, nbp);
        lden.mul(rho + f);
    }
    MCD_HD void rescale() { l.rescale(); }
    MCD_HD void rescale_density() { l.rescale(); lden.rescale(); }
    MCD_HD double finish() { return l.value(); }
    MCD_HD double finish_density() { return l.value() - lden.value(); }
    MCD_HD A value_for_anchor() const { return l.p; }
};
template <class A>
struct BgGaussAccF {
    A sum_min;
    LogProductF<A> ly, lden;
    MCD_HD void init() { sum_min = 0; ly.init(); lden.init(); }
    MCD_HD void add(float d, float n, float db, float nb, float rho, float f) {
        const float g = rsqf_(n), gb = rsqf_(nb);
        const float dg = d * g, dbg = db * gb;
        const float w = dg * dg, wb = dbg * dbg;
        const float t = wb - w;
        const float e = expf_(-0.5f * (t < 0.0f ? -t : t));
        const float a = rho * g, b = f * gb;
        ly.mul(t >= 0.0f ? fma_(b, e, a) : fma_(a, e, b));
        lden.mul(rho + f);
        sum_min += (A)(w < wb ? w : wb);
    }
    MCD_HD void rescale() { ly.rescale(); lden.rescale(); }
    MCD_HD double finish(int64_t count) {
        return fma_(-(double)count, kHalfLn2Pi, -0.5 * (double)sum_min) + (ly.value() - lden.value());
    }
    MCD_HD A value_for_anchor() const { return ly.p; }
};

struct KdeLane {
    double v, h, d2min, sum;
    MCD_HD void init(double v_, double verr, double sigma_int2) {
        v = v_;
        h = 0.5 / fma_(verr, verr, sigma_int2);
    }
    MCD_HD void nearest(double c, double& dmin) const { dmin = fmin_(dmin, fabs_(c - v)); }
    MCD_HD void begin_sum(double dmin) { d2min = dmin * dmin; sum = 0.0; }
    MCD_HD void add(double c, const double* __restrict__ exptab) {
        const double d = c - v;
        const double u = fmax_(fma_(-d, d, d2min) * h, -800.0);
        int k;
        const double er = exp_tab<false>(u, k, exptab);
        sum += ldexp_(er, k);
    }
};

template <int BYTES, bool ON>
struct RecordPrefetch {
    static constexpr int kLines = (BYTES + 63) / 64 > 8 ? 8 : (BYTES + 63) / 64;
    uint32_t t;
    template <class P>
    MCD_HD void issue(P next) {
#if defined(__HIP_DEVICE_COMPILE__)
        if constexpr (ON) {
            const unsigned lane = __builtin_amdgcn_mbcnt_hi(~0u, __builtin_amdgcn_mbcnt_lo(~0u, 0u));
            typedef const uint32_t __attribute__((address_space(1)))* global_word_ptr;
            t = 0;
            if (lane < (unsigned)kLines) t = *(global_word_ptr)((uint64_t)next + lane * 64u);
            return;
        }
#endif
        (void)next;
        t = 0;
    }
    MCD_HD void retire(double anchor) {
#if defined(__HIP_DEVICE_COMPILE__)
        if constexpr (ON) asm volatile("" :: "v"(t), "v"(anchor));
#endif
        (void)anchor;
    }
};

template <class T> struct WalkerConsts {
    T vsys, s2, vx, vy, sac, cac, sdc, cdc, vb, sb2, fb, a2, s2a, rp2, rp_2;
    template <class P>
    MCD_HD void load(const P* __restrict__ p) {
        vsys = p[W_VSYS]; s2 = p[W_S2]; vx = p[W_VX]; vy = p[W_VY];
        sac = p[W_SAC]; cac = p[W_CAC]; sdc = p[W_SDC]; cdc = p[W_CDC];
        vb = p[W_VB]; sb2 = p[W_SB2]; fb = p[W_FB];
        a2 = p[W_A2]; s2a = p[W_S2A]; rp2 = p[W_RP2]; rp_2 = p[W_2RP];
// ... 99 lines not shown
            pf.retire((double)acc.value_for_anchor());
        }
        for (int j = n4 * 4; j < count; ++j, r += ND) { one(r); rescale(); }
    };
    if constexpr (BG == BG_GAUSS) {
        BgGaussAccF<A> acc;
        acc.init();
        run4(acc, [&](RecPtr<float> rr) {
            float d, n;
            star_d_n<MODEL, float, FREE, true>(rr, w, d, n);
            acc.add(d, n, rr[0] - w.vb, rr[1] + w.sb2, rr[XB], w.fb);
        }, [&]() { acc.rescale(); });
        return acc.finish(count);
    } else if constexpr (BG == BG_FIXED) {
        BgFixedAccF<A> acc;
        acc.init();
        run4(acc, [&](RecPtr<float> rr) {
            float d, n;
            star_d_n<MODEL, float, FREE, true>(rr, w, d, n);
            acc.add(d, n, rr[XB + 2], rr[XB + 3]);
        }, [&]() { acc.rescale(); });
        return acc.finish();
    } else {
        BgFixedAccF<A> acc;
        acc.init();
        run4(acc, [&](RecPtr<float> rr) {
            float d, n;
            star_d_n<MODEL, float, FREE, true>(rr, w, d, n);
            acc.add_density(d, n, rr[XB + 2], w.fb, rr[XB + 1]);
        }, [&]() { acc.rescale_density(); });
        return acc.finish_density();
    }
}

template <int MODEL, bool FREE, class A, bool PF>
MCD_HD double chunk_const_f32(RecPtr<float> r, int count, const WalkerConsts<float>& w) {
    constexpr int ND = record_doubles(MODEL, FREE);
    ConstAccF<A> acc;
    acc.init();
    constexpr bool TREE16 = MODEL == MODEL_CONST && !FREE;
    const int n16 = TREE16 ? count >> 4 : 0;
    for (int g = 0; g < n16; ++g, r += 16 * ND) {
        RecordPrefetch<16 * ND * 4, PF> pf;
        pf.issue(r + 16 * ND);
        float qq[16], nn[16];
#pragma unroll
        for (int j = 0; j < 16; ++j) {
            float d;
            star_d_n<MODEL, float, FREE, true>(r + j * ND, w, d, nn[j]);
            qq[j] = d * d;
        }
#pragma unroll
        for (int t = 0; t < 4; ++t) acc.add4(qq + 4 * t, nn + 4 * t);
        pf.retire((double)acc.p);
    }
    const int done = n16 << 4;
    const int n4 = (count - done) >> 2;
    for (int g = 0; g < n4; ++g, r += 4 * ND) {
        float qq[4], nn[4];
#pragma unroll
        for (int j = 0; j < 4; ++j) {
            float d;
            star_d_n<MODEL, float, FREE, true>(r + j * ND, w, d, nn[j]);
            qq[j] = d * d;
        }
        acc.add4(qq, nn);
    }
    for (int j = done + n4 * 4; j < count; ++j, r += ND) {
        float d, n;
        star_d_n<MODEL, float, FREE, true>(r, w, d, n);
        acc.add1(d * d, n);
    }
    return acc.finish(count);
}

template <bool PF>
MCD_HD double chunk_profile_narrow(RecPtr<double> r, int count, const WalkerConsts<double>& w) {
    constexpr int ND = record_doubles(MODEL_PROFILE, false);
    ProfileNarrowAcc acc;
    acc.init();
    const double hs2a = 0.5 * w.s2a;
    auto one = [&](RecPtr<double> rr, double& q1, double& n1, double& m1) {
        m1 = w.rp2 + rr[4];
        const double t2 = rsqrt2_newton(w.a2 + rr[4]);
        const double n = fma_(hs2a, t2, rr[1]);
        const double cross = fma_(w.vx, rr[3], -(w.vy * rr[2]));
        const double nd = fma_(rr[0] - w.vsys, m1, -(w.rp_2 * cross));
        q1 = nd * nd;
        n1 = (m1 * m1) * n;
    };
    const int n8 = count >> 3;
    for (int g = 0; g < n8; ++g, r += 8 * ND) {
        RecordPrefetch<8 * ND * 8, PF> pf;
        pf.issue(r + 8 * ND);
        double qq[8], nn[8], mm[8];
#pragma unroll
        for (int j = 0; j < 8; ++j) one(r + j * ND, qq[j], nn[j], mm[j]);
        const double m_prod = ((mm[0] * mm[1]) * (mm[2] * mm[3])) * ((mm[4] * mm[5]) * (mm[6] * mm[7]));
        acc.add8(qq, nn, m_prod);
        pf.retire(acc.q);
    }
    for (int j = count & ~7; j < count; ++j, r += ND) {
        double q1, n1, m1;
        one(r, q1, n1, m1);
        acc.add1(q1, n1, m1);
    }
    return acc.finish(count);
}

template <int MODEL, bool FREE, bool PF>
MCD_HD double chunk_const_fast(RecPtr<double> r, int count, const WalkerConsts<double>& w) {
    constexpr int ND = record_doubles(MODEL, FREE);
    ConstAcc acc;
    acc.init();
    constexpr bool TREE16 = MODEL == MODEL_CONST && !FREE;
    const int n16 = TREE16 ? count >> 4 : 0;
    for (int g = 0; g < n16; ++g, r += 16 * ND) {
        RecordPrefetch<16 * ND * 8, PF> pf;
        pf.issue(r + 16 * ND);
        double qq[16], nn[16];
#pragma unroll
        for (int j = 0; j < 16; ++j) {
            double d;
            star_d_n<MODEL, double, FREE, true>(r + j * ND, w, d, nn[j]);
            qq[j] = d * d;
        }
        acc.add16(qq, nn);
        pf.retire(acc.q);
    }
    const int n8 = TREE16 ? (count >> 3) & 1 : count >> 3;
    for (int g = 0; g < n8; ++g, r += 8 * ND) {
        RecordPrefetch<8 * ND * 8, PF> pf;
        pf.issue(r + 8 * ND);
        double qq[8], nn[8];
#pragma unroll
        for (int j = 0; j < 8; ++j) {
            double d;
            star_d_n<MODEL, double, FREE, true>(r + j * ND, w, d, nn[j]);
            qq[j] = d * d;
        }
        acc.add8(qq, nn);
        pf.retire(acc.q);
    }
    for (int j = count & ~7; j < count; ++j, r += ND) {
        double d, n;
        star_d_n<MODEL, double, FREE, true>(r, w, d, n);
        acc.add1(d * d, n);
    }
    return acc.finish(count);
}

template <int MODEL, bool FREE, int FAST, bool PF, bool TAB_BIASED, bool BOUNDED>
MCD_HD double chunk_bgfixed_fast(RecPtr<double> r, int count, const WalkerConsts<double>& w, bool& denormal,
                                 const double* __restrict__ exptab, int rescale_iters, bool series, bool direct) {
    constexpr int ND = record_doubles(MODEL, FREE);
    constexpr int XB = geometry_doubles(MODEL, FREE);
    constexpr bool HALVED = MODEL == MODEL_BGFIXED;
    constexpr bool NARROW = FAST == 2 && MODEL == MODEL_BGFIXED;
    constexpr double kScale = NARROW ? 8.0 : 2.0;
    const double s2x = kScale * w.s2;
    const double scale = BOUNDED ? vgpr_constant(kScale) : kScale;
    BgFixedAcc acc;
    acc.init();
    RootSeries sr;
    auto one = [&](RecPtr<double> rr, auto SERIES, double sc) {
        double d, n;
        star_d_n<MODEL, double, FREE, true>(rr, w, d, n);
        if constexpr (std::is_same<decltype(SERIES), RootDirect>::value) {
            acc.add_g<true, HALVED, NARROW, TAB_BIASED, !BOUNDED>(d, SERIES.g_direct(rr[1]), rr[XB + 2], rr[XB + 3], exptab);
        } else if constexpr (decltype(SERIES)::value) {
            acc.add_g<true, HALVED, NARROW, TAB_BIASED, !BOUNDED>(d, sr.g(rr[1]), rr[XB + 2], rr[XB + 3], exptab);
        } else {
            if constexpr (HALVED) n = fma_(sc, rr[1], s2x);
            acc.add<true, HALVED, NARROW, TAB_BIASED, !BOUNDED>(d, n, rr[XB + 2], rr[XB + 3], exptab);
        }
    };
    const int n4 = count >> 2;
    static_assert(!BOUNDED || (NARROW && PF && TAB_BIASED && !FREE), "the bounded loop is the prefetching BGFIXED one");
    auto four = [&](RecPtr<double> r4, auto SERIES) {
#pragma unroll
        for (int j = 0; j < 4; ++j) one(r4 + j * ND, SERIES, scale);
    };
    auto run = [&](auto SERIES) {
        if constexpr (BOUNDED) {
            int until = rescale_iters;
            for (int g = 0; g < (count >> 3); ++g, r += 8 * ND) {
                RecordPrefetch<8 * ND * 8, PF> pf;
                pf.issue(r + 8 * ND);
                four(r, SERIES);
                four(r + 4 * ND, SERIES);
                pf.retire(acc.l.p);
                if (--until == 0) { until = rescale_iters; MCD_KEEP_BRANCH(); acc.rescale_narrow(); }
            }
            acc.rescale_narrow();
            if (n4 & 1) {
                four(r, SERIES);
                r += 4 * ND;
                acc.rescale_narrow();
            }
        } else if constexpr (NARROW && PF) {
            for (int g = 0; g < (count >> 3); ++g, r += 8 * ND) {
                RecordPrefetch<8 * ND * 8, PF> pf;
                pf.issue(r + 8 * ND);
                four(r, SERIES);
                four(r + 4 * ND, SERIES);
                pf.retire(acc.l.p);
                acc.rescale_narrow();
            }
            if (n4 & 1) {
                four(r, SERIES);
                r += 4 * ND;
                acc.rescale_narrow();
            }
        } else if constexpr (NARROW) {
            for (int g = 0; g < n4; ++g, r += 4 * ND) {
                four(r, SERIES);
                if (g & 1) { MCD_KEEP_BRANCH(); acc.rescale_narrow(); }
            }
            if (n4 & 1) acc.rescale_narrow();
        } else {
            for (int g = 0; g < n4; ++g, r += 4 * ND) {
                RecordPrefetch<4 * ND * 8, PF> pf;
                pf.issue(r + 4 * ND);
                four(r, SERIES);
                pf.retire(acc.l.p);
                acc.rescale();
            }
        }
        for (int j = n4 * 4; j < count; ++j, r += ND) {
            one(r, SERIES, kScale);
            acc.rescale();
        }
    };
    constexpr bool kCanSeries = NARROW && MODEL == MODEL_BGFIXED && !FREE;
    bool use_series = false, use_direct = false;
    if constexpr (kCanSeries) {
        if (series && count > 0) {
            RootSeries vote;
            const bool ok = vote.setup_chunk(r[1], r[(int64_t)(count - 1) * ND + 1], w.s2);
            use_series = wave_all(ok);
            if (use_series && direct) use_direct = wave_all(RootDirect::direct_ok(vote.eb, w.s2));
        }
    }
    if constexpr (kCanSeries) {
        if (use_direct) {
            const double e_first = vgpr_pinned(r[1]), e_last = vgpr_pinned(r[(int64_t)(count - 1) * ND + 1]);
            RootDirect sd;
            sd.setup(0.5 * e_first + 0.5 * e_last, vgpr_pinned((1.0 / kScale) * s2x));
            run(sd);
        } else if (use_series) {
            const double e_first = vgpr_pinned(r[1]), e_last = vgpr_pinned(r[(int64_t)(count - 1) * ND + 1]);
            sr.setup_chunk(e_first, e_last, vgpr_pinned((1.0 / kScale) * s2x));
            run(std::true_type());
        }
        else run(std::false_type());
    } else {
        run(std::false_type());
    }
    const double result = acc.finish();
    denormal = acc.denormal();
    return result;
}

template <int MODEL, bool FREE, class T, class A, int FAST, bool PF = false, bool TAB_BIASED = false, bool BOUNDED = false>
MCD_HD double chunk_loglike(RecPtr<T> r, int count, const WalkerConsts<T>& w, bool& denormal,
                            const double* __restrict__ exptab, int rescale_iters = 1, bool series = false, bool direct = false) {
    constexpr int BG = bg_kind(MODEL);
    denormal = false;
    if constexpr (!FAST) {
        if constexpr (BG == BG_NONE) return chunk_plain<MODEL, FREE, T, A>(r, count, w);
        else return chunk_plain_mixture<MODEL, FREE, T, A>(r, count, w);
    } else if constexpr (sizeof(T) == 4) {
        if constexpr (BG == BG_NONE) return chunk_const_f32<MODEL, FREE, A, PF>(r, count, w);
        else return chunk_mixture_f32<MODEL, FREE, A, PF>(r, count, w);
    } else if constexpr (BG == BG_NONE) {
        if constexpr (FAST == 2 && MODEL == MODEL_PROFILE && !FREE) return chunk_profile_narrow<PF>(r, count, w);
        else return chunk_const_fast<MODEL, FREE, PF>(r, count, w);
    } else if constexpr (BG == BG_FIXED) {
        return chunk_bgfixed_fast<MODEL, FREE, FAST, PF, TAB_BIASED, BOUNDED>(r, count, w, denormal, exptab, rescale_iters, series, direct);
    } else if constexpr (BG == BG_FIXED_DENSITY) {
        constexpr int ND = record_doubles(MODEL, FREE);
        constexpr int XB = geometry_doubles(MODEL, FREE);
        constexpr bool NARROW = FAST == 2;
        BgFixedAcc acc;
        acc.init();
        auto four = [&](RecPtr<double> r4) {
#pragma unroll
            for (int j = 0; j < 4; ++j) {
                RecPtr<double> rr = r4 + j * ND;
                double d, n;
                star_d_n<MODEL, double, FREE, true, NARROW>(rr, w, d, n);
                acc.add_density<NARROW>(d, n, rr[XB + 2], w.fb, rr[XB + 1], exptab);
            }
        };
        const int n4 = count >> 2;
        if constexpr (NARROW) {
            for (int g = 0; g < n4; ++g, r += 4 * ND) {
                RecordPrefetch<4 * ND * 8, PF> pf;
                pf.issue(r + 4 * ND);
                four(r);
                pf.retire(acc.l.p);
                if (g & 1) { MCD_KEEP_BRANCH(); acc.rescale_density_narrow(); }
            }
            if (n4 & 1) acc.rescale_density_narrow();
        } else {
            for (int g = 0; g < n4; ++g, r += 4 * ND) {
                RecordPrefetch<4 * ND * 8, PF> pf;
                pf.issue(r + 4 * ND);
                four(r);
                pf.retire(acc.l.p);
                acc.rescale_density();
            }
        }
        for (int j = n4 * 4; j < count; ++j, r += ND) {
            double d, n;
            star_d_n<MODEL, double, FREE, true, NARROW>(r, w, d, n);
            acc.add_density<NARROW>(d, n, r[XB + 2], w.fb, r[XB + 1], exptab);
            acc.rescale_density();
        }
        const double result = acc.finish_density();
        denormal = acc.denormal();
        return result;
    } else {
        constexpr int ND = record_doubles(MODEL, FREE);
        constexpr int XB = geometry_doubles(MODEL, FREE);
        constexpr bool HALVED = MODEL == MODEL_BGGAUSS;
        constexpr bool NARROW = FAST == 2;
        constexpr double kScale = NARROW ? 8.0 : 2.0;
        const double s2x = kScale * w.s2, sb2x = kScale * w.sb2;
        BgGaussAcc acc;
        acc.init();
        auto one = [&](RecPtr<double> rr) {
            double d, n;
            star_d_n<MODEL, double, FREE, true, NARROW>(rr, w, d, n);
            if constexpr (HALVED) acc.add<true, NARROW>(d, fma_(kScale, rr[1], s2x), rr[0] - w.vb, fma_(kScale, rr[1], sb2x), rr[XB], w.fb, exptab);
            else acc.add<false, NARROW>(d, n, rr[0] - w.vb, rr[1] + w.sb2, rr[XB], w.fb, exptab);
        };
        auto four = [&](RecPtr<double> r4) {
#pragma unroll
            for (int j = 0; j < 4; ++j) one(r4 + j * ND);
        };
        const int n4 = count >> 2;
        if constexpr (NARROW) {
            for (int g = 0; g < n4; ++g, r += 4 * ND) {
                RecordPrefetch<4 * ND * 8, PF> pf;
                pf.issue(r + 4 * ND);
                four(r);
                pf.retire(acc.ly.p);
                if (g & 1) { MCD_KEEP_BRANCH(); acc.rescale_narrow(); }
            }
            if (n4 & 1) acc.rescale_narrow();
        } else {
            for (int g = 0; g < n4; ++g, r += 4 * ND) {
                RecordPrefetch<4 * ND * 8, PF> pf;
                pf.issue(r + 4 * ND);
                four(r);
                pf.retire(acc.ly.p);
                acc.rescale();
            }
        }
        for (int j = n4 * 4; j < count; ++j, r += ND) {
            one(r);
            acc.rescale();
        }
        const double result = acc.finish<HALVED>(count);
        denormal = acc.denormal();
        return result;
    }
}

template <int MODEL, bool FREE, class T>
MCD_HD void star_components(RecPtr<T> r, const WalkerConsts<T>& w, T& lc, T& lb, T& m) {
    constexpr int XB = geometry_doubles(MODEL, FREE);
    constexpr int BG = bg_kind(MODEL);
    T d, n;
    star_d_n<MODEL, T, FREE>(r, w, d, n);
    lc = gauss_lnl(d, n);
    if (BG == BG_FIXED) { lb = r[XB]; m = r[XB + 1]; }
    else if (BG == BG_FIXED_DENSITY) { lb = r[XB]; const T rho = r[XB + 2]; m = rho / (rho + w.fb); }
    else if (BG == BG_GAUSS) { lb = gauss_lnl(r[0] - w.vb, r[1] + w.sb2); const T rho = r[XB]; m = rho / (rho + w.fb); }
    else { lb = T(-INFINITY); m = T(1); }
}

}
```

Measured before the change: 1634 billion terms/s.

## Fold per-star exponent offset into split records for direct-root BGFIXED chunks

Adds a second, host-precomputed record layout in which each star's background log-ratio is split into an integer exponent offset (baked into a magic-number shift constant) and a fractional part whose exponential is folded into a scaled omp term. The fractional contributions are summed per chunk into a constant added after the product. This removes per-star work from the inner exp reduction in the narrow direct-root chunks: the kernel reads the new fields, uses a fused reduce-with-shift, and evaluates a step-scaled polynomial. The cost is a second full copy of the sorted records in device memory, a host preprocessing pass, and a guard that decides when the rescaled range stays safe.

```diff
diff --git a/include/mcd.h b/include/mcd.h
--- a/include/mcd.h
+++ b/include/mcd.h
@@ -156,6 +156,7 @@
 int mcd_last_narrow_bounded(const mcd_catalog* cat);
 int64_t mcd_last_series_chunks(const mcd_catalog* cat);
 int64_t mcd_last_direct_chunks(const mcd_catalog* cat);
+int mcd_last_exp_split(const mcd_catalog* cat);
 int mcd_last_fast_level(const mcd_catalog* cat);
 
 int mcd_last_f32_domain(const mcd_catalog* cat, double* kappa_v, double* kappa_theta);
diff --git a/mcmc_dynamics_amd/_native.py b/mcmc_dynamics_amd/_native.py
--- a/mcmc_dynamics_amd/_native.py
+++ b/mcmc_dynamics_amd/_native.py
@@ -74,6 +74,7 @@
     "mcd_last_narrow_bounded": (ctypes.c_int, [ctypes.c_void_p]),
     "mcd_last_series_chunks": (ctypes.c_int64, [ctypes.c_void_p]),
     "mcd_last_direct_chunks": (ctypes.c_int64, [ctypes.c_void_p]),
+    "mcd_last_exp_split": (ctypes.c_int, [ctypes.c_void_p]),
     "mcd_last_fast_level": (ctypes.c_int, [ctypes.c_void_p]),
     "mcd_last_f32_domain": (ctypes.c_int, [ctypes.c_void_p, _c_double_p, _c_double_p]),
     "mcd_set_option": (ctypes.c_int, [ctypes.c_void_p, ctypes.c_char_p, ctypes.c_int64]),
@@ -501,6 +502,10 @@
     def last_direct_chunks(self):
         return self.lib.mcd_last_direct_chunks(self.handle)
 
+    @property
+    def last_exp_split(self):
+        return self.lib.mcd_last_exp_split(self.handle)
+
     def hmc_block(self, plan, chol, step_size, n_leap, pos, lnp, seed, step0, n_steps, chain=None, lnprob_chain=None,
                   accepted=None, energy_error=None, jitter=0.1):
         if n_steps < 0 or step0 < 0 or pos.ndim != 2:
@@ -571,7 +576,8 @@
         _check(self.lib, self.lib.mcd_last_launch_info(self.handle, ctypes.byref(wg), ctypes.byref(tile),
                                                        ctypes.byref(ch), ctypes.byref(rb)), "mcd_last_launch_info")
         return {"workgroups": wg.value, "walker_tile": tile.value, "chunks": ch.value, "record_bytes": rb.value,
-                "series_chunks": self.last_series_chunks, "direct_chunks": self.last_direct_chunks}
+                "series_chunks": self.last_series_chunks, "direct_chunks": self.last_direct_chunks,
+                "exp_split": self.last_exp_split}
 
     def close(self):
         if getattr(self, "handle", None):
diff --git a/mcmc_dynamics_amd/csrc/mcd_api_catalog.hip b/mcmc_dynamics_amd/csrc/mcd_api_catalog.hip
--- a/mcmc_dynamics_amd/csrc/mcd_api_catalog.hip
+++ b/mcmc_dynamics_amd/csrc/mcd_api_catalog.hip
@@ -16,6 +16,7 @@
     if (w.d_chunks) (void)hipFree(w.d_chunks);
     if (w.d_offsets) (void)hipFree(w.d_offsets);
     if (w.d_chunk_general) (void)hipFree(w.d_chunk_general);
+    if (w.d_split_const) (void)hipFree(w.d_split_const);
     if (w.d_params) (void)hipFree(w.d_params);
     if (w.d_wpar) (void)hipFree(w.d_wpar);
     if (w.d_partials) (void)hipFree(w.d_partials);
@@ -78,12 +79,22 @@
         sh.sorted_e2[i] = out[i * ND + 1];
     }
     sh.sorted_exceptions = mcd::permuted_exceptions(cat->stats.narrow_exceptions, perm, sh.star_begin);
-    void* d = nullptr;
-    MCD_HIP(hipMalloc(&d, bytes + 2048));
-    hipError_t e = hipMemset(d, 0, bytes + 2048);
-    if (e == hipSuccess) e = hipMemcpy(d, out.data(), bytes, hipMemcpyHostToDevice);
-    if (e != hipSuccess) { (void)hipFree(d); MCD_HIP(e); }
-    sh.records_sorted = d;
+    sh.sorted_nbf.resize(n);
+    mcd::exp_split_records(out.data(), (int64_t)n, rec.data(), sh.sorted_nbf.data());
+    void* d[2] = {nullptr, nullptr};
+    const double* src[2] = {out.data(), rec.data()};
+    for (int a = 0; a < 2; ++a) {
+        hipError_t e = hipMalloc(&d[a], bytes + 2048);
+        if (e == hipSuccess) e = hipMemset(d[a], 0, bytes + 2048);
+        if (e == hipSuccess) e = hipMemcpy(d[a], src[a], bytes, hipMemcpyHostToDevice);
+        if (e != hipSuccess) {
+            for (int b = 0; b <= a; ++b)
+                if (d[b]) (void)hipFree(d[b]);
+            MCD_HIP(e);
+        }
+    }
+    sh.records_sorted = d[0];
+    sh.records_split = d[1];
     return MCD_OK;
 }
 
@@ -111,6 +122,7 @@
     {"narrow_bounded", 0, 1, "narrow_bounded: 1 (where the guard admits it, default) or 0 (never)", false, false, MCD_SET(c->narrow_bounded = (int)v)},
     {"verr_sorted", -1, 1, "verr_sorted: -1 (by record volume, default), 0 (catalogue order) or 1 (sorted by verr)", true, true, MCD_SET(c->verr_sorted = (int)v)},
     {"root_series", 0, 1, "root_series: 1 (series root on the narrow chunks of verr-sorted records, default) or 0 (never)", false, false, MCD_SET(c->root_series = (int)v)},
+    {"exp_split", 0, 1, "exp_split: 1 (split exponent offset in the direct chunks where the guard admits it, default) or 0 (never)", false, false, MCD_SET(c->exp_split = (int)v)},
     {"root_direct", 0, 1, "root_direct: 1 (direct form of the series root where a chunk admits it, default) or 0 (delta form only)", false, false, MCD_SET(c->root_direct = (int)v)},
     {"prefetch", -1, 1, "prefetch: -1 (by record volume, default), 0 (off) or 1 (on)", false, false, MCD_SET(c->prefetch = (int)v)},
     {"spin_us", 0, kMax, "spin_us must be >= 0", false, false, MCD_SET(c->spin_us = v)},
@@ -197,6 +209,7 @@
         w.series_need = mcd::series_thresholds(plan, sh.sorted_e2.data());
         w.direct_need = mcd::direct_thresholds(plan, sh.sorted_e2.data());
     }
+    const std::vector<double> split_const = sorted ? mcd::exp_split_chunk_consts(plan, sh.sorted_nbf.data()) : std::vector<double>();
     {
         const int64_t n_wtiles = (n_walkers + 63) / 64;
         const bool shape_ok = plan.balanced_m > 0 && plan.balanced_m % 2 == 0 && (n_wtiles == 1 || n_wtiles == 2 || n_wtiles == 4) &&
@@ -216,6 +229,10 @@
         if (!general.empty()) {
             if ((e = hipMalloc(&w.d_chunk_general, general.size())) != hipSuccess) return e;
             if ((e = hipMemcpy(w.d_chunk_general, general.data(), general.size(), hipMemcpyHostToDevice)) != hipSuccess) return e;
+        }
+        if (!split_const.empty()) {
+            if ((e = hipMalloc(&w.d_split_const, split_const.size() * sizeof(double))) != hipSuccess) return e;
+            if ((e = hipMemcpy(w.d_split_const, split_const.data(), split_const.size() * sizeof(double), hipMemcpyHostToDevice)) != hipSuccess) return e;
         }
         if ((e = hipMalloc(&w.d_chunks, std::max<size_t>(1, chunks.size()) * sizeof(mcd::Chunk))) != hipSuccess) return e;
         if ((e = hipMalloc(&w.d_offsets, offs.size() * sizeof(int64_t))) != hipSuccess) return e;
@@ -372,6 +389,7 @@
         for (auto& kv : sh.work) free_workset(kv.second);
         if (sh.records) (void)hipFree(sh.records);
         if (sh.records_sorted) (void)hipFree(sh.records_sorted);
+        if (sh.records_split) (void)hipFree(sh.records_split);
         if (sh.d_pset_const) (void)hipFree(sh.d_pset_const);
         if (sh.ev_begin) (void)hipEventDestroy(sh.ev_begin);
         if (sh.ev_k0) (void)hipEventDestroy(sh.ev_k0);
@@ -491,6 +509,7 @@
 int64_t mcd_last_direct_chunks(const mcd_catalog* cat) { return cat ? cat->last_direct_chunks : -1; }
 
 int mcd_last_narrow_bounded(const mcd_catalog* cat) { return cat ? cat->last_narrow_bounded : -1; }
+int mcd_last_exp_split(const mcd_catalog* cat) { return cat ? cat->last_exp_split : -1; }
 
 int mcd_last_f32_domain(const mcd_catalog* cat, double* kappa_v, double* kappa_theta) {
     if (!cat) return -1;
diff --git a/mcmc_dynamics_amd/csrc/mcd_api_chain.hip b/mcmc_dynamics_amd/csrc/mcd_api_chain.hip
--- a/mcmc_dynamics_amd/csrc/mcd_api_chain.hip
+++ b/mcmc_dynamics_amd/csrc/mcd_api_chain.hip
@@ -190,6 +190,7 @@
     cat->last_narrow_bounded = 0;
     cat->last_series_chunks = 0;
     cat->last_direct_chunks = 0;
+    cat->last_exp_split = 0;
     const double* pset_const = fast_pset_const(cat, sh, level);
     const int64_t n_slots = mcd::partial_slots(shape, w.n_chunks, half);
     const int64_t max_slots = B == 1 ? n_slots : w.max_chunks_per_pset;
diff --git a/mcmc_dynamics_amd/csrc/mcd_api_eval.hip b/mcmc_dynamics_amd/csrc/mcd_api_eval.hip
--- a/mcmc_dynamics_amd/csrc/mcd_api_eval.hip
+++ b/mcmc_dynamics_amd/csrc/mcd_api_eval.hip
@@ -100,6 +100,10 @@
         w->lane1_knows_staging = false;
         w->fast = fast;
         w->narrow_rescale = narrow_rescale;
+        for (int b = 0; b < 2; ++b)
+            w->exp_split[b] = fast == 2 && cat->precision == MCD_F64 && (b == 0 || narrow_rescale != 0) &&
+                              mcd::exp_split_admitted(cat->stats, cat->model, cat->free_centre, cat->k, params, n_rows,
+                                                      b ? narrow_rescale : 0);
         w->series_chunks = series_chunk_count(cat, *w, fast, params, n_rows);
         w->direct_chunks = direct_chunk_count(cat, *w, fast, params, n_rows);
         w->staged = true;
@@ -183,6 +187,11 @@
         mcd::LaunchShape shape = main_launch_shape(cat, sh, w, w.fast, coll, out_buf, n_out);
         shape.narrow_rescale = cat->narrow_bounded ? w.narrow_rescale : 0;
         cat->last_narrow_bounded = mcd::narrow_bounded_launch(shape) ? shape.narrow_rescale : 0;
+        if (cat->exp_split && w.sorted && w.d_split_const && w.exp_split[cat->last_narrow_bounded ? 1 : 0]) {
+            shape.records_split = sh.records_split;
+            shape.split_const = w.d_split_const;
+        }
+        cat->last_exp_split = mcd::exp_split_launch(shape) ? 1 : 0;
         if (&sh == &cat->shards.front()) cat->last_series_chunks = cat->last_direct_chunks = 0;
         cat->last_series_chunks += shape.root_series && shape.fast == 2 ? w.series_chunks : 0;
         cat->last_direct_chunks += shape.root_direct && shape.fast == 2 ? w.direct_chunks : 0;
diff --git a/mcmc_dynamics_amd/csrc/mcd_exp_split.h b/mcmc_dynamics_amd/csrc/mcd_exp_split.h
--- /dev/null
+++ b/mcmc_dynamics_amd/csrc/mcd_exp_split.h
@@ -0,0 +1,58 @@
+#pragma once
+
+#include <cmath>
+#include <cstdint>
+#include <vector>
+
+#include "mcd_chunks.h"
+#include "mcd_math.h"
+
+namespace mcd {
+
+constexpr long double kExpSplitInvStepL = 1.44269504088896340735992468100189214L * kExpTabSize;
+constexpr long double kExpSplitStepL = 0.693147180559945309417232121458176568L / kExpTabSize;
+constexpr double kExpSplitMagic = 6755399441055744.0;
+
+struct ExpSplitRecord {
+    double M, ompk, nbf;
+};
+inline ExpSplitRecord exp_split_record(double nbp, double omp) {
+    const long double t = (long double)nbp * kExpSplitInvStepL;
+    const long double nbi = rintl(t);
+    const double nbf = (double)(t - nbi);
+    const long double kappa = ((long double)kExpSplitC / (1 << kExpSplitShift)) * expl(-(long double)nbf * kExpSplitStepL);
+    ExpSplitRecord out;
+    out.M = (double)((long double)kExpSplitMagic + (nbi - (long double)(kExpSplitShift * kExpTabSize)));
+    out.ompk = (double)((long double)omp * kappa);
+    out.nbf = nbf;
+    return out;
+}
+
+inline double exp_split_chunk_const(const double* nbf, int64_t count) {
+    long double s = 0.0L;
+    for (int64_t i = 0; i < count; ++i) s += (long double)nbf[i];
+    return (double)(s * kExpSplitStepL - (long double)count * logl((long double)kExpSplitC / (1 << kExpSplitShift)));
+}
+
+inline void exp_split_records(const double* rec, int64_t n, double* out, double* nbf) {
+    constexpr int ND = record_doubles(MODEL_BGFIXED, false), XB = geometry_doubles(MODEL_BGFIXED, false);
+    for (int64_t i = 0; i < n; ++i) {
+        const double* r = rec + i * ND;
+        double* o = out + i * ND;
+        for (int j = 0; j < XB; ++j) o[j] = r[j];
+        const ExpSplitRecord s = exp_split_record(r[XB + 3], r[XB + 2]);
+        o[XB] = s.M;
+        o[XB + 1] = s.ompk;
+        o[XB + 2] = o[XB + 3] = 0.0;
+        nbf[i] = s.nbf;
+    }
+}
+
+inline std::vector<double> exp_split_chunk_consts(const ChunkPlan& plan, const double* nbf) {
+    std::vector<double> out(plan.chunks.size());
+    for (size_t c = 0; c < plan.chunks.size(); ++c)
+        out[c] = exp_split_chunk_const(nbf + plan.chunks[c].begin, plan.chunks[c].count);
+    return out;
+}
+
+}
diff --git a/mcmc_dynamics_amd/csrc/mcd_guard.h b/mcmc_dynamics_amd/csrc/mcd_guard.h
--- a/mcmc_dynamics_amd/csrc/mcd_guard.h
+++ b/mcmc_dynamics_amd/csrc/mcd_guard.h
@@ -265,6 +265,19 @@
     return 0;
 }
 
+constexpr double kExpSplitLog2KappaMax = 0.264872;
+constexpr int kExpSplitKMinBounded = -1034127 - 5 * 1024;
+MCD_HD bool exp_split_admitted(const StatsScalars& st, int model, bool free_centre, int64_t n_rows, const ParamRanges& pr,
+                               int rescale) {
+    if (model != MODEL_BGFIXED || free_centre) return false;
+    if (level_verdict(st, model, false, n_rows, pr) != 2) return false;
+    if (rescale == 0) return true;
+    GuardRanges g;
+    if (!guard_verdict(st, model, false, n_rows, pr, &g)) return false;
+    const double hi2 = log2(1.0 + exp(st.nbp_max) / sqrt(g.n_min));
+    return rescale * (hi2 + kExpSplitLog2KappaMax) <= 1000.0;
+}
+
 constexpr double kF32KappaV = 96.0;
 constexpr double kF32KappaTheta = 2.0e-5;
 
@@ -326,5 +339,9 @@
 inline int bounded_rescale(const CatalogStats& st, int model, bool free_centre, int k, const double* params, int64_t n_rows) {
     return bounded_rescale(st, model, free_centre, n_rows, table_ranges(model, free_centre, k, params, n_rows));
 }
-
-}
+inline bool exp_split_admitted(const CatalogStats& st, int model, bool free_centre, int k, const double* params, int64_t n_rows,
+                               int rescale) {
+    return exp_split_admitted(st, model, free_centre, n_rows, table_ranges(model, free_centre, k, params, n_rows), rescale);
+}
+
+}
diff --git a/mcmc_dynamics_amd/csrc/mcd_host.h b/mcmc_dynamics_amd/csrc/mcd_host.h
--- a/mcmc_dynamics_amd/csrc/mcd_host.h
+++ b/mcmc_dynamics_amd/csrc/mcd_host.h
@@ -19,6 +19,7 @@
 #include <vector>
 
 #include "../../include/mcd.h"
+#include "mcd_exp_split.h"
 #include "mcd_internal.h"
 #include "mcd_guard.h"
 #include "mcd_math.h"
@@ -84,6 +85,7 @@
     mcd::Chunk* d_chunks = nullptr;
     int64_t* d_offsets = nullptr;
     uint8_t* d_chunk_general = nullptr;
+    double* d_split_const = nullptr;
     double* d_params = nullptr;
     void* d_wpar = nullptr;
     double* d_partials = nullptr;
@@ -108,6 +110,7 @@
     double launch_tag = 0.0;
     int fast = 0;
     int narrow_rescale = 0;
+    bool exp_split[2] = {false, false};
     bool staged = false;
     bool sorted = false;
     std::vector<double> series_need;
@@ -129,6 +132,8 @@
     void* records = nullptr;
     void* records_sorted = nullptr;
     std::vector<double> sorted_e2;
+    void* records_split = nullptr;
+    std::vector<double> sorted_nbf;
     std::vector<int64_t> sorted_exceptions;
     double* d_pset_const = nullptr;
     std::map<int64_t, WorkSet> work;
@@ -215,6 +220,7 @@
     int narrow_bounded = 1;
     int verr_sorted = -1;
     int root_series = 1;
+    int exp_split = 1;
     int root_direct = 1;
     int balance = -1;
     int two_lanes = 1;
@@ -245,6 +251,7 @@
     int last_prefetch = -1;
     int64_t last_series_chunks = -1;
     int64_t last_direct_chunks = -1;
+    int last_exp_split = -1;
     int last_narrow_bounded = -1;
 };
 
diff --git a/mcmc_dynamics_amd/csrc/mcd_internal.h b/mcmc_dynamics_amd/csrc/mcd_internal.h
--- a/mcmc_dynamics_amd/csrc/mcd_internal.h
+++ b/mcmc_dynamics_amd/csrc/mcd_internal.h
@@ -23,6 +23,8 @@
     int narrow_rescale = 0;
     bool root_series = false;
     bool root_direct = false;
+    const void* records_split = nullptr;
+    const double* split_const = nullptr;
     double* rerun_flag = nullptr;
     double launch_tag = 0.0;
 };
@@ -46,6 +48,11 @@
 inline bool narrow_bounded_launch(const LaunchShape& sh) {
     return sh.fast == 2 && sh.model == MODEL_BGFIXED && !sh.free_centre && sh.precision == 0 && sh.prefetch &&
            (sh.narrow_rescale == 16 || sh.narrow_rescale == 32);
+}
+
+inline bool exp_split_launch(const LaunchShape& sh) {
+    return sh.fast == 2 && sh.model == MODEL_BGFIXED && !sh.free_centre && sh.precision == 0 && sh.root_series &&
+           sh.root_direct && sh.records_split != nullptr && sh.split_const != nullptr;
 }
 
 hipError_t launch_loglike(hipStream_t s, const LaunchShape& shape, const void* records, const Chunk* chunks,
diff --git a/mcmc_dynamics_amd/csrc/mcd_kernels.hip b/mcmc_dynamics_amd/csrc/mcd_kernels.hip
--- a/mcmc_dynamics_amd/csrc/mcd_kernels.hip
+++ b/mcmc_dynamics_amd/csrc/mcd_kernels.hip
@@ -85,7 +85,9 @@
                                                                  int uniform_len, int uniform_extra, int64_t n_records,
                                                                  double* __restrict__ rerun_flag, double launch_tag,
                                                                  const uint8_t* __restrict__ chunk_general,
-                                                                 int64_t n_slots, int narrow_iters, int root_series) {
+                                                                 int64_t n_slots, int narrow_iters, int root_series,
+                                                                 const T* __restrict__ recs_split,
+                                                                 const double* __restrict__ split_const) {
     constexpr int ND = record_doubles(MODEL, FREE);
     constexpr int kThreads = WAVES * kWave;
     constexpr bool kCombine = WAVES > kWavesPerBlock;
@@ -153,9 +155,9 @@
         if constexpr (FAST == 2) {
             const bool general = bg_kind(MODEL) != BG_NONE && chunk_general != nullptr && chunk_general[chunk_id] != 0;
             if (general) result = chunk_loglike<MODEL, FREE, T, A, 1, PF, kTabBiased>(chunk_recs, ch.count, w, denormal, exptab_lds);
-            else result = chunk_loglike<MODEL, FREE, T, A, 2, PF, kTabBiased, BOUNDED>(chunk_recs, ch.count, w, denormal,
-                                                                                         exptab_lds, narrow_iters, root_series != 0,
-                                                                                         root_series > 1);
+            else result = chunk_loglike<MODEL, FREE, T, A, 2, PF, kTabBiased, BOUNDED>(
+                     chunk_recs, ch.count, w, denormal, exptab_lds, narrow_iters, root_series != 0, root_series > 1,
+                     recs_split ? (RecPtr<T>)(recs_split + ch.begin * ND) : (RecPtr<T>) nullptr, split_const + chunk_id);
         } else {
             result = chunk_loglike<MODEL, FREE, T, A, FAST, PF>(chunk_recs, ch.count, w, denormal, exptab_lds);
         }
@@ -259,7 +261,8 @@
     hipLaunchKernelGGL((loglike_kernel<MODEL, FREE, T, A, FAST, PF_, WAVES_, BOUNDED_>), dim3((unsigned)grid),               \
                        dim3(WAVES_ * kWave), 0, s, (const T*)records, chunks, (const T*)wpar, partials, n_tasks, n_wtiles,   \
                        n_walkers, n_chunks, sh.uniform_len, sh.uniform_extra, sh.n_records, sh.rerun_flag, sh.launch_tag,    \
-                       sh.chunk_general, n_slots, narrow_iters, sh.root_series ? (sh.root_direct ? 2 : 1) : 0)
+                       sh.chunk_general, n_slots, narrow_iters, sh.root_series ? (sh.root_direct ? 2 : 1) : 0,                \
+                       (const T*)(exp_split_launch(sh) ? sh.records_split : nullptr), sh.split_const)
     auto launch = [&](auto waves) {
         constexpr int W = decltype(waves)::value;
         if (bounded) MCD_LAUNCH_MAIN(true, W, kCanBound);
diff --git a/mcmc_dynamics_amd/csrc/mcd_math.h b/mcmc_dynamics_amd/csrc/mcd_math.h
--- a/mcmc_dynamics_amd/csrc/mcd_math.h
+++ b/mcmc_dynamics_amd/csrc/mcd_math.h
@@ -481,6 +481,47 @@
     }
 };
 
+static_assert(kExpTabBits == 10 || kExpTabBits == 8, "kExpSplitC is written for N = 1024 (and halved exactly for N = 256)");
+constexpr double kExpSplitC = 0x1.337cc2183b050p+5 / (kExpTabBits == 10 ? 1.0 : 2.0);
+constexpr int kExpSplitShift = 5;
+constexpr double kExpSplitS1 = kExpTabStepHi + kExpTabStepLo;
+constexpr double kExpSplitS2 = kExpPolyC2 * kExpSplitS1 * kExpSplitS1;
+constexpr double kExpSplitS3 = kExpPolyC3 * kExpSplitS1 * kExpSplitS1 * kExpSplitS1;
+constexpr double kExpSplitS4 = kExpPolyC4 * kExpSplitS1 * kExpSplitS1 * kExpSplitS1 * kExpSplitS1;
+MCD_HD double exp_split_reduce(double dgs, double M, int& k) {
+    const double shifted = fnma_sgpr_addend(dgs, dgs, M);
+    const double w = shifted - M;
+    uint64_t bits;
+    std::memcpy(&bits, &shifted, sizeof bits);
+    k = (int)(uint32_t)bits;
+    return fma_(-dgs, dgs, -w);
+}
+MCD_HD double exp_poly_steps(double rv, double s1) {
+    double p;
+    if constexpr (kExpPolyDegree == 4) p = fma_(fma_(rv, kExpSplitS4, kExpSplitS3), rv, kExpSplitS2);
+    else p = fma_(rv, kExpSplitS3, kExpSplitS2);
+    p = fma_sgpr_addend(p, rv, s1);
+    return fma_(p, rv, 1.0);
+}
+
+struct RootDirectSplit : RootDirect {
+    MCD_HD void setup_scaled(double eb, double s2, double scale) {
+        RootCentre c;
+        c.setup(eb, s2);
+        const double q = c.q;
+        const double G0s = c.G0 * scale;
+        const double eg = fma_(c.G0, scale, -G0s);
+        const double rho = c.p * c.inv;
+        const double P = rho * fma_(rho, fma_(rho, 0.3125, 0.375), 0.5);
+        c0 = fma_(G0s, (c.corr + P) + eg * ((0.25 / scale) * (c.m0 * c.G0)), G0s);
+        const double gq = G0s * q;
+        c1 = -gq * fma_(rho, fma_(rho, 0.9375, 0.75), 0.5);
+        const double gq2 = gq * q;
+        c2 = gq2 * fma_(rho, 0.9375, 0.375);
+        c3 = -0.3125 * (gq2 * q);
+    }
+};
+
 MCD_HD bool wave_all(bool ok) {
 #if defined(__HIP_DEVICE_COMPILE__)
     return __builtin_amdgcn_ballot_w64(!ok) == 0;
@@ -533,6 +574,28 @@
         const double y = UNIFORM_OMP ? fma_sgpr_addend(g, ldexp_(er, kc), omp) : fma_(g, ldexp_(er, kc), omp);
         l.mul_any_track(y, emin);
         l.e32 += k - kc;
+    }
+    template <bool TAB_BIASED = false, bool CLAMP = true>
+    MCD_HD void add_gs(double d, double gs, double M, double ompk, double s1, const double* __restrict__ exptab) {
+        int k;
+        const double p = exp_poly_steps(exp_split_reduce(d * gs, M, k), s1);
+        if constexpr (CLAMP) k = k > kExpTabKMin ? k : kExpTabKMin;
+        double es;
+        if constexpr (TAB_BIASED) {
+            const double t = exptab[k & (kExpTabSize - 1)];
+            const int32_t kh = (int32_t)((uint32_t)k << kExpTabHiShift);
+#if defined(__HIP_DEVICE_COMPILE__)
+            typedef uint32_t word2 __attribute__((ext_vector_type(2)));
+            word2 tw = __builtin_bit_cast(word2, t);
+            tw.y += (uint32_t)kh;
+            es = __builtin_bit_cast(double, tw) * p;
+#else
+            es = add_hi_word(t, kh) * p;
+#endif
+        } else {
+            es = ldexp_(exptab[k & (kExpTabSize - 1)] * p, k >> kExpTabBits);
+        }
+        l.mul(fma_sgpr_addend(gs, es, ompk));
     }
     MCD_HD void rescale() { l.rescale(); }
     MCD_HD void rescale_density() { l.rescale(); lden.rescale(); }
@@ -938,7 +1001,8 @@
 
 template <int MODEL, bool FREE, int FAST, bool PF, bool TAB_BIASED, bool BOUNDED>
 MCD_HD double chunk_bgfixed_fast(RecPtr<double> r, int count, const WalkerConsts<double>& w, bool& denormal,
-                                 const double* __restrict__ exptab, int rescale_iters, bool series, bool direct) {
+                                 const double* __restrict__ exptab, int rescale_iters, bool series, bool direct,
+                                 RecPtr<double> r_split, const double* __restrict__ split_const) {
     constexpr int ND = record_doubles(MODEL, FREE);
     constexpr int XB = geometry_doubles(MODEL, FREE);
     constexpr bool HALVED = MODEL == MODEL_BGFIXED;
@@ -952,7 +1016,9 @@
     auto one = [&](RecPtr<double> rr, auto SERIES, double sc) {
         double d, n;
         star_d_n<MODEL, double, FREE, true>(rr, w, d, n);
-        if constexpr (std::is_same<decltype(SERIES), RootDirect>::value) {
+        if constexpr (std::is_same<decltype(SERIES), RootDirectSplit>::value) {
+            acc.add_gs<TAB_BIASED, !BOUNDED>(d, SERIES.g_direct(rr[1]), rr[XB], rr[XB + 1], sc, exptab);
+        } else if constexpr (std::is_same<decltype(SERIES), RootDirect>::value) {
             acc.add_g<true, HALVED, NARROW, TAB_BIASED, !BOUNDED>(d, SERIES.g_direct(rr[1]), rr[XB + 2], rr[XB + 3], exptab);
         } else if constexpr (decltype(SERIES)::value) {
             acc.add_g<true, HALVED, NARROW, TAB_BIASED, !BOUNDED>(d, sr.g(rr[1]), rr[XB + 2], rr[XB + 3], exptab);
@@ -964,8 +1030,13 @@
     const int n4 = count >> 2;
     static_assert(!BOUNDED || (NARROW && PF && TAB_BIASED && !FREE), "the bounded loop is the prefetching BGFIXED one");
     auto four = [&](RecPtr<double> r4, auto SERIES) {
+        if constexpr (std::is_same<decltype(SERIES), RootDirectSplit>::value) {
 #pragma unroll
-        for (int j = 0; j < 4; ++j) one(r4 + j * ND, SERIES, scale);
+            for (int j = 0; j < 4; ++j) one(r4 + j * ND, SERIES, kExpSplitS1);
+        } else {
+#pragma unroll
+            for (int j = 0; j < 4; ++j) one(r4 + j * ND, SERIES, scale);
+        }
     };
     auto run = [&](auto SERIES) {
         if constexpr (BOUNDED) {
@@ -1014,22 +1085,33 @@
             }
         }
         for (int j = n4 * 4; j < count; ++j, r += ND) {
-            one(r, SERIES, kScale);
+            one(r, SERIES, std::is_same<decltype(SERIES), RootDirectSplit>::value ? kExpSplitS1 : kScale);
             acc.rescale();
         }
     };
     constexpr bool kCanSeries = NARROW && MODEL == MODEL_BGFIXED && !FREE;
     bool use_series = false, use_direct = false;
+    const bool split = kCanSeries && r_split != nullptr;
     if constexpr (kCanSeries) {
         if (series && count > 0) {
             RootSeries vote;
-            const bool ok = vote.setup_chunk(r[1], r[(int64_t)(count - 1) * ND + 1], w.s2);
+            const RecPtr<double> rv = split ? r_split : r;
+            const bool ok = vote.setup_chunk(rv[1], rv[(int64_t)(count - 1) * ND + 1], w.s2);
             use_series = wave_all(ok);
             if (use_series && direct) use_direct = wave_all(RootDirect::direct_ok(vote.eb, w.s2));
         }
     }
     if constexpr (kCanSeries) {
-        if (use_direct) {
+        if (use_direct && split) {
+            r = r_split;
+            const double e_first = vgpr_pinned(r[1]), e_last = vgpr_pinned(r[(int64_t)(count - 1) * ND + 1]);
+            RootDirectSplit sd;
+            sd.setup_scaled(0.5 * e_first + 0.5 * e_last, vgpr_pinned((1.0 / kScale) * s2x), kExpSplitC);
+            run(sd);
+            const double result = acc.finish() + *split_const;
+            denormal = acc.denormal();
+            return result;
+        } else if (use_direct) {
             const double e_first = vgpr_pinned(r[1]), e_last = vgpr_pinned(r[(int64_t)(count - 1) * ND + 1]);
             RootDirect sd;
             sd.setup(0.5 * e_first + 0.5 * e_last, vgpr_pinned((1.0 / kScale) * s2x));
@@ -1050,7 +1132,8 @@
 
 template <int MODEL, bool FREE, class T, class A, int FAST, bool PF = false, bool TAB_BIASED = false, bool BOUNDED = false>
 MCD_HD double chunk_loglike(RecPtr<T> r, int count, const WalkerConsts<T>& w, bool& denormal,
-                            const double* __restrict__ exptab, int rescale_iters = 1, bool series = false, bool direct = false) {
+                            const double* __restrict__ exptab, int rescale_iters = 1, bool series = false, bool direct = false,
+                            RecPtr<T> r_split = nullptr, const double* __restrict__ split_const = nullptr) {
     constexpr int BG = bg_kind(MODEL);
     denormal = false;
     if constexpr (!FAST) {
@@ -1063,7 +1146,7 @@
         if constexpr (FAST == 2 && MODEL == MODEL_PROFILE && !FREE) return chunk_profile_narrow<PF>(r, count, w);
         else return chunk_const_fast<MODEL, FREE, PF>(r, count, w);
     } else if constexpr (BG == BG_FIXED) {
-        return chunk_bgfixed_fast<MODEL, FREE, FAST, PF, TAB_BIASED, BOUNDED>(r, count, w, denormal, exptab, rescale_iters, series, direct);
+        return chunk_bgfixed_fast<MODEL, FREE, FAST, PF, TAB_BIASED, BOUNDED>(r, count, w, denormal, exptab, rescale_iters, series, direct, r_split, split_const);
     } else if constexpr (BG == BG_FIXED_DENSITY) {
         constexpr int ND = record_doubles(MODEL, FREE);
         constexpr int XB = geometry_doubles(MODEL, FREE);
```

After: 1692 billion terms/s (median of 6 runs). +3.6%, better.
